# eichenberger/stereo-svo-slam

Measured on AMD Instinct MI355X. Metric: tracked_frames_per_sec, higher is better.
Workload: dtype f32

## Files before the change

### include/svo_hip.h

```cpp
#ifndef SVO_HIP_H
#define SVO_HIP_H

#include <stddef.h>

#include "svo_types.h"

#ifdef __cplusplus
extern "C" {
#endif

enum {
    SVO_OK = 0,
    SVO_ERR_INVALID = -1,
    SVO_ERR_HIP = -2,
    SVO_ERR_NO_DEVICE = -3,
    SVO_ERR_CAPACITY = -4
};

typedef struct svo_handle svo_handle;

const char *svo_last_error(void);
int svo_version(void);

int svo_handle_create(int device, int max_keypoints, svo_handle **out);
int svo_handle_destroy(svo_handle *h);
int svo_handle_set_stream(svo_handle *h, void *hip_stream);
int svo_handle_synchronize(svo_handle *h);
int svo_handle_set_fast_solver(svo_handle *h, int on);
int svo_handle_set_exact_pinv(svo_handle *h, int on);

int svo_device_malloc(size_t bytes, void **out);
int svo_device_free(void *p);
int svo_copy_to_device(svo_handle *h, void *dst, const void *src, size_t bytes);
int svo_copy_to_host(svo_handle *h, void *dst, const void *src, size_t bytes);
int svo_copy_image_to_device(svo_handle *h, void *dst, size_t dst_stride, const void *src,
                             size_t src_stride, size_t width, size_t height);

int svo_build_pyramid(svo_handle *h, int n_levels, svo_image *levels);
int svo_build_lk_pyramid(svo_handle *h, int max_levels, int win, svo_image *levels, int *n_out);

int svo_remap_linear(svo_handle *h, int n, const svo_image *src, svo_image *dst,
                     const float *map_x, const float *map_y);

int svo_remap_linear_multi(svo_handle *h, int n, const svo_image *src, svo_image *dst, int n_maps,
                           const float *const *map_x, const float *const *map_y, const int *map_of_image);

typedef struct svo_camera_calibration {
    double K[9], D[8], R[9], P[9];
} svo_camera_calibration;
int svo_rectify_inverse(const svo_camera_calibration *cal, double ir[9]);
int svo_build_rectify_maps(svo_handle *h, int n, const svo_camera_calibration *cal, int width, int height,
                           float *const *map_x, float *const *map_y);

enum { SVO_INPUT_GRAY_PAIR = 0,
       SVO_INPUT_BGR_PAIR  = 1,
       SVO_INPUT_RGB_PAIR  = 2,
       SVO_INPUT_SBS_GRAY  = 3,
       SVO_INPUT_SBS_BGR   = 4,
       SVO_INPUT_SBS_RGB   = 5,
       SVO_INPUT_CH3_ECON  = 6 };
enum { SVO_INGEST_COPY = 0,
       SVO_INGEST_GRAY = 1 };
typedef struct svo_input_side {
    int32_t buffer;
    int32_t start_column;
    int32_t op, channel;
    int32_t weight[3];
} svo_input_side;
typedef struct svo_input_layout {
    int32_t buffers;
    int32_t channels;
    int32_t min_row_pixels;
    svo_input_side left, right;
} svo_input_layout;
int svo_input_format_info(int format, int width, svo_input_layout *out);
int svo_convert_frames(svo_handle *h, int format, int n, const svo_image *src_a, const svo_image *src_b,
                       svo_image *left, svo_image *right);

int svo_sparse_align(svo_handle *h, const svo_image *prev_pyr, const svo_image *cur_pyr,
                     const svo_kp2d *kps2d, const svo_kp3d *kps3d, const uint32_t *flags, int n,
                     const svo_camera_settings *cam, const float *pose_guess, float *pose_out,
                     float *cost, svo_gn_trace *trace, float *dbg, int dbg_level);

int svo_project_keypoints(svo_handle *h, const float *pose, const svo_kp3d *kps3d, int n,
                          const svo_camera_settings *cam, svo_kp2d *out);

int svo_klt_track(svo_handle *h, const svo_image *prev_lk, const svo_image *cur_lk, int n_levels,
                  const svo_kp2d *prev_pts, svo_kp2d *cur_pts, int n, int win,
                  uint8_t *status, float *err);

int svo_reproj_gn(svo_handle *h, svo_kp2d *kps2d, const svo_kp3d *kps3d, uint32_t *flags, int n,
                  const svo_camera_settings *cam, const svo_kp2d *tracked, const float *err,
                  const float *pose_in, float *pose_out, float *cost, svo_gn_trace *trace);

int svo_ssd_disparity(svo_handle *h, const svo_image *left, const svo_image *right,
                      const svo_kp2d *kps2d, int n, int win, int search_x, int search_y,
                      int clamp_half, float *disparity);

int svo_depth_filter_update(svo_handle *h, const svo_kp2d *kps2d, svo_kp3d *kps3d,
                            const uint32_t *flags, int n, const svo_camera_settings *cam,
                            const float *frame_pose, const float *disparity,
                            const svo_kp3d *ref3d, const svo_kp2d *ref2d, const float *kf_pose,
                            int32_t *outlier_count, int32_t *inlier_count,
                            float *kf_inv_depth, float *kf_variance,
                            int do_outlier_check, int do_update);

typedef struct svo_det_cell {
    float   x, y;
    float   score;
    int32_t type;
} svo_det_cell;
int svo_detect_keypoints(svo_handle *h, int n_levels, const svo_image *levels, int grid_width,
                         int grid_height, int max_cells, svo_det_cell *cells, int32_t *counts);
int svo_detect_shape(int width, int height, int n_levels, int grid_width, int grid_height,
                     int *max_cells, int *cell_width, int *cell_height, int *list_capacity);

typedef struct svo_ctx svo_ctx;

enum { SVO_MEM_HOST = 0, SVO_MEM_DEVICE = 1, SVO_MEM_DEVICE_BORROW = 2 };

int svo_ctx_create(const svo_camera_settings *cam, int width, int height, int n_sequences,
                   int device, svo_ctx **out);
int svo_ctx_destroy(svo_ctx *ctx);

int svo_new_images(svo_ctx *ctx, const uint8_t *const *left, const uint8_t *const *right,
                   int stride, const float *time_stamps, int mem);
int svo_submit_images(svo_ctx *ctx, const uint8_t *const *left, const uint8_t *const *right,
                      int stride, const float *time_stamps, int mem);
int svo_wait(svo_ctx *ctx);
int svo_ctx_get_groups(svo_ctx *ctx, int *n_groups);
int svo_ctx_restart_sequences(svo_ctx *ctx, const int *seqs, int n);
typedef struct svo_run_info {
    int32_t seq, run;
    int32_t frames, keyframes;
    float   last_time_stamp;
    float   pose[6];
} svo_run_info;
int svo_get_finished_runs(svo_ctx *ctx, int seq, int *n);
int svo_get_finished_run(svo_ctx *ctx, int seq, int i, svo_run_info *info, svo_pose *trajectory,
                         int cap, int *n_poses);
int svo_drop_finished_runs(svo_ctx *ctx, int seq);
typedef struct svo_memory {
    int64_t device_bytes;
    int64_t klt_cache_bytes;
    int32_t image_sets, image_sets_free;
    int32_t keyframe_slabs, keyframe_slabs_free;
} svo_memory;
int svo_ctx_get_memory(svo_ctx *ctx, svo_memory *out);
int svo_submit_trim_keyframes(svo_ctx *ctx, const int *seqs, const int *below, int n);
int svo_trim_keyframes(svo_ctx *ctx, const int *seqs, const int *below, int n);
int svo_ctx_set_keyframe_window(svo_ctx *ctx, int keep);
typedef struct svo_keyframe_range {
    int32_t first;
    int32_t retired;
    int32_t count;
    int32_t table;
} svo_keyframe_range;
int svo_get_keyframe_range(svo_ctx *ctx, int seq, svo_keyframe_range *out);
int svo_ctx_set_rectification(svo_ctx *ctx, const float *left_map_x, const float *left_map_y,
                              const float *right_map_x, const float *right_map_y, int mem);
typedef struct svo_rig {
    float baseline, fx, fy, cx, cy, k1, k2, k3, p1, p2;
    const float *left_map_x, *left_map_y, *right_map_x, *right_map_y;
    int32_t mem;
    int32_t _reserved;
} svo_rig;
int svo_ctx_add_rigs(svo_ctx *ctx, const svo_rig *rigs, int n, int *ids);
int svo_ctx_remove_rigs(svo_ctx *ctx, const int *ids, int n);
int svo_ctx_assign_rigs(svo_ctx *ctx, const int *seqs, const int *rigs, int n);
int svo_ctx_get_slot_rig(svo_ctx *ctx, int seq, int *rig, svo_camera_settings *cam);
int svo_ctx_get_rigs(svo_ctx *ctx, int *n, int64_t *map_bytes);
int svo_ctx_add_rigs_calibrated(svo_ctx *ctx, const svo_rig *rigs, const svo_camera_calibration *left,
                                const svo_camera_calibration *right, int n, int *ids);
int svo_ctx_set_calibration(svo_ctx *ctx, const svo_camera_calibration *left, const svo_camera_calibration *right);
int svo_ctx_set_input_format(svo_ctx *ctx, int format);
int svo_new_image(svo_ctx *ctx, const uint8_t *left, int left_stride, const uint8_t *right,
                  int right_stride, int width, int height, float time_stamp);

int svo_get_pose(svo_ctx *ctx, int seq, float pose[6]);
int svo_get_frame_keypoints(svo_ctx *ctx, int seq, svo_kp2d *kps2d, svo_kp3d *kps3d,
                            svo_kp_info *info, int cap, int *n);
int svo_get_keyframe_count(svo_ctx *ctx, int seq, int *count);
int svo_get_keyframe(svo_ctx *ctx, int seq, int id, svo_kp2d *kps2d, svo_kp3d *kps3d,
                     svo_kp_info *info, float pose[6], int cap, int *n);
int svo_get_trajectory(svo_ctx *ctx, int seq, svo_pose *out, int cap, int *n);
int svo_update_pose(svo_ctx *ctx, int seq, const float pose[6], const float speed[6],
                    const float pose_var[6], const float speed_var[6], double dt,
                    float filtered[6]);

int svo_submit_pose_updates(svo_ctx *ctx, const int *seqs, const int *counts, int n,
                            const svo_pose_sample *samples, float *filtered);
int svo_update_poses(svo_ctx *ctx, const int *seqs, const int *counts, int n,
                     const svo_pose_sample *samples, float *filtered);
int svo_pose_filter_batch(svo_handle *h, int n_states, const float *state_in, const float *start_pose,
                          const int *first, int n_samples, const svo_pose_sample *samples, float *state_out,
                          float *filtered);

enum { SVO_EXPORT_FRAMES = 0,
       SVO_EXPORT_LAST_KEYFRAMES = 1 };

typedef struct svo_export_segment {
    int32_t seq, run;
    int32_t frame_id;
    int32_t keyframe_id;
    int32_t is_keyframe;
    int32_t n;
    int64_t first;
    float   pose[6];
    float   time_stamp;
    int32_t _pad;
} svo_export_segment;

typedef struct svo_export_dst {
    svo_export_segment *segments;
    svo_kp2d *kps2d; svo_kp3d *kps3d; svo_kp_info *info;
    int64_t capacity;
} svo_export_dst;

int svo_export_capacity(const svo_camera_settings *cam, int width, int height, int *records_per_sequence);
int svo_submit_export(svo_ctx *ctx, int what, const int *seqs, int n, const svo_export_dst *dst, int mem);
int svo_export(svo_ctx *ctx, int what, const int *seqs, int n, const svo_export_dst *dst, int mem);
int svo_pack_keypoints(svo_handle *h, int n_sets, const svo_keypoints *sets, const int64_t *first,
                       svo_kp2d *kps2d, svo_kp3d *kps3d, svo_kp_info *info);

typedef struct svo_map_point {
    float   x, y, z;
    uint8_t color[3];
    uint8_t flags;
} svo_map_point;

typedef struct svo_map_filter {
    uint32_t drop_flags;
    int32_t  own_only;
    int32_t  min_inliers;
    int32_t  _reserved;
} svo_map_filter;

typedef struct svo_map_keyframe {
    int32_t id, n_total, n, _pad;
    int64_t first;
    float   pose[6];
} svo_map_keyframe;

enum { SVO_MAP_COMPLETE = 0,
       SVO_MAP_TOO_SMALL = 1 };

typedef struct svo_map_segment {
    int32_t seq, run;
    int32_t frame_id;
    int32_t status;
    int32_t n_keyframes, keyframes_retired;
    int32_t from_keyframe, n_exported;
    int64_t n_points;
    int64_t points_bound;
    float   time_stamp;
    union {
        int32_t first_keyframe;
        int32_t _pad[3];
    };
} svo_map_segment;

typedef struct svo_map_region {
    int64_t first_point;
    int64_t point_capacity;
    int64_t first_keyframe_entry;
    int32_t keyframe_capacity;
    int32_t from_keyframe;
} svo_map_region;

typedef struct svo_map_dst {
    svo_map_segment  *segments;
    svo_map_keyframe *keyframes;
    svo_map_point    *points;
} svo_map_dst;

int svo_map_size(svo_ctx *ctx, int seq, int from_keyframe, int *keyframes, int64_t *points_bound);
int svo_submit_export_map(svo_ctx *ctx, const int *seqs, int n, const svo_map_region *regions,
                          const svo_map_filter *filter, const svo_map_dst *dst, int mem);
int svo_export_map(svo_ctx *ctx, const int *seqs, int n, const svo_map_region *regions,
                   const svo_map_filter *filter, const svo_map_dst *dst, int mem);
int svo_pack_map_points(svo_handle *h, int n_regions, const int32_t *set_begin, const svo_keypoints *sets,
                        const int32_t *own_id, const int64_t *first, const svo_map_filter *filter,
                        svo_map_point *points, int32_t *counts);

enum { SVO_PLANE_LEFT = 0, SVO_PLANE_RIGHT = 1 };
enum { SVO_PIXEL_GRAY8 = 0, SVO_PIXEL_RGB8 = 1, SVO_PIXEL_RGBA8 = 2 };
enum { SVO_VIEW_OK = 0,
       SVO_VIEW_NONE = 1 };

typedef struct svo_view_style {
    int32_t  plane;
    int32_t  level;
    int32_t  pixel;
    int32_t  markers;
    uint32_t drop_flags;
    int32_t  size, size_temporary;
    int32_t  _reserved;
} svo_view_style;

typedef struct svo_view_segment {
    int32_t seq, run;
    int32_t frame_id;
    int32_t keyframe_id;
    int32_t status;
    int32_t n;
    int64_t offset;
    float   pose[6];
    float   time_stamp;
    int32_t _pad;
} svo_view_segment;

typedef struct svo_view_dst {
    svo_view_segment *segments;
    uint8_t *pixels;
    int64_t capacity;
} svo_view_dst;

int svo_view_size(const svo_camera_settings *cam, int width, int height, const svo_view_style *style,
                  int *cols, int *rows, int64_t *pitch, int64_t *image_bytes);
int svo_submit_export_views(svo_ctx *ctx, int what, const int *seqs, int n, const svo_view_style *style,
                            const svo_view_dst *dst, int mem);
int svo_export_views(svo_ctx *ctx, int what, const int *seqs, int n, const svo_view_style *style,
                     const svo_view_dst *dst, int mem);
typedef struct svo_view_src {
    svo_image     image;
    svo_keypoints kps;
} svo_view_src;
int svo_render_views(svo_handle *h, int n, const svo_view_src *src, const int64_t *offset,
                     const svo_view_style *style, uint8_t *pixels);

enum { SVO_SCENE_POINTS = 1, SVO_SCENE_TRAJECTORY = 2, SVO_SCENE_KEYFRAMES = 4, SVO_SCENE_POSE = 8 };
enum { SVO_SCENE_CLASS_POSE = 0, SVO_SCENE_CLASS_KEYFRAME = 1, SVO_SCENE_CLASS_TRAJECTORY = 2, SVO_SCENE_CLASS_POINT = 3 };
enum { SVO_SCENE_OK = 0,
       SVO_SCENE_NONE = 1 };

typedef struct svo_scene_camera {
    float view[12];
    float f, cx, cy;
    float near;
} svo_scene_camera;

typedef struct svo_scene_style {
    int32_t  cols, rows;
    int32_t  pixel;
    int32_t  point_size;
    uint32_t background, trajectory_rgb, keyframe_rgb, pose_rgb;
    float    frustum_w, frustum_h, frustum_d;
    uint32_t show;
    int32_t  from_keyframe;
    int32_t  trajectory_tail;
    svo_map_filter filter;
    int32_t  _reserved;
} svo_scene_style;

typedef struct svo_scene_line {
    float    a[3], b[3];
    uint32_t cls_rgb;
    uint32_t _pad;
} svo_scene_line;

typedef struct svo_scene_segment {
    int32_t  seq, run;
    int32_t  frame_id;
    uint16_t status;
    uint16_t n_keyframes;
    int32_t  from_keyframe;
    int32_t  n_keypoints;
    int32_t  n_poses;
    float    time_stamp;
    int64_t  offset;
    float    pose[6];
} svo_scene_segment;

typedef struct svo_scene_dst {
    svo_scene_segment *segments;
    uint8_t *pixels;
    int64_t capacity;
} svo_scene_dst;

int svo_scene_size(const svo_scene_style *style, int64_t *pitch, int64_t *image_bytes);
int svo_scene_look_at(const float eye[3], const float centre[3], const float up[3], float fov_y_deg, int cols, int rows,
                      float near, svo_scene_camera *camera);
int svo_scene_frustum(const float pose[6], const float dims[3], float out[8][6]);
int svo_submit_export_scenes(svo_ctx *ctx, const int *seqs, int n, const svo_scene_style *style,
                             const svo_scene_camera *cameras, const svo_scene_dst *dst, int mem);
int svo_export_scenes(svo_ctx *ctx, const int *seqs, int n, const svo_scene_style *style,
                      const svo_scene_camera *cameras, const svo_scene_dst *dst, int mem);
typedef struct svo_scene_src {
    int32_t cols, rows;
    int32_t n_sets, n_lines;
    const svo_keypoints *sets;
    const int32_t *own_id;
    const svo_scene_line *lines;
} svo_scene_src;
int svo_render_scene(svo_handle *h, int n, const svo_scene_src *src, const svo_scene_camera *cameras,
                     const int64_t *offset, const svo_scene_style *style, uint8_t *pixels);

#define SVO_SNAPSHOT_MAGIC   0x534f5653u
#define SVO_SNAPSHOT_VERSION 1
#define SVO_SNAPSHOT_BYTE_ORDER 0x01020304u
enum { SVO_SNAPSHOT_COMPLETE = 0,
       SVO_SNAPSHOT_TOO_SMALL = 1 };

struct svo_snapshot_info {
    uint32_t magic, version, byte_order;
    uint32_t status;
    int64_t  host_bytes, data_bytes;
    svo_camera_settings cam;
    int32_t  width, height;
    int32_t  capacity;
    int32_t  pyramid_levels, lk_levels;
    int32_t  frame_id;
    int32_t  n_keypoints;
    int32_t  n_trajectory;
    int32_t  n_keyframes, keyframes_retired;
    int32_t  n_image_sets;
    int32_t  n_planes;
    int32_t  first_keyframe;
};
typedef struct svo_snapshot_keyframe {
    float   pose[6];
    int32_t n;
    int32_t image_set;
} svo_snapshot_keyframe;
typedef struct svo_snapshot_plane {
    int64_t offset;
    int32_t row_bytes, rows;
} svo_snapshot_plane;

typedef struct svo_snapshot {
    void   *host;  int64_t host_capacity;
    void   *data;  int64_t data_capacity;
// ... 118 lines not shown
```

### stereo-svo-slam_amd/csrc/svo_ctx.hip

```cpp
#include <hip/hip_runtime.h>

#include <algorithm>
#include <atomic>
#include <climits>
#include <cmath>
#include <condition_variable>
#include <cstdlib>
#include <cstring>
#include <deque>
#include <memory>
#include <mutex>
#include <new>
#include <string>
#include <thread>
#include <vector>

#include "svo_group.hpp"
#include "svo_group_state.hpp"
#include "svo_host.hpp"
#include "svo_kernels.hpp"

struct svo_ctx {
    struct Export {
        int what = 0, mem = 0;
        std::vector<int> seqs, seg;
        int64_t base = 0;
        svo_export_dst dst{};
    };
    struct MapExport {
        int mem = 0;
        std::vector<int> seqs, seg;
        std::vector<svo_map_region> regions;
        svo_map_filter filter{};
        svo_map_dst dst{};
    };
    struct ViewExport {
        int what = 0, mem = 0;
        std::vector<int> seqs, seg;
        svo_view_style style{};
        svo_view_dst dst{};
    };
    struct SceneExport {
        int mem = 0;
        std::vector<int> seqs, seg;
        std::vector<svo_scene_camera> cameras;
        svo_scene_style style{};
        svo_scene_dst dst{};
    };
    struct Snapshots {
        int mem = 0;
        std::vector<int> seqs;
        std::vector<svo_snapshot> snaps;
        std::vector<SnapshotLoad> loads;
    };
    struct PoseUpdates {
        std::vector<int> seqs, counts;
        std::vector<svo_pose_sample> samples;
        std::vector<float*> filtered;
    };
    struct Job {
        std::vector<const uint8_t*> left, right;
        std::vector<float> ts;
        int stride = 0, mem = 0;
        std::vector<int> restart;
        std::vector<int> trim, trim_below;
        std::vector<int> assign;
        std::vector<RigBinding> bindings;
        Export exp;
        Snapshots snap;
        PoseUpdates pose;
        MapExport map;
        ViewExport view;
        SceneExport scene;
    };
    struct Worker {
        Group g;
        int first = 0, count = 0;
        std::thread th;
        std::mutex m;
        std::condition_variable cv, cv_idle;
        std::deque<Job> jobs;
        bool busy = false, stop = false;
        int err = SVO_OK;
        std::string msg;
        std::atomic<bool>* ctx_failed = nullptr;
    };
    int B = 0, device = 0, width = 0, height = 0;
    std::atomic<bool> failed{false};
    std::vector<std::unique_ptr<Worker>> workers;
    svo::DevPtr<uint8_t> rect_mem;
    svo::RemapMap rect[2];
    int input_format = SVO_INPUT_GRAY_PAIR;
    struct Rig {
        bool used = false;
        svo_camera_settings cam{};
        svo::DevPtr<uint8_t> maps;
    };
    std::vector<Rig> rigs;
    std::vector<int> slot_rig;
    size_t rig_map_bytes() const {
        size_t b = 0;
        for (size_t i = 1; i < rigs.size(); i++)
            if (rigs[i].used && rigs[i].maps) b += 2 * svo::remap_map_bytes(width, height);
        return b;
    }
    bool one_buffer() const { return svo::ingest_format(input_format)->buffers == 1; }
};

namespace {

void worker_submit(svo_ctx::Worker& w, svo_ctx::Job&& job);

void worker_run_job(svo_ctx::Worker& w, const svo_ctx::Job& job) {
    if (w.err != SVO_OK || w.ctx_failed->load()) return;
    const svo_ctx::Export& e = job.exp;
    const svo_ctx::Snapshots& sn = job.snap;
    const svo_ctx::PoseUpdates& pu = job.pose;
    const svo_ctx::MapExport& mp = job.map;
    const svo_ctx::ViewExport& vw = job.view;
    const svo_ctx::SceneExport& sc = job.scene;
    const int rc = !sc.seqs.empty()
                       ? grp_export_scenes(w.g.get(), sc.mem, sc.seqs.data(), sc.seg.data(), (int)sc.seqs.size(), w.first, &sc.style, sc.cameras.data(), &sc.dst)
                   : !vw.seqs.empty()
                       ? grp_export_views(w.g.get(), vw.what, vw.mem, vw.seqs.data(), vw.seg.data(), (int)vw.seqs.size(), w.first, &vw.style, &vw.dst)
                   : !mp.seqs.empty()
                       ? grp_export_map(w.g.get(), mp.mem, mp.seqs.data(), mp.seg.data(), mp.regions.data(), (int)mp.seqs.size(), w.first, &mp.filter, &mp.dst)
                   : !pu.seqs.empty()
                       ? grp_pose_updates(w.g.get(), pu.seqs.data(), pu.counts.data(), (int)pu.seqs.size(), pu.samples.data(), pu.filtered.data())
                   : !sn.loads.empty()
                       ? grp_load(w.g.get(), sn.loads.data(), (int)sn.loads.size(), sn.mem)
                   : !sn.seqs.empty()
                       ? grp_save(w.g.get(), sn.seqs.data(), (int)sn.seqs.size(), sn.snaps.data(), sn.mem)
                   : !e.seqs.empty()
                       ? grp_export(w.g.get(), e.what, e.mem, e.seqs.data(), e.seg.data(), (int)e.seqs.size(), w.first, e.base, &e.dst)
                   : !job.assign.empty()
                       ? grp_assign_rigs(w.g.get(), job.assign.data(), job.bindings.data(), (int)job.assign.size())
                   : !job.trim.empty()
                       ? grp_trim_keyframes(w.g.get(), job.trim.data(), job.trim_below.data(), (int)job.trim.size())
                   : !job.restart.empty()
                       ? grp_restart_sequences(w.g.get(), job.restart.data(), (int)job.restart.size())
                       : grp_new_images(w.g.get(), job.left.data(), job.right.empty() ? nullptr : job.right.data(), job.stride,
                                        job.ts.data(), job.mem);
    if (rc != SVO_OK) {
        w.err = rc;
        w.msg = svo_last_error();
        w.ctx_failed->store(true);
    }
}

void worker_loop(svo_ctx::Worker* w) {
    for (;;) {
        svo_ctx::Job job;
        {
            std::unique_lock<std::mutex> lk(w->m);
            w->cv.wait(lk, [w] { return w->stop || !w->jobs.empty(); });
            if (w->jobs.empty()) return;
            job = std::move(w->jobs.front());
            w->jobs.pop_front();
            w->busy = true;
        }
        worker_run_job(*w, job);
        {
            std::lock_guard<std::mutex> lk(w->m);
            w->busy = false;
            if (w->jobs.empty()) w->cv_idle.notify_all();
        }
    }
}

void worker_submit(svo_ctx::Worker& w, svo_ctx::Job&& job) {
    if (w.th.joinable()) {
        {
            std::lock_guard<std::mutex> lk(w.m);
            w.jobs.push_back(std::move(job));
        }
        w.cv.notify_one();
    } else {
        worker_run_job(w, job);
    }
}

int ctx_drain(svo_ctx* c) {
    int rc = SVO_OK;
    for (auto& wp : c->workers) {
        svo_ctx::Worker& w = *wp;
        if (w.th.joinable()) {
            std::unique_lock<std::mutex> lk(w.m);
            w.cv_idle.wait(lk, [&w] { return w.jobs.empty() && !w.busy; });
        }
        if (w.err != SVO_OK && rc == SVO_OK) {
            rc = svo_set_error(w.err, "%s", w.msg.c_str());
            w.err = SVO_OK;
        }
    }
    return rc;
}

int ctx_seq(svo_ctx* c, int seq, svo_group** g, int* local) {
    if (!c || seq < 0 || seq >= c->B) return svo_set_error(SVO_ERR_INVALID, "bad ctx / sequence index");
    const int rc = ctx_drain(c);
    if (rc) return rc;
    for (auto& w : c->workers)
        if (seq < w->first + w->count) {
            *g = w->g.get();
            *local = seq - w->first;
            break;
        }
    HIP_TRY(hipSetDevice(c->device));
    return SVO_OK;
}

}

extern "C" int svo_ctx_create(const svo_camera_settings* cam, int width, int height, int n_sequences,
                              int device, svo_ctx** out) {
    if (!cam || !out || n_sequences < 1) return svo_set_error(SVO_ERR_INVALID, "svo_ctx_create: bad arguments");
    int hwq = 4;
    if (const char* e = std::getenv("GPU_MAX_HW_QUEUES")) hwq = std::max(2, std::atoi(e));
    const int kp_cap = (cam->grid_width > 0 && cam->grid_height > 0 ? (width / cam->grid_width) * (height / cam->grid_height) : 0) + 64;
    const int per_group = std::max(32, std::min(256, 131072 / std::max(kp_cap, 1)));
    int G = n_sequences >= 64 ? std::max(2, (n_sequences + per_group / 2) / per_group) : 1;
    G = std::min(G, hwq - 1);
    if (const char* e = std::getenv("SVO_GROUPS")) G = std::atoi(e);
    G = std::max(1, std::min(G, std::min(n_sequences, 16)));
    std::unique_ptr<svo_ctx> c(new (std::nothrow) svo_ctx());
    if (!c) return svo_set_error(SVO_ERR_INVALID, "out of host memory");
    c->B = n_sequences; c->device = device; c->width = width; c->height = height;
    c->rigs.resize(1);
    c->rigs[0].used = true; c->rigs[0].cam = *cam;
    c->slot_rig.assign(n_sequences, 0);
    int first = 0;
    for (int g = 0; g < G; g++) {
        const int count = n_sequences / G + (g < n_sequences % G ? 1 : 0);
        auto w = std::make_unique<svo_ctx::Worker>();
        w->first = first; w->count = count; w->ctx_failed = &c->failed;
        const int rc = grp_create(cam, width, height, count, device, &w->g);
        if (rc) return rc;
        first += count;
        c->workers.push_back(std::move(w));
    }
    if (G > 1)
        for (auto& w : c->workers) w->th = std::thread(worker_loop, w.get());
    *out = c.release();
    return SVO_OK;
}

extern "C" int svo_ctx_destroy(svo_ctx* c) {
    if (!c) return SVO_OK;
    (void)ctx_drain(c);
    for (auto& w : c->workers) {
        if (w->th.joinable()) {
            {
                std::lock_guard<std::mutex> lk(w->m);
                w->stop = true;
            }
            w->cv.notify_all();
            w->th.join();
        }
        w->g.reset();
    }
    c->rect_mem.reset();
    delete c;
    return SVO_OK;
}

extern "C" int svo_ctx_get_groups(svo_ctx* c, int* n_groups) {
    if (!c || !n_groups) return svo_set_error(SVO_ERR_INVALID, "svo_ctx_get_groups: bad arguments");
    *n_groups = (int)c->workers.size();
    return SVO_OK;
}

extern "C" int svo_submit_images(svo_ctx* c, const uint8_t* const* left, const uint8_t* const* right,
                                 int stride, const float* time_stamps, int mem) {
    if (!c || !left || !time_stamps || (!right && !c->one_buffer()))
        return svo_set_error(SVO_ERR_INVALID, "svo_submit_images: bad arguments");
    const svo::IngestFormat& f = *svo::ingest_format(c->input_format);
    if ((long long)stride < (long long)svo::ingest_row_pixels(f, c->width) * f.channels)
        return svo_set_error(SVO_ERR_INVALID, "svo_submit_images: stride %d is below the row's bytes", stride);
    if (c->failed.load()) {
        const int rc = ctx_drain(c);
        return rc ? rc : svo_set_error(SVO_ERR_INVALID, "svo_submit_images: an earlier frame of this ctx failed; create a new ctx");
    }
    for (auto& wp : c->workers) {
        svo_ctx::Worker& w = *wp;
        svo_ctx::Job job;
        job.left.assign(left + w.first, left + w.first + w.count);
        if (right && !c->one_buffer()) job.right.assign(right + w.first, right + w.first + w.count);
        job.ts.assign(time_stamps + w.first, time_stamps + w.first + w.count);
        job.stride = stride; job.mem = mem;
        worker_submit(w, std::move(job));
    }
    return SVO_OK;
}

extern "C" int svo_ctx_restart_sequences(svo_ctx* c, const int* seqs, int n) {
    if (!c || n < 0 || (n > 0 && !seqs)) return svo_set_error(SVO_ERR_INVALID, "svo_ctx_restart_sequences: bad arguments");
    for (int i = 0; i < n; i++)
        if (seqs[i] < 0 || seqs[i] >= c->B)
            return svo_set_error(SVO_ERR_INVALID, "svo_ctx_restart_sequences: sequence %d out of range", seqs[i]);
    if (c->failed.load()) {
        const int rc = ctx_drain(c);
        return rc ? rc : svo_set_error(SVO_ERR_INVALID, "svo_ctx_restart_sequences: an earlier frame of this ctx failed; create a new ctx");
    }
    for (auto& wp : c->workers) {
        svo_ctx::Worker& w = *wp;
        svo_ctx::Job job;
        for (int i = 0; i < n; i++)
            if (seqs[i] >= w.first && seqs[i] < w.first + w.count) job.restart.push_back(seqs[i] - w.first);
        if (!job.restart.empty()) worker_submit(w, std::move(job));
    }
    return SVO_OK;
}

extern "C" int svo_submit_trim_keyframes(svo_ctx* c, const int* seqs, const int* below, int n) {
    if (!c || (seqs && n < 0)) return svo_set_error(SVO_ERR_INVALID, "svo_submit_trim_keyframes: bad arguments");
    if (!seqs) n = c->B;
    std::vector<char> named(c->B, 0);
    for (int i = 0; i < n; i++) {
        const int s = seqs ? seqs[i] : i;
        if (s < 0 || s >= c->B || named[s])
            return svo_set_error(SVO_ERR_INVALID, "svo_submit_trim_keyframes: sequence %d is out of range or named twice", s);
        named[s] = 1;
    }
    if (c->failed.load()) {
        const int rc = ctx_drain(c);
        return rc ? rc : svo_set_error(SVO_ERR_INVALID, "svo_submit_trim_keyframes: an earlier frame of this ctx failed; create a new ctx");
    }
    for (auto& wp : c->workers) {
        svo_ctx::Worker& w = *wp;
        svo_ctx::Job job;
        for (int i = 0; i < n; i++) {
            const int s = seqs ? seqs[i] : i;
            if (s < w.first || s >= w.first + w.count) continue;
            job.trim.push_back(s - w.first);
            job.trim_below.push_back(below ? below[i] : INT_MAX);
        }
        if (!job.trim.empty()) worker_submit(w, std::move(job));
    }
    return SVO_OK;
}

extern "C" int svo_trim_keyframes(svo_ctx* c, const int* seqs, const int* below, int n) {
    const int rc = svo_submit_trim_keyframes(c, seqs, below, n);
    return rc ? rc : svo_wait(c);
}

extern "C" int svo_ctx_set_keyframe_window(svo_ctx* c, int keep) {
    if (!c || keep < -1) return svo_set_error(SVO_ERR_INVALID, "svo_ctx_set_keyframe_window: bad ctx, or keep %d below -1", keep);
    const int rc = ctx_drain(c);
    if (!rc)
        for (auto& w : c->workers) grp_set_keyframe_window(w->g.get(), keep);
    return rc;
}

extern "C" int svo_get_keyframe_range(svo_ctx* ctx, int seq, svo_keyframe_range* out) {
    svo_group* g; int s;
    if (const int rc = ctx_seq(ctx, seq, &g, &s)) return rc;
    if (out) *out = grp_keyframe_range(g, s);
    return SVO_OK;
}

extern "C" int svo_submit_export(svo_ctx* c, int what, const int* seqs, int n, const svo_export_dst* dst, int mem) {
    if (!c || !dst || !dst->segments || (what != SVO_EXPORT_FRAMES && what != SVO_EXPORT_LAST_KEYFRAMES) ||
        (mem != SVO_MEM_HOST && mem != SVO_MEM_DEVICE) || (seqs && n < 0))
        return svo_set_error(SVO_ERR_INVALID, "svo_submit_export: bad arguments (what %d, mem %d)", what, mem);
    if (!seqs) n = c->B;
    std::vector<char> named(c->B, 0);
    for (int i = 0; i < n; i++) {
        const int s = seqs ? seqs[i] : i;
        if (s < 0 || s >= c->B || named[s])
            return svo_set_error(SVO_ERR_INVALID, "svo_submit_export: sequence %d is out of range or named twice", s);
        named[s] = 1;
    }
    for (const void* p : {(const void*)dst->kps2d, (const void*)dst->kps3d, (const void*)dst->info})
        if ((uintptr_t)p & 3) return svo_set_error(SVO_ERR_INVALID, "svo_submit_export: an array is not 4-byte aligned");
    const int64_t per_seq = grp_capacity(c->workers[0]->g.get());
    if ((dst->kps2d || dst->kps3d || dst->info) && dst->capacity < n * per_seq)
        return svo_set_error(SVO_ERR_CAPACITY, "svo_submit_export: %d slots need arrays of %lld records, capacity %lld", n,
                             (long long)(n * per_seq), (long long)dst->capacity);
    if (c->failed.load()) {
        const int rc = ctx_drain(c);
        return rc ? rc : svo_set_error(SVO_ERR_INVALID, "svo_submit_export: an earlier frame of this ctx failed; create a new ctx");
    }
    int64_t before = 0;
    for (auto& wp : c->workers) {
        svo_ctx::Worker& w = *wp;
        svo_ctx::Job job;
        svo_ctx::Export& e = job.exp;
        for (int i = 0; i < n; i++) {
            const int s = seqs ? seqs[i] : i;
            if (s >= w.first && s < w.first + w.count) { e.seqs.push_back(s - w.first); e.seg.push_back(i); }
        }
        if (e.seqs.empty()) continue;
        e.what = what; e.mem = mem; e.dst = *dst; e.base = before * per_seq;
        before += (int64_t)e.seqs.size();
        worker_submit(w, std::move(job));
    }
    return SVO_OK;
}

extern "C" int svo_export(svo_ctx* c, int what, const int* seqs, int n, const svo_export_dst* dst, int mem) {
    const int rc = svo_submit_export(c, what, seqs, n, dst, mem);
    return rc ? rc : svo_wait(c);
}

namespace {

int check_snapshot_call(svo_ctx* c, const char* name, const int* seqs, int n, const svo_snapshot* snaps, int mem) {
    if (!c || n < 0 || (n > 0 && (!seqs || !snaps)) || (mem != SVO_MEM_HOST && mem != SVO_MEM_DEVICE))
        return svo_set_error(SVO_ERR_INVALID, "%s: bad arguments (mem %d)", name, mem);
    std::vector<char> named(c->B, 0);
    for (int i = 0; i < n; i++) {
        if (seqs[i] < 0 || seqs[i] >= c->B || named[seqs[i]])
            return svo_set_error(SVO_ERR_INVALID, "%s: sequence %d is out of range or named twice", name, seqs[i]);
        named[seqs[i]] = 1;
    }
    return SVO_OK;
}

int reject_failed(svo_ctx* c, const char* name) {
    const int rc = ctx_drain(c);
    return rc ? rc : svo_set_error(SVO_ERR_INVALID, "%s: an earlier frame of this ctx failed; create a new ctx", name);
}

}

extern "C" int svo_submit_export_map(svo_ctx* c, const int* seqs, int n, const svo_map_region* regions,
                                     const svo_map_filter* filter, const svo_map_dst* dst, int mem) {
    if (!c || !dst || !dst->segments || (mem != SVO_MEM_HOST && mem != SVO_MEM_DEVICE) || (seqs && n < 0))
        return svo_set_error(SVO_ERR_INVALID, "svo_submit_export_map: bad arguments (mem %d)", mem);
    if (!seqs) n = c->B;
    if (n > 0 && !regions) return svo_set_error(SVO_ERR_INVALID, "svo_submit_export_map: no regions");
    const svo_map_filter f = filter ? *filter : svo_map_filter{0, 0, 0, 0};
    if ((f.drop_flags & ~(uint32_t)(SVO_IGNORE_DURING_REFINEMENT | SVO_IGNORE_COMPLETELY | SVO_IGNORE_TEMPORARY)) || f._reserved != 0)
        return svo_set_error(SVO_ERR_INVALID, "svo_submit_export_map: drop_flags 0x%x has unknown bits, or _reserved is not 0", f.drop_flags);
    if ((uintptr_t)dst->points & 15) return svo_set_error(SVO_ERR_INVALID, "svo_submit_export_map: points is not 16-byte aligned");
    std::vector<char> named(c->B, 0);
    for (int i = 0; i < n; i++) {
        const int s = seqs ? seqs[i] : i;
        if (s < 0 || s >= c->B || named[s])
            return svo_set_error(SVO_ERR_INVALID, "svo_submit_export_map: sequence %d is out of range or named twice", s);
        named[s] = 1;
        const svo_map_region& r = regions[i];
        if (r.first_point < 0 || r.point_capacity < 0 || r.first_keyframe_entry < 0 || r.keyframe_capacity < 0 || r.from_keyframe < 0)
            return svo_set_error(SVO_ERR_INVALID, "svo_submit_export_map: region %d has a negative field", i);
        if ((r.point_capacity > 0 && !dst->points) || (r.keyframe_capacity > 0 && !dst->keyframes))
            return svo_set_error(SVO_ERR_INVALID, "svo_submit_export_map: region %d has a capacity, but its array is NULL", i);
    }
    if (c->failed.load()) return reject_failed(c, "svo_submit_export_map");
    for (auto& wp : c->workers) {
        svo_ctx::Worker& w = *wp;
        svo_ctx::Job job;
        svo_ctx::MapExport& e = job.map;
        for (int i = 0; i < n; i++) {
            const int s = seqs ? seqs[i] : i;
            if (s >= w.first && s < w.first + w.count) { e.seqs.push_back(s - w.first); e.seg.push_back(i); e.regions.push_back(regions[i]); }
        }
        if (e.seqs.empty()) continue;
        e.mem = mem; e.filter = f; e.dst = *dst;
        worker_submit(w, std::move(job));
    }
    return SVO_OK;
}

extern "C" int svo_export_map(svo_ctx* c, const int* seqs, int n, const svo_map_region* regions, const svo_map_filter* filter,
                              const svo_map_dst* dst, int mem) {
    const int rc = svo_submit_export_map(c, seqs, n, regions, filter, dst, mem);
    return rc ? rc : svo_wait(c);
}

extern "C" int svo_submit_export_views(svo_ctx* c, int what, const int* seqs, int n, const svo_view_style* style,
                                       const svo_view_dst* dst, int mem) {
    if (!c || !dst || !dst->segments || (what != SVO_EXPORT_FRAMES && what != SVO_EXPORT_LAST_KEYFRAMES) ||
        (mem != SVO_MEM_HOST && mem != SVO_MEM_DEVICE) || (seqs && n < 0))
        return svo_set_error(SVO_ERR_INVALID, "svo_submit_export_views: bad arguments (what %d, mem %d)", what, mem);
    const svo_group* g0 = c->workers[0]->g.get();
    if (const int rc = grp_check_view_style(g0, style)) return rc;
    if (!dst->pixels || ((uintptr_t)dst->pixels & 3))
        return svo_set_error(SVO_ERR_INVALID, "svo_submit_export_views: pixels is NULL or not 4-byte aligned");
    if (!seqs) n = c->B;
    std::vector<char> named(c->B, 0);
    for (int i = 0; i < n; i++) {
        const int s = seqs ? seqs[i] : i;
        if (s < 0 || s >= c->B || named[s])
            return svo_set_error(SVO_ERR_INVALID, "svo_submit_export_views: sequence %d is out of range or named twice", s);
        named[s] = 1;
    }
    const int64_t image_bytes = grp_view_bytes(g0, style);
    if (dst->capacity < n * image_bytes)
        return svo_set_error(SVO_ERR_CAPACITY, "svo_submit_export_views: %d slots need %lld bytes, capacity %lld", n,
                             (long long)(n * image_bytes), (long long)dst->capacity);
    if (c->failed.load()) return reject_failed(c, "svo_submit_export_views");
    for (auto& wp : c->workers) {
        svo_ctx::Worker& w = *wp;
        svo_ctx::Job job;
        svo_ctx::ViewExport& e = job.view;
        for (int i = 0; i < n; i++) {
            const int s = seqs ? seqs[i] : i;
            if (s >= w.first && s < w.first + w.count) { e.seqs.push_back(s - w.first); e.seg.push_back(i); }
        }
        if (e.seqs.empty()) continue;
        e.what = what; e.mem = mem; e.style = *style; e.dst = *dst;
        worker_submit(w, std::move(job));
    }
    return SVO_OK;
}

extern "C" int svo_export_views(svo_ctx* c, int what, const int* seqs, int n, const svo_view_style* style,
                                const svo_view_dst* dst, int mem) {
    const int rc = svo_submit_export_views(c, what, seqs, n, style, dst, mem);
    return rc ? rc : svo_wait(c);
}

extern "C" int svo_submit_export_scenes(svo_ctx* c, const int* seqs, int n, const svo_scene_style* style,
                                        const svo_scene_camera* cameras, const svo_scene_dst* dst, int mem) {
    if (!c || !dst || !dst->segments || !cameras || (mem != SVO_MEM_HOST && mem != SVO_MEM_DEVICE) || (seqs && n < 0))
        return svo_set_error(SVO_ERR_INVALID, "svo_submit_export_scenes: bad arguments (mem %d)", mem);
    if (const int rc = svo::scene_check_style(style, "svo_submit_export_scenes")) return rc;
    if (!dst->pixels || ((uintptr_t)dst->pixels & 3))
        return svo_set_error(SVO_ERR_INVALID, "svo_submit_export_scenes: pixels is NULL or not 4-byte aligned");
    if (!seqs) n = c->B;
    std::vector<char> named(c->B, 0);
    for (int i = 0; i < n; i++) {
        const int s = seqs ? seqs[i] : i;
        if (s < 0 || s >= c->B || named[s])
            return svo_set_error(SVO_ERR_INVALID, "svo_submit_export_scenes: sequence %d is out of range or named twice", s);
        named[s] = 1;
        if (const int rc = svo::scene_check_camera(&cameras[i], "svo_submit_export_scenes", i)) return rc;
    }
    const int64_t image_bytes = grp_scene_bytes(style);
    if (dst->capacity < n * image_bytes)
        return svo_set_error(SVO_ERR_CAPACITY, "svo_submit_export_scenes: %d slots need %lld bytes, capacity %lld", n,
                             (long long)(n * image_bytes), (long long)dst->capacity);
    if (c->failed.load()) return reject_failed(c, "svo_submit_export_scenes");
    for (auto& wp : c->workers) {
        svo_ctx::Worker& w = *wp;
        svo_ctx::Job job;
        svo_ctx::SceneExport& e = job.scene;
        for (int i = 0; i < n; i++) {
            const int s = seqs ? seqs[i] : i;
            if (s >= w.first && s < w.first + w.count) { e.seqs.push_back(s - w.first); e.seg.push_back(i); e.cameras.push_back(cameras[i]); }
        }
        if (e.seqs.empty()) continue;
        e.mem = mem; e.style = *style; e.dst = *dst;
        worker_submit(w, std::move(job));
    }
    return SVO_OK;
}

extern "C" int svo_export_scenes(svo_ctx* c, const int* seqs, int n, const svo_scene_style* style,
                                 const svo_scene_camera* cameras, const svo_scene_dst* dst, int mem) {
    const int rc = svo_submit_export_scenes(c, seqs, n, style, cameras, dst, mem);
    return rc ? rc : svo_wait(c);
}

extern "C" int svo_map_size(svo_ctx* ctx, int seq, int from_keyframe, int* keyframes, int64_t* points_bound) {
    if (from_keyframe < 0) return svo_set_error(SVO_ERR_INVALID, "svo_map_size: from_keyframe %d", from_keyframe);
    svo_group* g; int s;
    if (const int rc = ctx_seq(ctx, seq, &g, &s)) return rc;
    grp_map_size(g, s, from_keyframe, keyframes, points_bound);
    return SVO_OK;
}

extern "C" int svo_submit_save(svo_ctx* c, const int* seqs, int n, svo_snapshot* snaps, int mem) {
    if (const int rc = check_snapshot_call(c, "svo_submit_save", seqs, n, snaps, mem)) return rc;
    for (int i = 0; i < n; i++)
        if (!snaps[i].host || snaps[i].host_capacity < (int64_t)sizeof(struct svo_snapshot_info) || snaps[i].data_capacity < 0 ||
            (!snaps[i].data && snaps[i].data_capacity > 0))
            return svo_set_error(SVO_ERR_INVALID, "svo_submit_save: snapshot %d: the host part needs room for its header, the data part its memory", i);
    if (c->failed.load()) return reject_failed(c, "svo_submit_save");
    for (auto& wp : c->workers) {
        svo_ctx::Worker& w = *wp;
        svo_ctx::Job job;
        for (int i = 0; i < n; i++)
            if (seqs[i] >= w.first && seqs[i] < w.first + w.count) {
                job.snap.seqs.push_back(seqs[i] - w.first);
                job.snap.snaps.push_back(snaps[i]);
            }
        if (job.snap.seqs.empty()) continue;
        job.snap.mem = mem;
        worker_submit(w, std::move(job));
    }
    return SVO_OK;
}

extern "C" int svo_save_sequences(svo_ctx* c, const int* seqs, int n, svo_snapshot* snaps, int mem) {
    const int rc = svo_submit_save(c, seqs, n, snaps, mem);
    return rc ? rc : svo_wait(c);
}

extern "C" int svo_submit_load(svo_ctx* c, const int* seqs, int n, const svo_snapshot* snaps, int mem) {
    if (const int rc = check_snapshot_call(c, "svo_submit_load", seqs, n, snaps, mem)) return rc;
    std::vector<SnapshotLoad> loads((size_t)n);
    for (int i = 0; i < n; i++) {
        loads[i].seq = seqs[i];
        loads[i].data = snaps[i].data;
        if (const int rc = grp_check_snapshot(c->workers[0]->g.get(), &c->rigs[c->slot_rig[seqs[i]]].cam, &snaps[i], &loads[i].host))
            return rc;
    }
    if (c->failed.load()) return reject_failed(c, "svo_submit_load");
    for (auto& wp : c->workers) {
        svo_ctx::Worker& w = *wp;
        svo_ctx::Job job;
        for (int i = 0; i < n; i++)
            if (seqs[i] >= w.first && seqs[i] < w.first + w.count) {
                loads[i].seq -= w.first;
                job.snap.loads.push_back(std::move(loads[i]));
            }
        if (job.snap.loads.empty()) continue;
        job.snap.mem = mem;
        worker_submit(w, std::move(job));
    }
    return SVO_OK;
}

extern "C" int svo_load_sequences(svo_ctx* c, const int* seqs, int n, const svo_snapshot* snaps, int mem) {
    const int rc = svo_submit_load(c, seqs, n, snaps, mem);
    return rc ? rc : svo_wait(c);
}

extern "C" int svo_submit_pose_updates(svo_ctx* c, const int* seqs, const int* counts, int n, const svo_pose_sample* samples,
                                       float* filtered) {
    if (!c || !counts || (seqs && n < 0)) return svo_set_error(SVO_ERR_INVALID, "svo_submit_pose_updates: bad arguments");
    if (!seqs) n = c->B;
    std::vector<char> named(c->B, 0);
    std::vector<int64_t> first((size_t)n + 1, 0);
    for (int i = 0; i < n; i++) {
        const int s = seqs ? seqs[i] : i;
        if (s < 0 || s >= c->B || named[s])
            return svo_set_error(SVO_ERR_INVALID, "svo_submit_pose_updates: sequence %d is out of range or named twice", s);
        named[s] = 1;
        if (counts[i] < 0) return svo_set_error(SVO_ERR_INVALID, "svo_submit_pose_updates: sequence %d: negative count", s);
        first[i + 1] = first[i] + counts[i];
    }
    const int64_t total = first[n];
    if (total > (1 << 24)) return svo_set_error(SVO_ERR_INVALID, "svo_submit_pose_updates: %lld samples in one call", (long long)total);
    if (total > 0 && !samples) return svo_set_error(SVO_ERR_INVALID, "svo_submit_pose_updates: no samples");
    for (int64_t k = 0; k < total; k++)
        if (samples[k].flags & ~(uint32_t)SVO_POSE_SAMPLE_CHAIN)
            return svo_set_error(SVO_ERR_INVALID, "svo_submit_pose_updates: sample %lld: unknown flag bits 0x%x", (long long)k, samples[k].flags);
    if (c->failed.load()) return reject_failed(c, "svo_submit_pose_updates");
    for (auto& wp : c->workers) {
        svo_ctx::Worker& w = *wp;
        svo_ctx::Job job;
        svo_ctx::PoseUpdates& u = job.pose;
        for (int i = 0; i < n; i++) {
            const int s = seqs ? seqs[i] : i;
            if (counts[i] == 0 || s < w.first || s >= w.first + w.count) continue;
            u.seqs.push_back(s - w.first);
            u.counts.push_back(counts[i]);
            u.samples.insert(u.samples.end(), samples + first[i], samples + first[i + 1]);
            u.filtered.push_back(filtered ? filtered + first[i] * 6 : nullptr);
        }
        if (!u.seqs.empty()) worker_submit(w, std::move(job));
    }
    return SVO_OK;
}

extern "C" int svo_update_poses(svo_ctx* c, const int* seqs, const int* counts, int n, const svo_pose_sample* samples,
                                float* filtered) {
    const int rc = svo_submit_pose_updates(c, seqs, counts, n, samples, filtered);
    return rc ? rc : svo_wait(c);
}

extern "C" int svo_snapshot_size(svo_ctx* ctx, int seq, int64_t* host_bytes, int64_t* data_bytes) {
    svo_group* g; int s;
    if (const int rc = ctx_seq(ctx, seq, &g, &s)) return rc;
    return grp_snapshot_size(g, s, host_bytes, data_bytes);
}

extern "C" int svo_drop_finished_runs(svo_ctx* c, int seq) {
    if (!c || seq >= c->B) return svo_set_error(SVO_ERR_INVALID, "bad ctx / sequence index");
    const int rc = ctx_drain(c);
    if (rc) return rc;
    for (auto& w : c->workers) {
        if (seq < 0) grp_drop_finished_runs(w->g.get(), -1);
        else if (seq >= w->first && seq < w->first + w->count) grp_drop_finished_runs(w->g.get(), seq - w->first);
    }
    return SVO_OK;
}

extern "C" int svo_ctx_get_memory(svo_ctx* c, svo_memory* out) {
    if (!c || !out) return svo_set_error(SVO_ERR_INVALID, "svo_ctx_get_memory: bad arguments");
    const int rc = ctx_drain(c);
    if (rc) return rc;
    std::memset(out, 0, sizeof(*out));
    for (auto& w : c->workers) {
        const svo_memory m = grp_memory(w->g.get());
        out->device_bytes += m.device_bytes; out->klt_cache_bytes += m.klt_cache_bytes;
        out->image_sets += m.image_sets; out->image_sets_free += m.image_sets_free;
        out->keyframe_slabs += m.keyframe_slabs; out->keyframe_slabs_free += m.keyframe_slabs_free;
    }
    out->device_bytes += (int64_t)c->rig_map_bytes();
    return SVO_OK;
}

extern "C" int svo_wait(svo_ctx* c) {
    if (!c) return svo_set_error(SVO_ERR_INVALID, "svo_wait: bad ctx");
    return ctx_drain(c);
}

extern "C" int svo_new_images(svo_ctx* c, const uint8_t* const* left, const uint8_t* const* right,
                              int stride, const float* time_stamps, int mem) {
    const int rc = svo_submit_images(c, left, right, stride, time_stamps, mem);
    return rc ? rc : svo_wait(c);
}

extern "C" int svo_new_image(svo_ctx* c, const uint8_t* left, int left_stride, const uint8_t* right,
                             int right_stride, int width, int height, float time_stamp) {
    if (!c || c->B != 1) return svo_set_error(SVO_ERR_INVALID, "svo_new_image needs a 1-sequence ctx");
    if (width != c->width || height != c->height || (!c->one_buffer() && left_stride != right_stride))
        return svo_set_error(SVO_ERR_INVALID, "svo_new_image: image size / stride mismatch");
    return grp_new_images(c->workers[0]->g.get(), &left, &right, left_stride, &time_stamp, SVO_MEM_HOST);
}

extern "C" int svo_ctx_set_input_format(svo_ctx* c, int format) {
    if (!c || !svo::ingest_format(format))
        return svo_set_error(SVO_ERR_INVALID, "svo_ctx_set_input_format: unknown format %d", format);
    const int rc = ctx_drain(c);
    if (rc) return rc;
    for (size_t i = 0; i < c->workers.size(); i++) {
        const int e = grp_set_input_format(c->workers[i]->g.get(), format);
        if (e == SVO_OK) continue;
        for (size_t k = 0; k < i; k++) (void)grp_set_input_format(c->workers[k]->g.get(), c->input_format);
        return e;
    }
    c->input_format = format;
    return SVO_OK;
}

namespace {

int rig_cameras(const char* who, const svo_ctx* c, const svo_camera_calibration* left, const svo_camera_calibration* right,
                int n, std::vector<svo::RigCam>& cams) {
    const long long tiles = (long long)((c->width + svo::REMAP_TILE - 1) / svo::REMAP_TILE) * ((c->height + svo::REMAP_TILE - 1) / svo::REMAP_TILE);
    if (tiles * 2 * n >= svo::RIG_MAX_WORKGROUPS) return svo_set_error(SVO_ERR_INVALID, "%s: %d rigs are too many for one call", who, n);
    cams.resize(2 * (size_t)n);
    for (int i = 0; i < n; i++)
        for (int side = 0; side < 2; side++)
            if (!svo::rig_camera(side ? right[i] : left[i], cams[2 * (size_t)i + side]))
                return svo_set_error(SVO_ERR_INVALID, "%s: rig %d, %s camera: a value is not finite, or P R has no inverse", who, i,
                                     side ? "right" : "left");
    return SVO_OK;
}

int build_calibrated_maps(svo_ctx* c, std::vector<svo::RigCam>& cams, std::vector<svo::DevPtr<uint8_t>>& out) {
    const size_t n = cams.size() / 2, map_bytes = svo::remap_map_bytes(c->width, c->height);
    std::vector<svo::DevPtr<uint8_t>> made(n);
    for (size_t i = 0; i < n; i++) {
        HIP_TRY(svo::dev_malloc(made[i], 2 * map_bytes));
        cams[2 * i].fixed = made[i].get();
        cams[2 * i + 1].fixed = made[i].get() + map_bytes;
    }
    if (n == 0) return SVO_OK;
    svo::DevPtr<svo::RigCam> table;
    HIP_TRY(svo::dev_malloc(table, sizeof(svo::RigCam) * cams.size()));
    svo::Stream st;
    HIP_TRY(svo::make_stream(st));
    HIP_TRY(hipMemcpyAsync(table.get(), cams.data(), sizeof(svo::RigCam) * cams.size(), hipMemcpyHostToDevice, st.get()));
    svo::launch_rig_maps(table.get(), (int)cams.size(), c->width, c->height, true, st.get());
    HIP_TRY(hipGetLastError());
    HIP_TRY(hipStreamSynchronize(st.get()));
    out = std::move(made);
    return SVO_OK;
}

}

extern "C" int svo_ctx_set_calibration(svo_ctx* c, const svo_camera_calibration* left, const svo_camera_calibration* right) {
    if (!c || (left != nullptr) != (right != nullptr))
        return svo_set_error(SVO_ERR_INVALID, "svo_ctx_set_calibration: give both calibrations or none");
    if (!left) return svo_ctx_set_rectification(c, nullptr, nullptr, nullptr, nullptr, SVO_MEM_HOST);
    std::vector<svo::RigCam> cams;
    if (const int e = rig_cameras("svo_ctx_set_calibration", c, left, right, 1, cams)) return e;
    const int rc = ctx_drain(c);
    if (rc) return rc;
    HIP_TRY(hipSetDevice(c->device));
    std::vector<svo::DevPtr<uint8_t>> made;
    if (const int e = build_calibrated_maps(c, cams, made)) return e;
    const size_t map_bytes = svo::remap_map_bytes(c->width, c->height);
    for (int side = 0; side < 2; side++) c->rect[side] = svo::remap_map_view(made[0].get() + side * map_bytes, c->width, c->height);
    c->rect_mem = std::move(made[0]);
    for (auto& w : c->workers) grp_set_rectification(w->g.get(), c->rect);
    return SVO_OK;
}

extern "C" int svo_ctx_set_rectification(svo_ctx* c, const float* left_map_x, const float* left_map_y,
                                         const float* right_map_x, const float* right_map_y, int mem) {
    const float* maps[4] = {left_map_x, left_map_y, right_map_x, right_map_y};
    const int given = (int)std::count_if(maps, maps + 4, [](const float* p) { return p != nullptr; });
    if (!c || (given != 0 && given != 4) || (mem != SVO_MEM_HOST && mem != SVO_MEM_DEVICE))
        return svo_set_error(SVO_ERR_INVALID, "svo_ctx_set_rectification: give all four maps or none, mem host or device");
    const int rc = ctx_drain(c);
    if (rc) return rc;
    HIP_TRY(hipSetDevice(c->device));
    if (given == 0) {
        for (auto& w : c->workers) grp_set_rectification(w->g.get(), nullptr);
        c->rect_mem.reset();
        return SVO_OK;
    }
    const size_t map_bytes = svo::remap_map_bytes(c->width, c->height);
    const size_t plane = sizeof(float) * (size_t)c->width * c->height;
    svo::DevPtr<uint8_t> mem_new;
    HIP_TRY(svo::dev_malloc(mem_new, 2 * map_bytes + (mem == SVO_MEM_HOST ? 4 * plane : 0)));
    svo::Stream st;
    HIP_TRY(svo::make_stream(st));
    const float* dev_maps[4];
    for (int i = 0; i < 4; i++) {
        if (mem == SVO_MEM_HOST) {
            float* d = reinterpret_cast<float*>(mem_new.get() + 2 * map_bytes + i * plane);
            HIP_TRY(hipMemcpyAsync(d, maps[i], plane, hipMemcpyHostToDevice, st.get()));
            dev_maps[i] = d;
        } else {
            dev_maps[i] = maps[i];
        }
    }
    svo::RemapMap rect[2];
    for (int side = 0; side < 2; side++) {
        rect[side] = svo::remap_map_view(mem_new.get() + side * map_bytes, c->width, c->height);
        svo::launch_remap_prep(dev_maps[2 * side], dev_maps[2 * side + 1], rect[side], st.get());
        HIP_TRY(hipGetLastError());
    }
    HIP_TRY(hipStreamSynchronize(st.get()));
    c->rect[0] = rect[0];
    c->rect[1] = rect[1];
    c->rect_mem = std::move(mem_new);
    for (auto& w : c->workers) grp_set_rectification(w->g.get(), c->rect);
    return SVO_OK;
}


namespace {

int build_rig_maps(svo_ctx* c, const float* const maps[4], int mem, svo::DevPtr<uint8_t>& out) {
    const size_t map_bytes = svo::remap_map_bytes(c->width, c->height);
    const size_t plane = sizeof(float) * (size_t)c->width * c->height;
    svo::DevPtr<uint8_t> mem_new, stage;
    HIP_TRY(svo::dev_malloc(mem_new, 2 * map_bytes));
    if (mem == SVO_MEM_HOST) HIP_TRY(svo::dev_malloc(stage, 4 * plane));
    svo::Stream st;
    HIP_TRY(svo::make_stream(st));
    const float* dev_maps[4];
    for (int i = 0; i < 4; i++) {
        dev_maps[i] = maps[i];
        if (mem != SVO_MEM_HOST) continue;
        float* d = reinterpret_cast<float*>(stage.get() + i * plane);
        HIP_TRY(hipMemcpyAsync(d, maps[i], plane, hipMemcpyHostToDevice, st.get()));
        dev_maps[i] = d;
    }
    for (int side = 0; side < 2; side++) {
        svo::launch_remap_prep(dev_maps[2 * side], dev_maps[2 * side + 1],
                               svo::remap_map_view(mem_new.get() + side * map_bytes, c->width, c->height), st.get());
        HIP_TRY(hipGetLastError());
    }
    HIP_TRY(hipStreamSynchronize(st.get()));
    out = std::move(mem_new);
    return SVO_OK;
}

bool rig_exists(const svo_ctx* c, int id) { return id >= 0 && id < (int)c->rigs.size() && c->rigs[id].used; }

}

namespace {

int check_rigs(const char* who, const svo_rig* rigs, int n) {
    for (int i = 0; i < n; i++) {
        const svo_rig& r = rigs[i];
        const float v[10] = {r.baseline, r.fx, r.fy, r.cx, r.cy, r.k1, r.k2, r.k3, r.p1, r.p2};
        for (float x : v)
            if (!std::isfinite(x)) return svo_set_error(SVO_ERR_INVALID, "%s: rig %d has a value that is not finite", who, i);
        if (!(r.fx > 0) || !(r.fy > 0)) return svo_set_error(SVO_ERR_INVALID, "%s: rig %d: fx and fy must be positive", who, i);
        const int given = (r.left_map_x != nullptr) + (r.left_map_y != nullptr) + (r.right_map_x != nullptr) + (r.right_map_y != nullptr);
        if ((given != 0 && given != 4) || (given == 4 && r.mem != SVO_MEM_HOST && r.mem != SVO_MEM_DEVICE) || r._reserved != 0)
            return svo_set_error(SVO_ERR_INVALID, "%s: rig %d: give all four maps or none, mem host or device, _reserved 0", who, i);
    }
    return SVO_OK;
}

svo_ctx::Rig new_rig(const svo_ctx* c, const svo_rig& r) {
    svo_ctx::Rig out;
    svo_camera_settings& s = out.cam;
    s = c->rigs[0].cam;
    s.baseline = r.baseline; s.fx = r.fx; s.fy = r.fy; s.cx = r.cx; s.cy = r.cy;
    s.k1 = r.k1; s.k2 = r.k2; s.k3 = r.k3; s.p1 = r.p1; s.p2 = r.p2;
    out.used = true;
    return out;
}

}

extern "C" int svo_ctx_add_rigs(svo_ctx* c, const svo_rig* rigs, int n, int* ids) {
    if (!c || n < 0 || (n > 0 && (!rigs || !ids))) return svo_set_error(SVO_ERR_INVALID, "svo_ctx_add_rigs: bad arguments");
    if (const int e = check_rigs("svo_ctx_add_rigs", rigs, n)) return e;
    const int rc = ctx_drain(c);
    if (rc) return rc;
    HIP_TRY(hipSetDevice(c->device));
    std::vector<svo_ctx::Rig> made((size_t)n);
    for (int i = 0; i < n; i++) {
        const svo_rig& r = rigs[i];
        made[i] = new_rig(c, r);
        if (!r.left_map_x) continue;
        const float* const maps[4] = {r.left_map_x, r.left_map_y, r.right_map_x, r.right_map_y};
        if (const int e = build_rig_maps(c, maps, r.mem, made[i].maps)) return e;
    }
    for (int i = 0; i < n; i++) {
        ids[i] = (int)c->rigs.size();
        c->rigs.push_back(std::move(made[i]));
    }
    return SVO_OK;
}

extern "C" int svo_ctx_add_rigs_calibrated(svo_ctx* c, const svo_rig* rigs, const svo_camera_calibration* left,
                                           const svo_camera_calibration* right, int n, int* ids) {
    const char* who = "svo_ctx_add_rigs_calibrated";
    if (!c || n < 0 || (n > 0 && (!rigs || !left || !right || !ids))) return svo_set_error(SVO_ERR_INVALID, "%s: bad arguments", who);
    if (const int e = check_rigs(who, rigs, n)) return e;
    for (int i = 0; i < n; i++)
        if (rigs[i].left_map_x) return svo_set_error(SVO_ERR_INVALID, "%s: rig %d: the maps come from the calibrations, the map pointers are NULL", who, i);
    std::vector<svo::RigCam> cams;
    if (const int e = rig_cameras(who, c, left, right, n, cams)) return e;
    const int rc = ctx_drain(c);
    if (rc) return rc;
    HIP_TRY(hipSetDevice(c->device));
    std::vector<svo::DevPtr<uint8_t>> maps;
    if (const int e = build_calibrated_maps(c, cams, maps)) return e;
    for (int i = 0; i < n; i++) {
        svo_ctx::Rig r = new_rig(c, rigs[i]);
        r.maps = std::move(maps[i]);
        ids[i] = (int)c->rigs.size();
        c->rigs.push_back(std::move(r));
    }
    return SVO_OK;
}

extern "C" int svo_ctx_remove_rigs(svo_ctx* c, const int* ids, int n) {
    if (!c || n < 0 || (n > 0 && !ids)) return svo_set_error(SVO_ERR_INVALID, "svo_ctx_remove_rigs: bad arguments");
    const int rc = ctx_drain(c);
    if (rc) return rc;
    for (int i = 0; i < n; i++) {
        if (ids[i] == 0 || !rig_exists(c, ids[i]))
            return svo_set_error(SVO_ERR_INVALID, "svo_ctx_remove_rigs: rig %d is rig 0 or does not exist", ids[i]);
        if (std::find(c->slot_rig.begin(), c->slot_rig.end(), ids[i]) != c->slot_rig.end())
            return svo_set_error(SVO_ERR_INVALID, "svo_ctx_remove_rigs: a slot is bound to rig %d", ids[i]);
    }
    HIP_TRY(hipSetDevice(c->device));
    for (int i = 0; i < n; i++) {
        c->rigs[ids[i]].used = false;
        c->rigs[ids[i]].maps.reset();
    }
    return SVO_OK;
}

extern "C" int svo_ctx_assign_rigs(svo_ctx* c, const int* seqs, const int* rigs, int n) {
    if (!c || n < 0 || (n > 0 && (!seqs || !rigs))) return svo_set_error(SVO_ERR_INVALID, "svo_ctx_assign_rigs: bad arguments");
    for (int i = 0; i < n; i++) {
        if (seqs[i] < 0 || seqs[i] >= c->B)
            return svo_set_error(SVO_ERR_INVALID, "svo_ctx_assign_rigs: sequence %d out of range", seqs[i]);
        if (!rig_exists(c, rigs[i])) return svo_set_error(SVO_ERR_INVALID, "svo_ctx_assign_rigs: rig %d does not exist", rigs[i]);
    }
    if (c->failed.load()) return reject_failed(c, "svo_ctx_assign_rigs");
    const size_t map_bytes = svo::remap_map_bytes(c->width, c->height);
    for (auto& wp : c->workers) {
        svo_ctx::Worker& w = *wp;
        svo_ctx::Job job;
        for (int i = 0; i < n; i++) {
            if (seqs[i] < w.first || seqs[i] >= w.first + w.count) continue;
            const svo_ctx::Rig& r = c->rigs[rigs[i]];
            const uint8_t* base = r.maps.get();
            job.assign.push_back(seqs[i] - w.first);
            job.bindings.push_back(RigBinding{rigs[i], r.cam, {base, base ? base + map_bytes : nullptr}});
        }
        if (!job.assign.empty()) worker_submit(w, std::move(job));
    }
    for (int i = 0; i < n; i++) c->slot_rig[seqs[i]] = rigs[i];
    return SVO_OK;
}

extern "C" int svo_ctx_get_slot_rig(svo_ctx* c, int seq, int* rig, svo_camera_settings* cam) {
    if (!c || seq < 0 || seq >= c->B) return svo_set_error(SVO_ERR_INVALID, "bad ctx / sequence index");
    const int rc = ctx_drain(c);
    if (rc) return rc;
    if (rig) *rig = c->slot_rig[seq];
    if (cam) *cam = c->rigs[c->slot_rig[seq]].cam;
    return SVO_OK;
}

extern "C" int svo_ctx_get_rigs(svo_ctx* c, int* n, int64_t* map_bytes) {
    if (!c) return svo_set_error(SVO_ERR_INVALID, "svo_ctx_get_rigs: bad ctx");
    const int rc = ctx_drain(c);
    if (rc) return rc;
    if (n) *n = (int)std::count_if(c->rigs.begin(), c->rigs.end(), [](const svo_ctx::Rig& r) { return r.used; });
    if (map_bytes) *map_bytes = (int64_t)c->rig_map_bytes();
    return SVO_OK;
}

extern "C" int svo_ctx_set_exact_pinv(svo_ctx* c, int on);
extern "C" int svo_ctx_set_fast_solver(svo_ctx* c, int on) { return svo_ctx_set_exact_pinv(c, on == 0); }

// ... 173 lines not shown
```

### stereo-svo-slam_amd/csrc/svo_group.hip

```cpp
#include <hip/hip_runtime.h>

#include <algorithm>
#include <cstdio>
#include <cstdlib>
#include <cstring>
#include <memory>
#include <new>
#include <vector>

#include "svo_group_state.hpp"

using namespace svo;

void GroupDelete::operator()(svo_group* c) const {
    (void)hipSetDevice(c->device);
    if (c->stream) (void)hipStreamSynchronize(c->stream.get());
    if (std::getenv("SVO_HOST_TIMING") && c->host_steps > 0) {
        static const char* names[7] = {"args", "launch", "pose_filter", "wait_frame", "kf_enqueue", "wait_kf", "bookkeeping"};
        std::fprintf(stderr, "[svo host ms/step over %ld steps]", c->host_steps);
        for (int i = 0; i < 7; i++) std::fprintf(stderr, " %s=%.3f", names[i], c->host_ms[i] / c->host_steps);
        std::fprintf(stderr, "\n");
    }
    delete c;
}

namespace svo {

size_t align_up(size_t v, size_t a) { return (v + a - 1) / a * a; }

void dev_release(svo_group* c, void* p, size_t bytes) {
    for (auto it = c->dev_mem.begin(); it != c->dev_mem.end(); ++it)
        if (it->get() == p) {
            c->dev_mem.erase(it);
            c->device_bytes -= bytes;
            return;
        }
}


static int grow_set_slabs(svo_group* c, int count) {
    uint8_t* base = nullptr;
    const int rc = dev_alloc(c, &base, c->set_layout.bytes * (size_t)count, false);
    if (rc) return rc;
    for (int i = count - 1; i >= 0; i--) c->set_slabs.push_back(base + c->set_layout.bytes * (size_t)i);
    return SVO_OK;
}

static SetLayout image_set_layout(const svo_group* c) {
    SetLayout t{};
    size_t off = 0;
    auto place = [&off](ImgView& v, size_t& at, int w, int h) {
        v = ImgView{nullptr, w, h, (int)align_up((size_t)std::max(w, 1), 64)};
        at = off;
        off += align_up((size_t)v.stride * std::max(h, 1), 256);
    };
    int w = c->width, h = c->height;
    for (int l = 0; l < c->cam.max_pyramid_levels; l++, w /= 2, h /= 2) place(t.views.left[l], t.left[l], w, h);
    place(t.views.right, t.right, c->width, c->height);
    w = c->width; h = c->height;
    for (int l = 1; l < c->n_lk; l++) {
        w = (w + 1) / 2; h = (h + 1) / 2;
        place(t.views.lk[l], t.lk[l], w, h);
    }
    t.bytes = off;
    return t;
}

static int new_image_set(svo_group* c, Seq& q) {
    if (c->set_slabs.empty()) {
        const int rc = grow_set_slabs(c, std::max(c->B, 16));
        if (rc) return rc;
    }
    const SetLayout& t = c->set_layout;
    auto s = std::make_unique<ImageSet>(t.views);
    s->base = c->set_slabs.back();
    c->set_slabs.pop_back();
    for (int l = 0; l < c->cam.max_pyramid_levels; l++) s->left[l].data = s->base + t.left[l];
    s->right.data = s->base + t.right;
    s->lk[0] = s->left[0];
    s->own_left0 = s->left[0];
    s->own_right = s->right;
    for (int l = 1; l < c->n_lk; l++) s->lk[l].data = s->base + t.lk[l];
    q.free_sets.push_back(s.get());
    q.sets.push_back(std::move(s));
    c->image_sets++;
    return SVO_OK;
}

int acquire_set(svo_group* c, Seq& q, ImageSet** out) {
    if (q.free_sets.empty()) {
        const int rc = new_image_set(c, q);
        if (rc) return rc;
    }
    *out = q.free_sets.back();
    q.free_sets.pop_back();
    (*out)->refs = 1;
    return SVO_OK;
}

void release_set(Seq& q, ImageSet*& s) {
    if (s && --s->refs <= 0) q.free_sets.push_back(s);
    s = nullptr;
}

static int alloc_kps(svo_group* c, KpsDev& k, int* n_ptr) {
    int rc = SVO_OK;
    auto alloc = [&](auto** p) { if (!rc) rc = dev_alloc(c, p, (size_t)c->cap); };
    alloc(&k.kps2d); alloc(&k.kps3d); alloc(&k.flags); alloc(&k.kf_id); alloc(&k.kp_index); alloc(&k.outl);
    alloc(&k.inl); alloc(&k.kfx); alloc(&k.kfP); alloc(&k.score); alloc(&k.level_type); alloc(&k.color);
    k.n = n_ptr;
    return rc;
}

static size_t kf_slab_bytes(const svo_group* c) { return align_up((size_t)c->cap * 15 * 4, 256); }

static int grow_kf_slabs(svo_group* c, int count) {
    const size_t sb = kf_slab_bytes(c);
    uint8_t* base = nullptr;
    const int rc = dev_alloc(c, &base, sb * count, false);
    if (rc) return rc;
    for (int i = count - 1; i >= 0; i--) c->kf_slabs.push_back(base + sb * i);
    c->kf_slab_count += count;
    return SVO_OK;
}

static KpsDev carve_kps(uint8_t* base, size_t cap) {
    KpsDev k;
    std::memset(&k, 0, sizeof(k));
    k.kps3d = reinterpret_cast<svo_kp3d*>(base);
    k.kps2d = reinterpret_cast<svo_kp2d*>(base + cap * sizeof(svo_kp3d));
    k.flags = reinterpret_cast<uint32_t*>(base + cap * (sizeof(svo_kp3d) + sizeof(svo_kp2d)));
    k.outl = reinterpret_cast<int*>(k.flags + cap);
    k.inl = k.outl + cap;
    k.kf_id = k.inl + cap;
    k.kp_index = k.kf_id + cap;
    k.score = reinterpret_cast<float*>(k.kp_index + cap);
    k.level_type = reinterpret_cast<int*>(k.score + cap);
    k.color = reinterpret_cast<uint32_t*>(k.level_type + cap);
    k.kfx = reinterpret_cast<float*>(k.color + cap);
    k.kfP = k.kfx + cap;
    return k;
}

void fill_kf_record(const svo_group* c, const Seq& q, int id, const KfHost& k, KfDev& d) {
    clear(d);
    if (k.set)
        for (int l = 0; l < c->n_lk; l++) d.lk[l] = k.set->lk[l];
    d.n_lk = c->n_lk;
    d.kps2d = k.kps.kps2d; d.kps3d = k.kps.kps3d; d.flags = k.kps.flags;
    d.outlier_count = k.kps.outl; d.inlier_count = k.kps.inl;
    d.kf_id = k.kps.kf_id; d.kp_index = k.kps.kp_index; d.score = k.kps.score; d.level_type = k.kps.level_type;
    d.color = k.kps.color; d.kfx = k.kps.kfx; d.kfP = k.kps.kfP;
    if (c->tmpl_kf > 0) {
        const int r = id % c->tmpl_kf;
        d.tmpl = q.tmpl_base + (size_t)r * c->tmpl_block_bytes;
        d.tmpl_valid = q.tmpl_valid + (size_t)r * c->tmpl_valid_bytes;
        d.tmpl_cap = c->tmpl_cap;
        d.tmpl_win = c->cam.window_size_opt_flow;
    }
}

int take_kf_slab(svo_group* c, KpsDev* out) {
    if (c->kf_slabs.empty()) {
        const int rc = grow_kf_slabs(c, std::max(c->B, 32));
        if (rc) return rc;
    }
    *out = carve_kps(c->kf_slabs.back(), c->cap);
    c->kf_slabs.pop_back();
    return SVO_OK;
}


int check_settings(const svo_camera_settings* cam, int width, int height, int n_sequences) {
    if (!cam || width < 16 || height < 16 || n_sequences < 1)
        return svo_set_error(SVO_ERR_INVALID, "svo_ctx_create: bad arguments");
    if (cam->max_pyramid_levels < 1 || cam->max_pyramid_levels > 7 ||
        cam->min_pyramid_level_pose_estimation < 0 ||
        cam->min_pyramid_level_pose_estimation >= cam->max_pyramid_levels)
        return svo_set_error(SVO_ERR_INVALID, "max_pyramid_levels must be 1..7 and > min level");
    if (cam->window_size_opt_flow < 3 || cam->window_size_opt_flow > 35 ||
        cam->window_size_depth_calculator < 1 || cam->window_size_depth_calculator > 35 ||
        cam->search_x < 0 || cam->search_x > 64 || cam->search_y < 0 || cam->search_y > 8)
        return svo_set_error(SVO_ERR_INVALID, "windows <= 35, search_x <= 64, search_y <= 8 supported");
    if (cam->window_size_pose_estimator != 4)
        return svo_set_error(SVO_ERR_INVALID, "window_size_pose_estimator must be 4");
    if (cam->grid_width < 4 || cam->grid_height < 4 || cam->grid_width > 96 || cam->grid_height > 64)
        return svo_set_error(SVO_ERR_INVALID, "grid cell must be within 4..96 x 4..64");
    return SVO_OK;
}

int keypoint_capacity(const svo_camera_settings& cam, int width, int height) {
    const int cells = (width / cam.grid_width) * (height / cam.grid_height);
    return (int)align_up((size_t)(2 * cells + 128), 64);
}

int usable_lk_levels(const svo_camera_settings& cam, int width, int height) {
    for (int l = 0, w = width, h = height; l < SVO_LK_LEVELS; l++) {
        w = (w + 1) / 2; h = (h + 1) / 2;
        if (w <= cam.window_size_opt_flow || h <= cam.window_size_opt_flow) return l + 1;
    }
    return SVO_LK_LEVELS;
}


static void size_group(svo_group* c) {
    const svo_camera_settings& cam = c->cam;
    const int width = c->width, height = c->height;
    c->cap = keypoint_capacity(cam, width, height);
    c->rec_cap = (int)align_up((size_t)c->cap, 512);
    c->max_kf = MAX_KEYFRAMES;
    if (const char* e = std::getenv("SVO_KEYFRAME_TABLE")) {
        const int t = std::atoi(e);
        if (t >= 4 && t <= MAX_KEYFRAMES && (t & (t - 1)) == 0) c->max_kf = t;
    }
    if (const char* e = std::getenv("SVO_KEEP_KEYFRAME_IMAGES")) c->retire_kf_images = std::atoi(e) == 0;
    c->n_lk = usable_lk_levels(cam, width, height);
    c->det_levels = cam.max_pyramid_levels / 2;
    c->max_cells = 1;
    for (int l = 0; l < c->det_levels; l++) {
        const int gw = cam.grid_width >> l, gh = cam.grid_height >> l;
        if (gw <= 0 || gh <= 0) { c->det_levels = l; break; }
        const int nc = ((width >> l) / gw) * std::max((height >> l) / gh, 1);
        c->max_cells = std::max(c->max_cells, nc);
    }
    c->merge_cells = ((width + cam.grid_height - 1) / cam.grid_height) *
                     ((height + cam.grid_width - 1) / cam.grid_width);
    c->set_layout = image_set_layout(c);
}

static int alloc_blocks(svo_group* c) {
    ArgBlocks& a = c->args;
    const size_t B = c->B;
    size_t off = 0;
    auto size = [&](auto& arr) { off += align_up(sizeof(typename std::decay_t<decltype(arr)>::type) * B, 256); };
    a.frame_arrays(size);
    a.frame_bytes = off;
    a.rig_arrays(size);
    a.frame_rig_bytes = off;
    a.keyframe_arrays(size);
    a.bytes = off;
    HIP_TRY(pinned_malloc(a.host, a.bytes));
    std::memset(a.host.get(), 0, a.bytes);
    int rc;
    if ((rc = dev_alloc(c, &a.dev, a.bytes))) return rc;
    off = 0;
    auto place = [&](auto& arr) {
        using T = typename std::decay_t<decltype(arr)>::type;
        arr.h = reinterpret_cast<T*>(a.host.get() + off);
        arr.d = reinterpret_cast<T*>(a.dev + off);
        off += align_up(sizeof(T) * B, 256);
    };
    a.frame_arrays(place);
    a.rig_arrays(place);
    a.keyframe_arrays(place);

    const size_t res_bytes = sizeof(FrameResult) * B, n_bytes = sizeof(int) * 2 * B, in_bytes = sizeof(int) * B;
    c->readback_bytes = res_bytes + n_bytes;
    uint8_t* db = nullptr;
    HIP_TRY(pinned_malloc(c->readback_host, res_bytes + n_bytes + in_bytes));
    uint8_t* hb = c->readback_host.get();
    std::memset(hb, 0, res_bytes + n_bytes + in_bytes);
    if ((rc = dev_alloc(c, &db, res_bytes + n_bytes + in_bytes))) return rc;
    c->h_res = reinterpret_cast<FrameResult*>(hb); c->d_res = reinterpret_cast<FrameResult*>(db);
    c->h_n = reinterpret_cast<int*>(hb + res_bytes); c->d_n_all = reinterpret_cast<int*>(db + res_bytes);
    c->h_inside = reinterpret_cast<int*>(hb + res_bytes + n_bytes);
    c->d_inside = reinterpret_cast<int*>(db + res_bytes + n_bytes);
    return SVO_OK;
}

static int alloc_sequence(svo_group* c, Seq& q, int s) {
    q.d_n = c->d_n_all + 2 * s;
    int rc = alloc_kps(c, q.kps[0], q.d_n);
    if (!rc) rc = alloc_kps(c, q.kps[1], q.d_n + 1);
    auto alloc = [&](auto** p, size_t count) { if (!rc) rc = dev_alloc(c, p, count); };
    const size_t cap = c->cap, cells = c->max_cells;
    alloc(&q.tracked, cap); alloc(&q.klt_err, cap); alloc(&q.klt_status, cap); alloc(&q.disparity, cap);
    alloc(&q.sia_rec, sia_rec_ws_floats(c->cam, c->rec_cap)); alloc(&q.sia_kpws, (size_t)9 * c->rec_cap);
    alloc(&q.sia_mats, 1); alloc(&q.d_kfs, c->max_kf);
    alloc(&q.det, SVO_MAX_PYRAMID_LEVELS * cells); alloc(&q.n_det, SVO_MAX_PYRAMID_LEVELS);
    alloc(&q.sel, cells); alloc(&q.sel_level, cells); alloc(&q.sel_cell, cells); alloc(&q.occupied, c->merge_cells);
    alloc(&q.color_lcg, 1);
    if (rc) return rc;
    q.kf.init();
    std::memset(&q.stats, 0, sizeof(q.stats));
    for (int i = 0; i < 4; i++)
        if ((rc = new_image_set(c, q))) return rc;
    return SVO_OK;
}

static int alloc_template_cache(svo_group* c) {
    const int B = c->B;
    const int cells = (c->width / c->cam.grid_width) * (c->height / c->cam.grid_height);
    c->tmpl_cap = std::min(c->cap, cells + 64);
    c->tmpl_block_bytes = align_up((size_t)c->tmpl_cap * SVO_LK_LEVELS * klt_template_bytes(c->cam.window_size_opt_flow), 256);
    int K = c->tmpl_block_bytes <= ((size_t)8 << 20) ? 8 : 4;
    if (const char* e = std::getenv("SVO_KLT_CACHE_KF")) K = std::max(0, std::min(std::atoi(e), 64));
    c->tmpl_valid_bytes = align_up((size_t)c->tmpl_cap * SVO_LK_LEVELS, 256);
    size_t free_b = 0, total_b = 0;
    HIP_TRY(hipMemGetInfo(&free_b, &total_b));
    while (K > 0 && (size_t)B * K * c->tmpl_block_bytes > free_b / 3) K--;
    c->tmpl_kf = K;
    if (K == 0) return SVO_OK;
    uint8_t* base = nullptr; uint8_t* vbase = nullptr;
    int rc;
    if ((rc = dev_alloc(c, &base, (size_t)B * K * c->tmpl_block_bytes, false))) return rc;
    if ((rc = dev_alloc(c, &vbase, (size_t)B * K * c->tmpl_valid_bytes))) return rc;
    for (int s = 0; s < B; s++) {
        c->seqs[s].tmpl_base = base + (size_t)s * K * c->tmpl_block_bytes;
        c->seqs[s].tmpl_valid = vbase + (size_t)s * K * c->tmpl_valid_bytes;
    }
    return SVO_OK;
}

template <typename T>
static int alloc_mirrored_table(svo_group* c, ArgArray<T>& table, PinnedPtr<T>& host, size_t n) {
    PinnedPtr<T> pinned;
    HIP_TRY(pinned_malloc(pinned, sizeof(T) * n));
    T* dev = nullptr;
    if (const int rc = dev_alloc(c, &dev, n)) return rc;
    host = std::move(pinned);
    table.h = host.get();
    table.d = dev;
    return SVO_OK;
}

}

int grp_create(const svo_camera_settings* cam, int width, int height, int n_sequences, int device, Group* out) {
    int rc = check_settings(cam, width, height, n_sequences);
    if (rc) return rc;
    int count = 0;
    if (hipGetDeviceCount(&count) != hipSuccess || count <= 0)
        return svo_set_error(SVO_ERR_NO_DEVICE, "no HIP device visible: libsvo_hip has no CPU fallback");
    if (device < 0 || device >= count) return svo_set_error(SVO_ERR_INVALID, "device %d out of range", device);
    HIP_TRY(hipSetDevice(device));
    Group g(new (std::nothrow) svo_group());
    svo_group* c = g.get();
    if (!c) return svo_set_error(SVO_ERR_INVALID, "out of host memory");
    c->fmt = ingest_format(SVO_INPUT_GRAY_PAIR);
    c->device = device; c->B = n_sequences; c->width = width; c->height = height; c->cam = *cam;
    std::memset(&c->totals, 0, sizeof(c->totals));
    HIP_TRY(make_stream(c->stream));
    size_group(c);
    if ((rc = alloc_blocks(c))) return rc;
    for (Event& e : c->ev) HIP_TRY(make_event(e));
    c->seqs.resize(n_sequences);
    for (Seq& q : c->seqs) q.cam = c->cam;
    if ((rc = grow_set_slabs(c, 4 * n_sequences))) return rc;
    for (int s = 0; s < n_sequences; s++)
        if ((rc = alloc_sequence(c, c->seqs[s], s))) return rc;
    if ((rc = grow_kf_slabs(c, std::max(2 * n_sequences, 32)))) return rc;
    if ((rc = alloc_template_cache(c))) return rc;
    if ((rc = alloc_mirrored_table(c, c->remap_img, c->remap_img_host, 2 * (size_t)n_sequences))) return rc;
    HIP_TRY(hipDeviceSynchronize());
    *out = std::move(g);
    return SVO_OK;
}

void grp_set_exact_pinv(svo_group* c, int on) { c->exact_pinv = on != 0; }
void grp_set_rectification(svo_group* c, const RemapMap* maps) { c->rect = maps; }
void grp_enable_timing(svo_group* c, int on) { c->timing = on != 0; }

int grp_set_input_format(svo_group* c, int format) {
    if (converts(format) && !c->ingest_img.d) {
        HIP_TRY(hipSetDevice(c->device));
        if (const int rc = alloc_mirrored_table(c, c->ingest_img, c->ingest_img_host, 2 * (size_t)c->B)) return rc;
    }
    c->input_format = format;
    c->fmt = ingest_format(format);
    return SVO_OK;
}

svo_totals grp_totals(const svo_group* c) {
    svo_totals t = c->totals;
    t.image_sets = c->image_sets;
    return t;
}

const std::vector<svo_launch_shape>& grp_launch_shapes(const svo_group* c) { return c->launch_shapes; }

namespace svo {

void flush_one(Seq& q) {
    if (!q.pending) return;
    q.pending = false;
    float prev_pose[6];
    std::memcpy(prev_pose, q.pose, sizeof(prev_pose));
    std::memcpy(q.pose, q.pending_pose, sizeof(q.pose));
    const double dt = q.pending_ts - q.ts;
    const double inv = 1. / dt;
    float motion[6];
    for (int i = 0; i < 6; i++) motion[i] = (float)((q.pose[i] - prev_pose[i]) * inv);
    const float pv[6] = {0.1f, 0.1f, 0.1f, 0.1f, 0.1f, 0.1f};
    const float mv[6] = {1, 1, 1, 1, 1, 1};
    float filtered[6];
    q.kf.update(q.pose, motion, pv, mv, 0.0, filtered);
    std::memcpy(q.pose, filtered, sizeof(q.pose));
    q.ts = q.pending_ts;
    svo_pose p;
    std::memcpy(&p, q.pose, sizeof(p));
    q.trajectory.push_back(p);
}

void flush_pending(svo_group* c) {
    for (Seq& q : c->seqs) flush_one(q);
}


void end_sequence(svo_group* c, int s) {
    Seq& q = c->seqs[s];
    if (q.frame_id < 0) return;
    flush_one(q);
    FinishedRun f;
    clear(f.info);
    f.info.seq = s; f.info.run = q.run; f.info.frames = q.frame_id + 1; f.info.keyframes = (int)q.kfs.size();
    f.info.last_time_stamp = (float)q.ts;
    std::memcpy(f.info.pose, q.pose, sizeof(f.info.pose));
    f.trajectory = std::move(q.trajectory);
    c->finished.push_back(std::move(f));
    for (KfHost& k : q.kfs) {
        release_set(q, k.set);
        c->kf_slabs.push_back(reinterpret_cast<uint8_t*>(k.kps.kps3d));
    }
    release_set(q, q.cur_set);
    release_set(q, q.prev_set);
    q.kfs.clear();
    q.kfs_retired = 0;
    q.trajectory.clear();
    q.cur = 0; q.n_host = 0; q.frame_id = -1; q.ts = 0; q.run++;
    std::memset(q.pose, 0, sizeof(q.pose));
    q.kf.init();
    clear(q.stats);
}

void trim_keyframes(svo_group* c, Seq& q, int below) {
    const int to = std::min(below, q.kfs_retired);
    if (to <= q.kfs.first()) return;
    for (int id = q.kfs.first(); id < to; id++) {
        KfHost& k = q.kfs[(size_t)id];
        release_set(q, k.set);
        c->kf_slabs.push_back(reinterpret_cast<uint8_t*>(k.kps.kps3d));
    }
    q.kfs.drop_below(to);
}

}

int grp_trim_keyframes(svo_group* c, const int* seqs, const int* below, int n) {
    if (c->failed)
        return svo_set_error(SVO_ERR_INVALID, "svo_submit_trim_keyframes: an earlier frame of this ctx failed; create a new ctx");
    for (int i = 0; i < n; i++) trim_keyframes(c, c->seqs[seqs[i]], below[i]);
    return SVO_OK;
}

void grp_set_keyframe_window(svo_group* c, int keep) { c->kf_window = keep; }

svo_keyframe_range grp_keyframe_range(const svo_group* c, int seq) {
    const Seq& q = c->seqs[seq];
    return svo_keyframe_range{q.kfs.first(), q.kfs_retired, (int)q.kfs.size(), c->max_kf};
}

int grp_restart_sequences(svo_group* c, const int* seqs, int n) {
    if (c->failed)
        return svo_set_error(SVO_ERR_INVALID, "svo_ctx_restart_sequences: an earlier frame of this ctx failed; create a new ctx");
    for (int i = 0; i < n; i++) end_sequence(c, seqs[i]);
    return SVO_OK;
}

int grp_assign_rigs(svo_group* c, const int* seqs, const RigBinding* b, int n) {
    if (c->failed)
        return svo_set_error(SVO_ERR_INVALID, "svo_ctx_assign_rigs: an earlier frame of this ctx failed; create a new ctx");
    for (int i = 0; i < n; i++) {
        end_sequence(c, seqs[i]);
        Seq& q = c->seqs[seqs[i]];
        q.rig = b[i].rig; q.cam = b[i].cam;
        q.rig_maps[0] = b[i].rig ? b[i].maps[0] : nullptr;
        q.rig_maps[1] = b[i].rig ? b[i].maps[1] : nullptr;
    }
    return SVO_OK;
}

void grp_drop_finished_runs(svo_group* c, int seq) {
    if (seq < 0) { c->finished.clear(); return; }
    c->finished.erase(std::remove_if(c->finished.begin(), c->finished.end(),
                                     [seq](const FinishedRun& f) { return f.info.seq == seq; }),
                      c->finished.end());
}

svo_memory grp_memory(const svo_group* c) {
    svo_memory m;
    clear(m);
    m.device_bytes = (int64_t)c->device_bytes;
    m.klt_cache_bytes = (int64_t)((size_t)c->B * c->tmpl_kf * (c->tmpl_block_bytes + c->tmpl_valid_bytes));
    m.image_sets = c->image_sets;
    for (const Seq& q : c->seqs) m.image_sets_free += (int)q.free_sets.size();
    m.keyframe_slabs = c->kf_slab_count;
    m.keyframe_slabs_free = (int)c->kf_slabs.size();
    return m;
}
```

### stereo-svo-slam_amd/csrc/svo_group.hpp

```cpp
#pragma once

#include <cstdint>
#include <memory>
#include <vector>

#include "../../include/svo_hip.h"

namespace svo { struct RemapMap; }
struct svo_group;
struct GroupDelete { void operator()(svo_group* g) const; };
using Group = std::unique_ptr<svo_group, GroupDelete>;

int grp_create(const svo_camera_settings* cam, int width, int height, int n_sequences, int device, Group* out);
int grp_new_images(svo_group* g, const uint8_t* const* left, const uint8_t* const* right, int stride,
                   const float* time_stamps, int mem);
int grp_restart_sequences(svo_group* g, const int* seqs, int n);
int grp_trim_keyframes(svo_group* g, const int* seqs, const int* below, int n);
void grp_set_keyframe_window(svo_group* g, int keep);
svo_keyframe_range grp_keyframe_range(const svo_group* g, int seq);
struct RigBinding {
    int rig;
    svo_camera_settings cam;
    const uint8_t* maps[2];
};
int grp_assign_rigs(svo_group* g, const int* seqs, const RigBinding* b, int n);
int grp_export(svo_group* g, int what, int mem, const int* seqs, const int* seg, int n, int seq0, int64_t base,
               const svo_export_dst* dst);
int grp_export_map(svo_group* g, int mem, const int* seqs, const int* seg, const svo_map_region* regions, int n, int seq0,
                   const svo_map_filter* filter, const svo_map_dst* dst);
int grp_export_views(svo_group* g, int what, int mem, const int* seqs, const int* seg, int n, int seq0,
                     const svo_view_style* style, const svo_view_dst* dst);
int grp_check_view_style(const svo_group* g, const svo_view_style* style);
int64_t grp_view_bytes(const svo_group* g, const svo_view_style* style);
int grp_export_scenes(svo_group* g, int mem, const int* seqs, const int* seg, int n, int seq0, const svo_scene_style* style,
                      const svo_scene_camera* cameras, const svo_scene_dst* dst);
int64_t grp_scene_bytes(const svo_scene_style* style);
void grp_map_size(const svo_group* g, int seq, int from_keyframe, int* keyframes, int64_t* points_bound, int* from = nullptr);
struct SnapshotLoad {
    int seq;
    std::vector<uint8_t> host;
    const void* data;
};
int grp_check_snapshot(const svo_group* g, const svo_camera_settings* slot_cam, const svo_snapshot* snap,
                       std::vector<uint8_t>* host_copy);
int grp_save(svo_group* g, const int* seqs, int n, const svo_snapshot* snaps, int mem);
int grp_load(svo_group* g, const SnapshotLoad* loads, int n, int mem);
int grp_snapshot_size(svo_group* g, int seq, int64_t* host_bytes, int64_t* data_bytes);
int grp_pose_updates(svo_group* g, const int* seqs, const int* counts, int n, const svo_pose_sample* samples,
                     float* const* filtered);
int grp_capacity(const svo_group* g);
void grp_drop_finished_runs(svo_group* g, int seq);
svo_memory grp_memory(const svo_group* g);
void grp_set_exact_pinv(svo_group* g, int on);
void grp_set_rectification(svo_group* g, const svo::RemapMap* maps);
int grp_set_input_format(svo_group* g, int format);
void grp_enable_timing(svo_group* g, int on);
svo_totals grp_totals(const svo_group* g);
const std::vector<svo_launch_shape>& grp_launch_shapes(const svo_group* g);
```

### stereo-svo-slam_amd/csrc/svo_group_state.hpp

```cpp
#pragma once

#include <hip/hip_runtime.h>

#include <algorithm>
#include <cmath>
#include <cstddef>
#include <cstdint>
#include <cstring>
#include <memory>
#include <vector>

#include "svo_group.hpp"
#include "svo_host.hpp"
#include "svo_tracker.hpp"
namespace svo {

struct PoseFilter {
    static constexpr int N = 12;
    float statePre[N], statePost[N];
    float A[N * N], Hm[N * N], Q[N * N], R[N * N];
    float errorCovPre[N * N], errorCovPost[N * N], gain[N * N];

    static void identity(float* m, float v) {
        std::memset(m, 0, sizeof(float) * N * N);
        for (int i = 0; i < N; i++) m[i * N + i] = v;
    }
    void init() {
        std::memset(this, 0, sizeof(*this));
        identity(A, 1.f); identity(Hm, 1.f); identity(Q, 100.f); identity(R, 1.f);
        identity(errorCovPost, 1.f);
    }
    static void gemm(const float* a, const float* b, bool bt, double alpha, const float* c,
                     double beta, float* d, int m, int k, int n) {
        float tmp[N * N];
        for (int i = 0; i < m; i++)
            for (int j = 0; j < n; j++) {
                double s = 0;
                for (int p = 0; p < k; p++)
                    s += (double)a[i * k + p] * (double)(bt ? b[j * k + p] : b[p * n + j]);
                s *= alpha;
                if (c) s += (double)c[i * n + j] * beta;
                tmp[i * n + j] = (float)s;
            }
        std::memcpy(d, tmp, sizeof(float) * m * n);
    }
    static void solve_svd(const float* Am, const float* B, float* X) {
        float At[N][N], Vt[N][N], W[N];
        for (int i = 0; i < N; i++)
            for (int j = 0; j < N; j++) At[i][j] = Am[j * N + i];
        jacobi_svd<N, N>(At, W, Vt);
        for (int i = 0; i < N * N; i++) X[i] = 0;
        double threshold = 0;
        for (int i = 0; i < N; i++) threshold += W[i];
        threshold *= (float)(DBL_EPSILON * 2);
        for (int i = 0; i < N; i++) {
            double wi = W[i];
            if (std::fabs(wi) <= threshold) continue;
            wi = 1 / wi;
            double buffer[N];
            for (int j = 0; j < N; j++) buffer[j] = 0;
            for (int r = 0; r < N; r++) {
                const float s = At[i][r];
                for (int j = 0; j < N; j++) buffer[j] = buffer[j] + (double)(s * B[r * N + j]);
            }
            for (int j = 0; j < N; j++) buffer[j] *= wi;
            for (int r = 0; r < N; r++) {
                const float s = Vt[i][r];
                for (int j = 0; j < N; j++) X[r * N + j] = (float)(X[r * N + j] + s * buffer[j]);
            }
        }
    }
    void predict() {
        float temp1[N * N];
        gemm(A, statePost, false, 1, nullptr, 0, statePre, N, N, 1);
        gemm(A, errorCovPost, false, 1, nullptr, 0, temp1, N, N, N);
        gemm(temp1, A, true, 1, Q, 1, errorCovPre, N, N, N);
        std::memcpy(statePost, statePre, sizeof(statePre));
        std::memcpy(errorCovPost, errorCovPre, sizeof(errorCovPre));
    }
    void correct(const float* z) {
        float temp2[N * N], temp3[N * N], temp4[N * N], temp5[N], hx[N];
        gemm(Hm, errorCovPre, false, 1, nullptr, 0, temp2, N, N, N);
        gemm(temp2, Hm, true, 1, R, 1, temp3, N, N, N);
        solve_svd(temp3, temp2, temp4);
        for (int i = 0; i < N; i++)
            for (int j = 0; j < N; j++) gain[i * N + j] = temp4[j * N + i];
        gemm(Hm, statePre, false, 1, nullptr, 0, hx, N, N, 1);
        for (int i = 0; i < N; i++) temp5[i] = z[i] - hx[i];
        gemm(gain, temp5, false, 1, statePre, 1, statePost, N, N, 1);
        gemm(gain, temp2, false, -1, errorCovPre, 1, errorCovPost, N, N, N);
    }
    void update(const float pose[6], const float speed[6], const float pv[6], const float sv[6],
                double dt, float filtered[6]) {
        for (int i = 0; i < 6; i++) A[i * N + 6 + i] = (float)dt;
        predict();
        for (int i = 0; i < 6; i++) { R[i * N + i] = pv[i]; R[(6 + i) * N + 6 + i] = sv[i]; }
        float z[N];
        for (int i = 0; i < 6; i++) { z[i] = pose[i]; z[6 + i] = speed[i]; }
        correct(z);
        for (int i = 0; i < 6; i++) filtered[i] = statePost[i];
    }
};

struct ImageSet {
    uint8_t* base = nullptr;
    ImgView left[SVO_MAX_PYRAMID_LEVELS];
    ImgView right;
    ImgView lk[SVO_LK_LEVELS];
    ImgView own_left0, own_right;
    int refs = 0;
};

struct SetLayout {
    ImageSet views;
    size_t left[SVO_MAX_PYRAMID_LEVELS], right, lk[SVO_LK_LEVELS];
    size_t bytes;
};

struct FrameResult {
    float pose_sia[6];
    float pose_refined[6];
    float sia_cost, reproj_cost;
    int inside, overflow, kf_n, old_count;
    int min_kf;
    unsigned live_kf[2];
    svo_gn_trace sia_trace[SVO_MAX_PYRAMID_LEVELS];
    svo_gn_trace reproj_trace;
};

struct KfHost {
    ImageSet* set;
    float pose[6];
    int n;
    KpsDev kps;
};

class KfList {
  public:
    int first() const { return first_; }
    size_t size() const { return (size_t)first_ + v_.size(); }
    int resident() const { return (int)v_.size(); }
    bool empty() const { return v_.empty(); }
    KfHost& operator[](size_t id) { return v_[id - (size_t)first_]; }
    const KfHost& operator[](size_t id) const { return v_[id - (size_t)first_]; }
    KfHost& back() { return v_.back(); }
    const KfHost& back() const { return v_.back(); }
    void push_back(const KfHost& k) { v_.push_back(k); }
    std::vector<KfHost>::iterator begin() { return v_.begin(); }
    std::vector<KfHost>::iterator end() { return v_.end(); }
    std::vector<KfHost>::const_iterator begin() const { return v_.begin(); }
    std::vector<KfHost>::const_iterator end() const { return v_.end(); }
    void drop_below(int id) {
        v_.erase(v_.begin(), v_.begin() + (id - first_));
        first_ = id;
    }
    void clear(int first = 0) { v_.clear(); first_ = first; }
  private:
    std::vector<KfHost> v_;
    int first_ = 0;
};

struct Seq {
    KpsDev kps[2];
    int cur = 0;
    int* d_n = nullptr;
    svo_kp2d* tracked = nullptr;
    float* klt_err = nullptr;
    uint8_t* klt_status = nullptr;
    float* disparity = nullptr;
    float* sia_rec = nullptr;
    float* sia_kpws = nullptr;
    PoseMats* sia_mats = nullptr;
    uint8_t* tmpl_base = nullptr;
    uint8_t* tmpl_valid = nullptr;
    KfDev* d_kfs = nullptr;
    KfList kfs;
    int kfs_retired = 0;
    DetCell* det = nullptr; int* n_det = nullptr;
    DetCell* sel = nullptr; int* sel_level = nullptr; int* sel_cell = nullptr; int* occupied = nullptr;
    uint32_t* color_lcg = nullptr;
    std::vector<std::unique_ptr<ImageSet>> sets;
    std::vector<ImageSet*> free_sets;
    ImageSet* cur_set = nullptr;
    ImageSet* prev_set = nullptr;
    int rig = 0;
    svo_camera_settings cam{};
    const uint8_t* rig_maps[2] = {nullptr, nullptr};
    PoseFilter kf;
    int frame_id = -1;
    int run = 0;
    double ts = 0;
    float pose[6] = {0, 0, 0, 0, 0, 0};
    std::vector<svo_pose> trajectory;
    svo_frame_stats stats;
    int n_host = 0;
    bool pending = false;
    float pending_pose[6] = {0, 0, 0, 0, 0, 0};
    double pending_ts = 0;
};

struct FinishedRun {
    svo_run_info info;
    std::vector<svo_pose> trajectory;
};

template <typename T>
struct ArgArray {
    using type = T;
    T* h = nullptr;
    T* d = nullptr;
};

struct ArgBlocks {
    ArgArray<PyrArgs> pyr;
    ArgArray<CompactArgs> compact;
    ArgArray<SiaArgs> sia;
    ArgArray<KltArgs> klt;
    ArgArray<ReprojArgs> reproj;
    ArgArray<SsdArgs> ssd;
    ArgArray<FilterArgs> filter;
    ArgArray<float[8]> guess;
    ArgArray<RemapChunk> remap_chunk;
    ArgArray<DetectArgs> detect;
    ArgArray<MergeArgs> merge;
    ArgArray<KfInitArgs> kf_init;
    ArgArray<int> enable;
    ArgArray<KfDev> kf_record;
    template <typename F> void frame_arrays(F f) { f(pyr); f(compact); f(sia); f(klt); f(reproj); f(ssd); f(filter); f(guess); }
    template <typename F> void rig_arrays(F f) { f(remap_chunk); }
    template <typename F> void keyframe_arrays(F f) { f(detect); f(merge); f(kf_init); f(enable); f(kf_record); }
    PinnedPtr<uint8_t> host;
    uint8_t* dev = nullptr;
    size_t frame_bytes = 0, frame_rig_bytes = 0, bytes = 0;
};

}

struct svo_group {
    svo::Stream stream;
    int device, B, width, height, cap, rec_cap, max_kf, n_lk, det_levels, max_cells, merge_cells;
    svo_camera_settings cam;
    std::vector<svo::DevPtr<void>> dev_mem;
    std::vector<svo::Seq> seqs;
    svo::ArgBlocks args;
    svo::PinnedPtr<uint8_t> readback_host;
    svo::FrameResult* d_res = nullptr; svo::FrameResult* h_res = nullptr;
    int* h_n = nullptr;
    int* d_n_all = nullptr;
    int* d_inside = nullptr; int* h_inside = nullptr;
    size_t readback_bytes = 0;
    uint8_t* d_stage_in = nullptr; size_t stage_frame_bytes = 0;
    const svo::RemapMap* rect = nullptr;
    svo::ArgArray<svo::RemapImg> remap_img;
    svo::PinnedPtr<svo::RemapImg> remap_img_host;
    int input_format = SVO_INPUT_GRAY_PAIR;
    const svo::IngestFormat* fmt = nullptr;
    svo::ArgArray<svo::IngestImg> ingest_img;
    svo::PinnedPtr<svo::IngestImg> ingest_img_host;
    uint8_t* d_raw_gray = nullptr; size_t raw_plane_bytes = 0;
    uint8_t* d_export = nullptr;
    uint8_t* d_snap = nullptr; size_t snap_bytes = 0;
    int* d_map_counts = nullptr; size_t map_counts = 0;
    svo::PinnedPtr<int> map_counts_host;
    svo_map_point* d_map_points = nullptr; size_t map_points = 0;
    uint8_t* d_view = nullptr; size_t view_bytes = 0;
    uint8_t* d_scene_in = nullptr; size_t scene_in_bytes = 0;
    svo::PinnedPtr<uint8_t> scene_in_host;
    uint8_t* d_scene = nullptr; size_t scene_bytes = 0;
    uint8_t* d_pose = nullptr; size_t pose_up_bytes = 0, pose_down_bytes = 0;
    svo::PinnedPtr<uint8_t> pose_host;
    bool timing = false;
    bool failed = false;
    int exact_pinv = 1;
    svo::Event ev[10];
    svo::SetLayout set_layout;
    std::vector<uint8_t*> kf_slabs;
    int kf_slab_count = 0;
    size_t device_bytes = 0;
    std::vector<svo::FinishedRun> finished;
    std::vector<uint8_t*> set_slabs;
    int tmpl_kf = 0, tmpl_cap = 0;
    size_t tmpl_block_bytes = 0, tmpl_valid_bytes = 0;
    svo_totals totals;
    std::vector<svo_launch_shape> launch_shapes;
    bool retire_kf_images = true;
    int kf_window = -1;
    int image_sets = 0;
    double host_ms[8] = {0, 0, 0, 0, 0, 0, 0, 0};
    long host_steps = 0;
};

namespace svo {

template <typename T>
T& clear(T& x) {
    std::memset(&x, 0, sizeof(x));
    return x;
}

template <typename T>
int dev_alloc(svo_group* c, T** p, size_t count, bool zero = true) {
    const size_t bytes = sizeof(T) * std::max<size_t>(count, 1);
    DevPtr<void> q;
    HIP_TRY(dev_malloc(q, bytes));
    if (zero) {
        HIP_TRY(hipMemsetAsync(q.get(), 0, bytes, nullptr));
        HIP_TRY(hipStreamSynchronize(nullptr));
    }
    *p = static_cast<T*>(q.get());
    c->dev_mem.push_back(std::move(q));
    c->device_bytes += bytes;
    return SVO_OK;
}

inline bool converts(int format) { return format != SVO_INPUT_GRAY_PAIR && format != SVO_INPUT_SBS_GRAY; }

constexpr int MAX_KEYFRAMES = 4096;

template <typename Tile, typename Launch>
TileTable<Tile, Launch> group_tile_table(svo_group* c, const char* env, Launch run) {
    return {reinterpret_cast<Tile*>(c->args.host.get()), reinterpret_cast<Tile*>(c->args.dev),
            table_tiles(env, c->args.bytes / sizeof(Tile)), c->stream.get(), run};
}

size_t align_up(size_t v, size_t a);
void dev_release(svo_group* c, void* p, size_t bytes);
int acquire_set(svo_group* c, Seq& q, ImageSet** out);
void release_set(Seq& q, ImageSet*& s);
int take_kf_slab(svo_group* c, KpsDev* out);
void fill_kf_record(const svo_group* c, const Seq& q, int id, const KfHost& k, KfDev& d);
void flush_one(Seq& q);
void flush_pending(svo_group* c);
void end_sequence(svo_group* c, int s);
void trim_keyframes(svo_group* c, Seq& q, int below);
int check_settings(const svo_camera_settings* cam, int width, int height, int n_sequences);
int keypoint_capacity(const svo_camera_settings& cam, int width, int height);
int usable_lk_levels(const svo_camera_settings& cam, int width, int height);
}
```

### stereo-svo-slam_amd/csrc/svo_group_step.hip

```cpp
#include <hip/hip_runtime.h>

#include <algorithm>
#include <chrono>
#include <cstring>
#include <vector>

#include "svo_group_state.hpp"

using namespace svo;

namespace {

struct Step {
    const uint8_t* const* left;
    const uint8_t* const* right;
    int stride, mem;
    const float* time_stamps;
    std::vector<int> act;
    std::vector<int> trk;
    std::vector<int> start;
    std::vector<int> need;
    int pyr_stream = -1;
    struct Remap { const uint8_t* map[2]; RemapImg left, right; };
    std::vector<Remap> remap;
    bool remap_shared = true, remap_single = false;
    int remap_chunks = 0;
    bool copy_right = false;
    float stage_ms[8] = {0, 0, 0, 0, 0, 0, 0, 0};
    std::chrono::steady_clock::time_point t0, lap_start;
};

hipError_t mark(svo_group* c, int i) {
    return c->timing ? hipEventRecord(c->ev[i].get(), c->stream.get()) : hipSuccess;
}

void lap(svo_group* c, Step& s, int phase) {
    const auto now = std::chrono::steady_clock::now();
    c->host_ms[phase] += std::chrono::duration<double, std::milli>(now - s.lap_start).count();
    s.lap_start = now;
}

int select_sequences(svo_group* c, Step& s) {
    s.act.reserve(c->B);
    s.trk.reserve(c->B);
    s.start.assign(c->B, 0);
    s.need.assign(c->B, 0);
    const bool one_buffer = c->fmt->buffers == 1;
    for (int q = 0; q < c->B; q++)
        if (s.left[q] && (one_buffer || s.right[q])) {
            s.act.push_back(q);
            if (c->seqs[q].frame_id < 0) s.start[q] = 1;
            else s.trk.push_back(q);
        } else if (!one_buffer && (s.left[q] != nullptr) != (s.right[q] != nullptr)) {
            return svo_set_error(SVO_ERR_INVALID, "svo_new_images: sequence %d has only one image", q);
        }
    return SVO_OK;
}

int stage_host_frames(svo_group* c, const Step& s) {
    const int B = c->B;
    const size_t row_bytes = (size_t)ingest_row_pixels(*c->fmt, c->width) * c->fmt->channels;
    const size_t used = (size_t)(c->height - 1) * s.stride + row_bytes;
    const size_t fb = align_up((size_t)c->height * s.stride, 256);
    if (fb > c->stage_frame_bytes) {
        HIP_TRY(hipStreamSynchronize(c->stream.get()));
        const int rc = dev_alloc(c, &c->d_stage_in, fb * 2 * B);
        if (rc) return rc;
        c->stage_frame_bytes = fb;
    }
    const size_t spacing = (size_t)c->height * s.stride;
    for (int side = 0; side < c->fmt->buffers; side++) {
        const uint8_t* const* src = side ? s.right : s.left;
        int s0 = 0;
        while (s0 < B) {
            if (!src[s0]) { s0++; continue; }
            int s1 = s0 + 1;
            while (s1 < B && src[s1] && src[s1] == src[s1 - 1] + spacing) s1++;
            uint8_t* dst = c->d_stage_in + (size_t)(side * B + s0) * c->stage_frame_bytes;
            if (s1 - s0 > 1) {
                HIP_TRY(hipMemcpy2DAsync(dst, c->stage_frame_bytes, src[s0], spacing, spacing, s1 - s0,
                                         hipMemcpyHostToDevice, c->stream.get()));
            } else {
                HIP_TRY(hipMemcpyAsync(dst, src[s0], used, hipMemcpyHostToDevice, c->stream.get()));
            }
            s0 = s1;
        }
    }
    return SVO_OK;
}

void slot_maps(const svo_group* c, const Seq& q, const uint8_t* maps[2]) {
    for (int side = 0; side < 2; side++)
        maps[side] = q.rig ? q.rig_maps[side] : c->rect ? reinterpret_cast<const uint8_t*>(c->rect[side].xy) : nullptr;
}

void pack_remap(svo_group* c, Step& s) {
    const int R = (int)s.remap.size();
    for (const Step::Remap& r : s.remap)
        s.remap_shared = s.remap_shared && r.map[0] == s.remap[0].map[0] && r.map[1] == s.remap[0].map[1];
    std::vector<int> order((size_t)R);
    for (int k = 0; k < R; k++) order[k] = k;
    if (!s.remap_shared) {
        std::vector<const uint8_t*> rigs;
        for (const Step::Remap& r : s.remap) rigs.push_back(r.map[0]);
        std::sort(rigs.begin(), rigs.end());
        rigs.erase(std::unique(rigs.begin(), rigs.end()), rigs.end());
        std::vector<int> map_of((size_t)R);
        for (int k = 0; k < R; k++) map_of[k] = (int)(std::lower_bound(rigs.begin(), rigs.end(), s.remap[k].map[0]) - rigs.begin());
        std::vector<RemapChunkSpan> spans;
        s.remap_single = remap_chunks(map_of.data(), R, order, spans) == 1;
        s.remap_chunks = (int)spans.size();
        for (int k = 0; k < s.remap_chunks; k++) {
            const Step::Remap& r = s.remap[order[spans[k].first]];
            c->args.remap_chunk.h[k] = RemapChunk{{r.map[0], r.map[1]}, spans[k].first, spans[k].count};
        }
    }
    for (int k = 0; k < R; k++) {
        c->remap_img.h[k] = s.remap[order[k]].left;
        c->remap_img.h[R + k] = s.remap[order[k]].right;
    }
}

int pack_pyramids(svo_group* c, Step& s) {
    bool any_rect = false;
    for (int seq : s.act) {
        const uint8_t* maps[2];
        slot_maps(c, c->seqs[seq], maps);
        any_rect = any_rect || maps[0] != nullptr;
    }
    if (converts(c->input_format) && any_rect && !c->d_raw_gray) {
        c->raw_plane_bytes = align_up(align_up((size_t)c->width, 64) * c->height, 256);
        const int rc = dev_alloc(c, &c->d_raw_gray, c->raw_plane_bytes * 2 * c->B, false);
        if (rc) return rc;
    }
    for (int j = 0; j < (int)s.act.size(); j++) {
        const int seq = s.act[j];
        Seq& q = c->seqs[seq];
        release_set(q, q.prev_set);
        q.prev_set = q.cur_set;
        const int rc = acquire_set(c, q, &q.cur_set);
        if (rc) return rc;
        ImageSet* is = q.cur_set;
        PyrArgs& hs = clear(c->args.pyr.h[j]);
        hs.n_levels = c->cam.max_pyramid_levels;
        const bool host = s.mem == SVO_MEM_HOST;
        const uint8_t* buf[2];
        buf[0] = host ? c->d_stage_in + (size_t)seq * c->stage_frame_bytes : s.left[seq];
        buf[1] = c->fmt->buffers == 1 ? buf[0] : host ? c->d_stage_in + (size_t)(c->B + seq) * c->stage_frame_bytes : s.right[seq];
        const uint8_t* src_l = buf[c->fmt->left.buffer] + (size_t)c->fmt->left.start * c->width;
        const uint8_t* src_r = buf[c->fmt->right.buffer] + (size_t)c->fmt->right.start * c->width;
        const int M = (int)s.act.size();
        const uint8_t* maps[2];
        slot_maps(c, q, maps);
        const bool rect = maps[0] != nullptr;
        if (converts(c->input_format)) {
            is->left[0] = is->own_left0;
            is->right = is->own_right;
            ImgView gray_l = is->own_left0, gray_r = is->own_right;
            if (rect) {
                const int pitch = (int)align_up((size_t)c->width, 64);
                gray_l = ImgView{c->d_raw_gray + (size_t)seq * c->raw_plane_bytes, c->width, c->height, pitch};
                gray_r = ImgView{c->d_raw_gray + (size_t)(c->B + seq) * c->raw_plane_bytes, c->width, c->height, pitch};
                s.remap.push_back({{maps[0], maps[1]}, RemapImg{gray_l, is->own_left0}, RemapImg{gray_r, is->own_right}});
            }
            c->ingest_img.h[j] = ingest_image(*c->fmt, 0, buf[c->fmt->left.buffer], s.stride, gray_l);
            c->ingest_img.h[M + j] = ingest_image(*c->fmt, 1, buf[c->fmt->right.buffer], s.stride, gray_r);
            hs.src_left = is->left[0];
        } else if (rect) {
            is->left[0] = is->own_left0;
            is->right = is->own_right;
            s.remap.push_back({{maps[0], maps[1]}, RemapImg{ImgView{src_l, c->width, c->height, s.stride}, is->own_left0},
                               RemapImg{ImgView{src_r, c->width, c->height, s.stride}, is->own_right}});
            hs.src_left = is->left[0];
        } else if (s.mem == SVO_MEM_DEVICE_BORROW) {
            is->left[0] = ImgView{src_l, c->width, c->height, s.stride};
            is->right = ImgView{src_r, c->width, c->height, s.stride};
            hs.src_left = is->left[0];
        } else {
            is->left[0] = is->own_left0;
            is->right = is->own_right;
            hs.src_left = ImgView{src_l, c->width, c->height, s.stride};
            hs.src_right = ImgView{src_r, c->width, c->height, s.stride};
            hs.dst_right = is->right;
            s.copy_right = true;
        }
        is->lk[0] = is->left[0];
        for (int l = 0; l < hs.n_levels; l++) hs.level[l] = is->left[l];
        hs.n_lk = c->n_lk;
        for (int l = 0; l < c->n_lk; l++) hs.lk[l] = is->lk[l];
        const int rows = pyr_stream_rows(hs);
        s.pyr_stream = (s.pyr_stream == 0 || rows == 0) ? 0 : std::max(s.pyr_stream, rows);
    }
    if (!s.remap.empty()) pack_remap(c, s);
    return SVO_OK;
}

CompactArgs& pack_compact(svo_group* c, Seq& q, int slot, int mode) {
    CompactArgs& ca = clear(c->args.compact.h[slot]);
    ca.src = q.kps[q.cur]; ca.dst = q.kps[q.cur ^ 1]; ca.mode = mode;
    q.cur ^= 1;
    return ca;
}

void pack_ssd(svo_group* c, const Seq& q, int slot, int clamp_half, const int* first_ptr) {
    SsdArgs& sa = clear(c->args.ssd.h[slot]);
    const KpsDev& k = q.kps[q.cur];
    sa.left = q.cur_set->left[0]; sa.right = q.cur_set->right;
    sa.n_ptr = k.n; sa.kps2d = k.kps2d; sa.disparity = q.disparity;
    sa.win = c->cam.window_size_depth_calculator; sa.search_x = c->cam.search_x;
    sa.search_y = c->cam.search_y; sa.clamp_half = clamp_half;
    sa.first = 0; sa.first_ptr = first_ptr;
}

void pack_tracking_args(svo_group* c, const Step& st) {
    ArgBlocks& a = c->args;
    for (int slot = 0; slot < (int)st.trk.size(); slot++) {
        const int s = st.trk[slot];
        Seq& q = c->seqs[s];
        FrameResult* dr = c->d_res + s;
        for (int i = 0; i < 6; i++) a.guess.h[s][i] = q.pending ? q.kf.statePost[i] : q.kf.statePre[i];
        pack_compact(c, q, slot, 0).min_kf = &dr->min_kf;
        const KpsDev& k = q.kps[q.cur];
        SiaArgs& sa = clear(a.sia.h[slot]);
        for (int l = 0; l < c->cam.max_pyramid_levels; l++) {
            sa.prev[l] = q.prev_set->left[l];
            sa.cur[l] = q.cur_set->left[l];
        }
        sa.cam = q.cam; sa.n_ptr = k.n; sa.kps2d = k.kps2d; sa.kps3d = k.kps3d; sa.flags = k.flags;
        sa.pose_guess = a.guess.d[s]; sa.pose_out = dr->pose_sia; sa.cost_out = &dr->sia_cost;
        sa.trace = dr->sia_trace; sa.kp_ws = q.sia_kpws;
        sa.rec_ws = q.sia_rec; sa.rec_cap = c->rec_cap;
        sa.mats_out = q.sia_mats;
        sa.dbg_H = nullptr; sa.dbg_level = -1; sa.cap = c->cap; sa.exact_pinv = c->exact_pinv;
        KltArgs& ka = clear(a.klt.h[slot]);
        ka.kfs = q.d_kfs; ka.kf_mask = c->max_kf - 1; ka.kf_id = k.kf_id; ka.n_cur = c->n_lk;
        for (int l = 0; l < c->n_lk; l++) ka.cur[l] = q.cur_set->lk[l];
        ka.n_ptr = k.n; ka.prev_pts = nullptr; ka.cur_pts = q.tracked; ka.status = q.klt_status;
        ka.err = q.klt_err; ka.win = c->cam.window_size_opt_flow;
        ka.proj_pose = dr->pose_sia; ka.proj_mats = q.sia_mats; ka.kps3d = k.kps3d; ka.proj_out = k.kps2d;
        ka.kp_index = k.kp_index; ka.ref_out = nullptr; ka.cam = q.cam;
        ReprojArgs& ra = clear(a.reproj.h[slot]);
        ra.cam = q.cam; ra.n_ptr = k.n; ra.kps2d = k.kps2d; ra.kps3d = k.kps3d; ra.flags = k.flags;
        ra.tracked = q.tracked; ra.err = q.klt_err; ra.pose_in = dr->pose_sia;
        ra.pose_out = dr->pose_refined; ra.cost_out = &dr->reproj_cost; ra.trace = &dr->reproj_trace;
        ra.exact_pinv = c->exact_pinv;
        ra.zero_out = c->d_inside + s;
        pack_ssd(c, q, slot, 1, nullptr);
        FilterArgs& fa = clear(a.filter.h[slot]);
        fa.cam = q.cam; fa.n_ptr = k.n; fa.frame_pose = dr->pose_refined;
        fa.kps2d = k.kps2d; fa.kps3d = k.kps3d; fa.flags = k.flags;
        fa.outlier_count = k.outl; fa.inlier_count = k.inl; fa.kf_inv_depth = k.kfx;
        fa.kf_variance = k.kfP; fa.disparity = q.disparity;
        fa.kfs = q.d_kfs; fa.kf_mask = c->max_kf - 1; fa.kf_id = k.kf_id; fa.kp_index = k.kp_index;
        fa.do_outlier_check = 1; fa.do_update = 1; fa.do_flags = 1; fa.do_reproject = 1;
        fa.width = c->width; fa.height = c->height; fa.inside_count = c->d_inside + s;
    }
}

void count_launch(svo_group* c, int kernel, const LaunchShape& sh) {
    for (svo_launch_shape& e : c->launch_shapes)
        if (e.kernel == kernel && e.waves == sh.waves && e.mode == sh.mode && e.cap == sh.cap) {
            e.launches++;
            return;
        }
    c->launch_shapes.push_back({kernel, sh.waves, sh.mode, sh.cap, 1});
}

int launch_tracking(svo_group* c, const Step& s) {
    const ArgBlocks& a = c->args;
    hipStream_t st = c->stream.get();
    const int M = (int)s.act.size(), T = (int)s.trk.size();
    HIP_TRY(hipMemcpyAsync(a.dev, a.host.get(), s.remap_chunks ? a.frame_rig_bytes : a.frame_bytes, hipMemcpyHostToDevice, st));
    const bool ingest = converts(c->input_format);
    if (ingest) {
        HIP_TRY(hipMemcpyAsync(c->ingest_img.d, c->ingest_img.h, sizeof(IngestImg) * 2 * M, hipMemcpyHostToDevice, st));
        for (int i0 = 0; i0 < 2 * M; i0 += 32768) {
            launch_ingest(c->ingest_img.d + i0, std::min(32768, 2 * M - i0), c->width, c->height, st);
            HIP_TRY(hipGetLastError());
        }
    }
    if (const int R = (int)s.remap.size()) {
        HIP_TRY(hipMemcpyAsync(c->remap_img.d, c->remap_img.h, sizeof(RemapImg) * 2 * R, hipMemcpyHostToDevice, st));
        if (s.remap_shared) {
            RemapLaunch ra;
            for (int side = 0; side < 2; side++)
                ra.map[side] = remap_map_view(const_cast<uint8_t*>(s.remap[0].map[side]), c->width, c->height);
            ra.img = c->remap_img.d; ra.n = R;
            launch_remap(ra, 2, st);
        } else {
            RemapMultiLaunch ra;
            clear(ra);
            ra.chunks = a.remap_chunk.d; ra.img = c->remap_img.d; ra.n = R;
            launch_remap_multi(ra, c->width, c->height, s.remap_chunks, s.remap_single, 2, st);
        }
        HIP_TRY(hipGetLastError());
    }
    launch_pyr_fused(a.pyr.d, M, c->width, c->height, s.copy_right, std::max(s.pyr_stream, 0), st);
    HIP_TRY(hipGetLastError());
    HIP_TRY(mark(c, 1));
    if (T == 0) {
        for (int i = 2; i <= 7; i++) HIP_TRY(mark(c, i));
        return SVO_OK;
    }
    launch_compact(a.compact.d, T, c->cap, st);
    HIP_TRY(hipGetLastError());
    HIP_TRY(mark(c, 2));
    int grid_n = 1;
    for (int seq : s.trk) grid_n = std::max(grid_n, c->seqs[seq].n_host);
    grid_n = std::min(grid_n, c->cap);
    const LaunchStatus sia_launch =
        launch_sia(a.sia.d, T, c->cam, c->width, c->height, grid_n, c->rec_cap, c->exact_pinv, st);
    HIP_TRY(sia_launch.err);
    if (!sia_launch.shape.fits)
        return svo_set_error(SVO_ERR_CAPACITY, "sparse alignment: %d keypoints exceed the workspaces", grid_n);
    count_launch(c, SVO_KERNEL_SIA_GN, sia_launch.shape);
    HIP_TRY(hipGetLastError());
    HIP_TRY(mark(c, 3));
    launch_klt(a.klt.d, T, grid_n, c->cam.window_size_opt_flow, st);
    HIP_TRY(hipGetLastError());
    HIP_TRY(mark(c, 4));
    const LaunchStatus reproj_launch = launch_reproj(a.reproj.d, T, grid_n, st);
    HIP_TRY(reproj_launch.err);
    if (!reproj_launch.shape.fits)
        return svo_set_error(SVO_ERR_CAPACITY, "reprojection GN: %d keypoints do not fit LDS", grid_n);
    count_launch(c, SVO_KERNEL_REPROJ_GN, reproj_launch.shape);
    HIP_TRY(hipGetLastError());
    HIP_TRY(mark(c, 5));
    launch_ssd(a.ssd.d, T, grid_n, c->cam.window_size_depth_calculator, c->cam.search_y, st);
    HIP_TRY(hipGetLastError());
    HIP_TRY(mark(c, 6));
    launch_filter(a.filter.d, T, grid_n, st);
    HIP_TRY(hipGetLastError());
    HIP_TRY(mark(c, 7));
    HIP_TRY(hipMemcpyAsync(c->h_inside, c->d_inside, sizeof(int) * c->B, hipMemcpyDeviceToHost, st));
    return SVO_OK;
}

int new_keyframe_storage(svo_group* c, Seq& q, int s, int id) {
    if (id - q.kfs.first() >= c->max_kf)
        return svo_set_error(SVO_ERR_CAPACITY, "more than %d resident keyframes (svo_trim_keyframes makes room)", c->max_kf);
    KfHost k{};
    if (const int rc = take_kf_slab(c, &k.kps)) return rc;
    k.set = q.cur_set;
    q.cur_set->refs++;
    q.kfs.push_back(k);
    fill_kf_record(c, q, id, k, c->args.kf_record.h[s]);
    return SVO_OK;
}

int pack_keyframe_args(svo_group* c, int slot, int s, bool first_frame) {
    ArgBlocks& a = c->args;
    Seq& q = c->seqs[s];
    FrameResult* dr = c->d_res + s;
    const int id = (int)q.kfs.size();
    const int rc = new_keyframe_storage(c, q, s, id);
    if (rc) return rc;
    CompactArgs& ca = pack_compact(c, q, slot, 1);
    ca.width = c->width; ca.height = c->height;
    ca.zero = q.n_det; ca.zero_count = SVO_MAX_PYRAMID_LEVELS;
    if (first_frame) {
        ca.start = 1;
        ca.zero_res = reinterpret_cast<int*>(dr); ca.zero_res_count = (int)(sizeof(FrameResult) / sizeof(int));
    }
    DetectArgs& da = clear(a.detect.h[slot]);
    for (int l = 0; l < c->cam.max_pyramid_levels; l++) da.level[l] = q.cur_set->left[l];
    da.n_levels = c->det_levels; da.grid_w = c->cam.grid_width; da.grid_h = c->cam.grid_height;
    da.out = q.det; da.n_out = q.n_det; da.max_cells = c->max_cells;
    MergeArgs& ma = clear(a.merge.h[slot]);
    ma.cam = q.cam; ma.width = c->width; ma.height = c->height;
    ma.det = q.det; ma.n_det = q.n_det; ma.n_levels = c->det_levels; ma.max_cells = c->max_cells;
    ma.kps = q.kps[q.cur]; ma.cap = c->cap;
    ma.sel = q.sel; ma.sel_level = q.sel_level; ma.sel_cell = q.sel_cell; ma.occupied = q.occupied;
    ma.old_count = &dr->old_count; ma.overflow = &dr->overflow;
    pack_ssd(c, q, slot, 0, &dr->old_count);
    KfInitArgs& ia = clear(a.kf_init.h[slot]);
    ia.cam = q.cam; ia.kps = q.kps[q.cur]; ia.old_count = &dr->old_count;
    ia.disparity = q.disparity; ia.frame_pose = dr->pose_refined;
    ia.first_frame = first_frame ? 1 : 0; ia.new_kf_id = id; ia.kfs = q.d_kfs; ia.kf_mask = c->max_kf - 1;
    ia.color_lcg = q.color_lcg; ia.n_out = &dr->kf_n;
    ia.record = a.kf_record.h[s];
    ia.tmpl_valid_bytes = (int)c->tmpl_valid_bytes;
    ia.evict_id = (c->tmpl_kf > 0 && id - c->tmpl_kf >= q.kfs.first()) ? id - c->tmpl_kf : -1;
    return SVO_OK;
}

int enqueue_keyframes(svo_group* c, const Step& s) {
    const ArgBlocks& a = c->args;
    hipStream_t st = c->stream.get();
    int m = 0;
    for (int seq = 0; seq < c->B; seq++) {
        if (!s.need[seq]) continue;
        const int rc = pack_keyframe_args(c, m++, seq, s.start[seq] != 0);
        if (rc) return rc;
    }
    if (m == 0) return SVO_OK;
    HIP_TRY(hipMemcpyAsync(a.dev, a.host.get(), a.bytes, hipMemcpyHostToDevice, st));
    launch_compact(a.compact.d, m, c->cap, st);
    HIP_TRY(hipGetLastError());
    if (c->det_levels > 0) {
        launch_detect(a.detect.d, m, c->max_cells, c->det_levels, c->cam.grid_width, c->cam.grid_height, st);
        HIP_TRY(hipGetLastError());
    }
    launch_select_merge(a.merge.d, m, c->max_cells, st);
    HIP_TRY(hipGetLastError());
    launch_ssd(a.ssd.d, m, c->cap, c->cam.window_size_depth_calculator, c->cam.search_y, st);
    HIP_TRY(hipGetLastError());
    launch_kf_init(a.kf_init.d, m, st);
    HIP_TRY(hipGetLastError());
    return SVO_OK;
}

int decide_keyframes(svo_group* c, Step& s) {
    const int max_keypoints = (c->width / c->cam.grid_width) * (c->height / c->cam.grid_height);
    bool any = false;
    for (int seq : s.act) {
        s.need[seq] = s.start[seq] || (double)c->h_inside[seq] < 0.66 * max_keypoints ? 1 : 0;
        any = any || s.need[seq];
    }
    return any ? enqueue_keyframes(c, s) : SVO_OK;
}

int read_stage_times(svo_group* c, Step& s) {
    HIP_TRY(mark(c, 8));
    if (!c->timing) return SVO_OK;
    HIP_TRY(hipEventSynchronize(c->ev[8].get()));
    for (int i = 0; i < 8; i++) (void)hipEventElapsedTime(&s.stage_ms[i], c->ev[i].get(), c->ev[i + 1].get());
    return SVO_OK;
}

void retire_keyframe_images(svo_group* c, const Step& s) {
    for (int seq : s.trk) {
        Seq& q = c->seqs[seq];
        const FrameResult& r = c->h_res[seq];
        const int newest = (int)q.kfs.size() - 1;
        for (; q.kfs_retired < std::min(r.min_kf, newest); q.kfs_retired++) release_set(q, q.kfs[q.kfs_retired].set);
        for (int i = 0; i < 64 && r.min_kf < newest && r.min_kf + i < newest; i++) {
            KfHost& old = q.kfs[r.min_kf + i];
            if (old.set && !((r.live_kf[i >> 5] >> (i & 31)) & 1u)) release_set(q, old.set);
        }
    }
}

int book_frame(svo_group* c, Step& s) {
    int overflow_seq = -1;
    for (int seq : s.act) {
        Seq& q = c->seqs[seq];
        const FrameResult& r = c->h_res[seq];
        const double ts = (double)s.time_stamps[seq];
        const bool first = s.start[seq] != 0;
        q.frame_id++;
        if (first) {
            std::memset(q.pose, 0, sizeof(q.pose));
            q.ts = ts;
            q.trajectory.push_back(svo_pose{});
        } else {
            q.pending = true;
            std::memcpy(q.pending_pose, r.pose_refined, sizeof(q.pending_pose));
            q.pending_ts = ts;
        }
        if (s.need[seq]) {
            KfHost& k = q.kfs.back();
            k.n = r.kf_n;
            if (first) std::memset(k.pose, 0, sizeof(k.pose));
            else std::memcpy(k.pose, r.pose_refined, sizeof(k.pose));
        }
        q.n_host = c->h_n[2 * seq + q.cur];
        svo_frame_stats& st = clear(q.stats);
        st.frame_id = q.frame_id; st.is_keyframe = s.need[seq]; st.n_keypoints = q.n_host;
        st.n_keyframes = (int)q.kfs.size(); st.inside_count = first ? 0 : c->h_inside[seq]; st.overflow = r.overflow;
        std::memcpy(st.pose_sia, r.pose_sia, sizeof(st.pose_sia));
        std::memcpy(st.pose_refined, r.pose_refined, sizeof(st.pose_refined));
        st.sia_cost = r.sia_cost; st.reproj_cost = r.reproj_cost; st.sia_ms = s.stage_ms[2];
        std::memcpy(st.stage_ms, s.stage_ms, sizeof(s.stage_ms));
        std::memcpy(st.sia_trace, r.sia_trace, sizeof(st.sia_trace));
        st.reproj_trace = r.reproj_trace;
        c->totals.frames++;
        c->totals.keyframes += s.need[seq];
        c->totals.keypoints += q.n_host;
        if (!first)
            for (int l = 0; l < SVO_MAX_PYRAMID_LEVELS; l++) {
                c->totals.gn_gradient_calls += r.sia_trace[l].n_gradient;
                c->totals.gn_cost_calls += r.sia_trace[l].n_cost;
            }
        if (r.overflow && overflow_seq < 0) overflow_seq = seq;
    }
    lap(c, s, 6);
    c->host_steps++;
    c->totals.launches++;
    for (int i = 0; i < 8; i++) c->totals.stage_ms[i] += s.stage_ms[i];
    c->totals.wall_ms += std::chrono::duration<double, std::milli>(std::chrono::steady_clock::now() - s.t0).count();
    if (overflow_seq >= 0)
        return svo_set_error(SVO_ERR_CAPACITY, "sequence %d: more than %d keypoints", overflow_seq, c->cap);
    return SVO_OK;
}

int step(svo_group* c, Step& s) {
    HIP_TRY(hipSetDevice(c->device));
    s.t0 = s.lap_start = std::chrono::steady_clock::now();
    int rc = select_sequences(c, s);
    if (rc || s.act.empty()) return rc;
    HIP_TRY(mark(c, 0));
    if (s.mem == SVO_MEM_HOST && (rc = stage_host_frames(c, s))) return rc;
    if ((rc = pack_pyramids(c, s))) return rc;
    pack_tracking_args(c, s);
    lap(c, s, 0);
    if ((rc = launch_tracking(c, s))) return rc;
    lap(c, s, 1);
    flush_pending(c);
    lap(c, s, 2);
    if (!s.trk.empty()) HIP_TRY(hipStreamSynchronize(c->stream.get()));
    lap(c, s, 3);
    if ((rc = decide_keyframes(c, s))) return rc;
    lap(c, s, 4);
    HIP_TRY(hipMemcpyAsync(c->h_res, c->d_res, c->readback_bytes, hipMemcpyDeviceToHost, c->stream.get()));
    HIP_TRY(hipStreamSynchronize(c->stream.get()));
    lap(c, s, 5);
    if ((rc = read_stage_times(c, s))) return rc;
    if (c->retire_kf_images) retire_keyframe_images(c, s);
    if (c->kf_window >= 0)
        for (int seq : s.trk) {
            Seq& q = c->seqs[seq];
            if (q.kfs_retired - q.kfs.first() > c->kf_window) trim_keyframes(c, q, q.kfs_retired - c->kf_window);
        }
    return book_frame(c, s);
}

}

int grp_new_images(svo_group* c, const uint8_t* const* left, const uint8_t* const* right, int stride,
                   const float* time_stamps, int mem) {
    if (!c || !left || (!right && c->fmt->buffers == 2) || !time_stamps ||
        (long long)stride < (long long)ingest_row_pixels(*c->fmt, c->width) * c->fmt->channels)
        return svo_set_error(SVO_ERR_INVALID, "svo_new_images: bad arguments");
    if (c->failed)
        return svo_set_error(SVO_ERR_INVALID, "svo_new_images: an earlier frame of this ctx failed; create a new ctx");
    Step s;
    s.left = left; s.right = right; s.stride = stride; s.mem = mem; s.time_stamps = time_stamps;
    const int rc = step(c, s);
    if (rc != SVO_OK) c->failed = true;
    return rc;
}
```

### stereo-svo-slam_amd/stereo_svo_slam_amd/hip_lib.py

```python
import ctypes as C
import os

import numpy as np
import torch

_HERE = os.path.dirname(os.path.abspath(__file__))
CSRC = os.path.normpath(os.path.join(_HERE, "..", "csrc"))
LIB_PATH = os.environ.get("SVO_HIP_LIB", os.path.join(CSRC, "libsvo_hip.so"))
_LIB = None

SYMBOLS = (
    "svo_last_error", "svo_version", "svo_handle_create", "svo_handle_destroy",
    "svo_handle_set_stream", "svo_handle_synchronize", "svo_build_pyramid",
    "svo_build_lk_pyramid", "svo_sparse_align", "svo_klt_track", "svo_reproj_gn",
    "svo_ssd_disparity", "svo_depth_filter_update",
    "svo_ctx_create", "svo_ctx_destroy", "svo_new_images", "svo_submit_images", "svo_wait",
    "svo_ctx_get_groups", "svo_new_image", "svo_get_pose",
    "svo_get_frame_keypoints", "svo_get_keyframe_count", "svo_get_keyframe",
    "svo_get_trajectory", "svo_update_pose", "svo_get_frame_stats", "svo_ctx_enable_timing",
    "svo_get_totals", "svo_handle_set_exact_pinv", "svo_ctx_set_exact_pinv",
    "svo_handle_set_fast_solver", "svo_ctx_set_fast_solver",
    "svo_device_malloc", "svo_device_free", "svo_copy_to_device", "svo_copy_to_host",
    "svo_copy_image_to_device", "svo_project_keypoints",
    "svo_ctx_get_launch_shapes", "svo_pick_launch_shapes", "svo_pick_sia_lds_bytes", "svo_pinv6_check",
    "svo_solve6_check", "svo_remap_linear", "svo_ctx_set_rectification",
    "svo_detect_keypoints", "svo_detect_shape",
    "svo_ctx_restart_sequences", "svo_get_finished_runs", "svo_get_finished_run",
    "svo_drop_finished_runs", "svo_ctx_get_memory",
    "svo_input_format_info", "svo_convert_frames", "svo_ctx_set_input_format",
    "svo_export_capacity", "svo_submit_export", "svo_export", "svo_pack_keypoints",
    "svo_snapshot_size", "svo_submit_save", "svo_save_sequences", "svo_submit_load", "svo_load_sequences",
    "svo_snapshot_info", "svo_copy_segments",
    "svo_reproj_gn_batch", "svo_filter_update_batch", "svo_sparse_align_batch",
    "svo_submit_pose_updates", "svo_update_poses", "svo_pose_filter_batch",
    "svo_map_size", "svo_submit_export_map", "svo_export_map", "svo_pack_map_points",
    "svo_view_size", "svo_submit_export_views", "svo_export_views", "svo_render_views",
    "svo_scene_size", "svo_scene_look_at", "svo_scene_frustum", "svo_submit_export_scenes", "svo_export_scenes",
    "svo_render_scene",
    "svo_remap_linear_multi", "svo_ctx_add_rigs", "svo_ctx_remove_rigs", "svo_ctx_assign_rigs", "svo_ctx_get_slot_rig",
    "svo_ctx_get_rigs",
    "svo_klt_track_batch", "svo_klt_cache_layout",
    "svo_rectify_inverse", "svo_build_rectify_maps", "svo_ctx_add_rigs_calibrated", "svo_ctx_set_calibration",
    "svo_submit_trim_keyframes", "svo_trim_keyframes", "svo_ctx_set_keyframe_window", "svo_get_keyframe_range",
)

INPUT_GRAY_PAIR, INPUT_BGR_PAIR, INPUT_RGB_PAIR, INPUT_SBS_GRAY, INPUT_SBS_BGR, INPUT_SBS_RGB, INPUT_CH3_ECON = range(7)
INPUT_FORMATS = ("gray_pair", "bgr_pair", "rgb_pair", "sbs_gray", "sbs_bgr", "sbs_rgb", "ch3_econ")
INGEST_COPY, INGEST_GRAY = 0, 1
EXPORT_FRAMES, EXPORT_LAST_KEYFRAMES = 0, 1
EXPORT_WHAT = ("frames", "last_keyframes")
MEM_HOST, MEM_DEVICE = 0, 1


class SvoError(RuntimeError):
    pass


class CameraSettings(C.Structure):
    _fields_ = [(n, C.c_float) for n in
                ("baseline", "fx", "fy", "cx", "cy", "k1", "k2", "k3", "p1", "p2")] + \
               [(n, C.c_int32) for n in
                ("grid_height", "grid_width", "search_x", "search_y",
                 "window_size_pose_estimator", "window_size_opt_flow",
                 "window_size_depth_calculator", "max_pyramid_levels",
                 "min_pyramid_level_pose_estimation")]

    @classmethod
    def from_dict(cls, d):
        cam = cls()
        for name, _ in cls._fields_:
            setattr(cam, name, d[name])
        return cam


RIG_FLOATS = ("baseline", "fx", "fy", "cx", "cy", "k1", "k2", "k3", "p1", "p2")


class Rig(C.Structure):
    _fields_ = [(n, C.c_float) for n in RIG_FLOATS] + \
               [(n, C.c_void_p) for n in ("left_map_x", "left_map_y", "right_map_x", "right_map_y")] + \
               [("mem", C.c_int32), ("_reserved", C.c_int32)]

    @classmethod
    def from_dict(cls, d):
        get = d.__getitem__ if isinstance(d, dict) else lambda n: getattr(d, n)
        return cls(**{n: get(n) for n in RIG_FLOATS})


assert C.sizeof(Rig) == 80


class CameraCalibration(C.Structure):
    _fields_ = [("K", C.c_double * 9), ("D", C.c_double * 8), ("R", C.c_double * 9), ("P", C.c_double * 9)]

    @classmethod
    def from_mats(cls, K, D, R, P):
        K, P = np.asarray(K, np.float64), np.asarray(P, np.float64)
        D = np.asarray(D, np.float64).ravel()
        R = np.eye(3) if R is None else np.asarray(R, np.float64)
        if K.shape != (3, 3) or R.shape != (3, 3) or P.shape not in ((3, 3), (3, 4)):
            raise ValueError(f"K, R are 3x3 and P is 3x3 or 3x4, not {K.shape}, {R.shape}, {P.shape}")
        if D.size not in (4, 5, 8):
            raise ValueError(f"D has 4, 5 or 8 coefficients, not {D.size}")
        cal = cls()
        cal.K[:] = K.ravel().tolist()
        cal.D[:] = D.tolist() + [0.0] * (8 - D.size)
        cal.R[:] = R.ravel().tolist()
        cal.P[:] = P[:, :3].ravel().tolist()
        return cal


assert C.sizeof(CameraCalibration) == 280


class Image(C.Structure):
    _fields_ = [("data", C.c_void_p), ("width", C.c_int32), ("height", C.c_int32),
                ("stride", C.c_int32)]


class KltKeyframe(C.Structure):
    _fields_ = [("lk", Image * 3), ("n_lk", C.c_int32), ("n_kps", C.c_int32), ("kps2d", C.c_void_p),
                ("tmpl", C.c_void_p), ("tmpl_valid", C.c_void_p), ("tmpl_bytes", C.c_int64),
                ("tmpl_valid_bytes", C.c_int64), ("tmpl_cap", C.c_int32), ("tmpl_win", C.c_int32)]


class KltSequence(C.Structure):
    _fields_ = [("kfs", C.POINTER(KltKeyframe)), ("n_kfs", C.c_int32), ("n_cur", C.c_int32), ("cur", Image * 3),
                ("n", C.c_void_p), ("kf_id", C.c_void_p), ("kp_index", C.c_void_p), ("kps3d", C.c_void_p),
                ("pose", C.c_void_p), ("cam", CameraSettings)] + \
               [(n, C.c_void_p) for n in ("tracked", "status", "err", "proj_out", "ref_out")]


assert (C.sizeof(KltKeyframe), C.sizeof(KltSequence)) == (128, 248)


class InputSide(C.Structure):
    _fields_ = [("buffer", C.c_int32), ("start_column", C.c_int32), ("op", C.c_int32), ("channel", C.c_int32),
                ("weight", C.c_int32 * 3)]


class InputLayout(C.Structure):
    _fields_ = [("buffers", C.c_int32), ("channels", C.c_int32), ("min_row_pixels", C.c_int32),
                ("left", InputSide), ("right", InputSide)]


GN_TRACE_DTYPE = np.dtype([("level", "<i4"), ("n_gradient", "<i4"), ("n_cost", "<i4"),
                           ("n_accepted", "<i4"), ("exit_small", "<i4"),
                           ("initial_cost", "<f4"), ("final_cost", "<f4"), ("pose", "<f4", (6,))])
assert GN_TRACE_DTYPE.itemsize == 52


DET_CELL_DTYPE = np.dtype([("x", "<f4"), ("y", "<f4"), ("score", "<f4"), ("type", "<i4")])
assert DET_CELL_DTYPE.itemsize == 16


EXPORT_SEGMENT_DTYPE = np.dtype([("seq", "<i4"), ("run", "<i4"), ("frame_id", "<i4"), ("keyframe_id", "<i4"),
                                 ("is_keyframe", "<i4"), ("n", "<i4"), ("first", "<i8"), ("pose", "<f4", (6,)),
                                 ("time_stamp", "<f4"), ("_pad", "<i4")])
assert EXPORT_SEGMENT_DTYPE.itemsize == 64


class ExportDst(C.Structure):
    _fields_ = [("segments", C.c_void_p), ("kps2d", C.c_void_p), ("kps3d", C.c_void_p), ("info", C.c_void_p),
                ("capacity", C.c_int64)]


MAP_POINT_DTYPE = np.dtype([("x", "<f4"), ("y", "<f4"), ("z", "<f4"), ("color", "u1", (3,)), ("flags", "u1")])
MAP_KEYFRAME_DTYPE = np.dtype([("id", "<i4"), ("n_total", "<i4"), ("n", "<i4"), ("_pad", "<i4"), ("first", "<i8"),
                               ("pose", "<f4", (6,))])
MAP_SEGMENT_DTYPE = np.dtype([("seq", "<i4"), ("run", "<i4"), ("frame_id", "<i4"), ("status", "<i4"),
                              ("n_keyframes", "<i4"), ("keyframes_retired", "<i4"), ("from_keyframe", "<i4"),
                              ("n_exported", "<i4"), ("n_points", "<i8"), ("points_bound", "<i8"),
                              ("time_stamp", "<f4"), ("_pad", "<i4", (3,))])
MAP_REGION_DTYPE = np.dtype([("first_point", "<i8"), ("point_capacity", "<i8"), ("first_keyframe_entry", "<i8"),
                             ("keyframe_capacity", "<i4"), ("from_keyframe", "<i4")])
assert (MAP_POINT_DTYPE.itemsize, MAP_KEYFRAME_DTYPE.itemsize, MAP_SEGMENT_DTYPE.itemsize,
        MAP_REGION_DTYPE.itemsize) == (16, 48, 64, 32)
MAP_COMPLETE, MAP_TOO_SMALL = 0, 1


def map_first_keyframe(segment):
    return int(segment["_pad"][0])
IGNORE_DURING_REFINEMENT, IGNORE_COMPLETELY, IGNORE_TEMPORARY = 1, 2, 4


class MapFilter(C.Structure):
    _fields_ = [("drop_flags", C.c_uint32), ("own_only", C.c_int32), ("min_inliers", C.c_int32),
                ("_reserved", C.c_int32)]


class MapDst(C.Structure):
    _fields_ = [("segments", C.c_void_p), ("keyframes", C.c_void_p), ("points", C.c_void_p)]


def map_filter(f):
    if f is None:
        return MapFilter()
    return f if isinstance(f, MapFilter) else MapFilter(**f)


PLANE_LEFT, PLANE_RIGHT = 0, 1
PLANES = ("left", "right")
PIXEL_GRAY8, PIXEL_RGB8, PIXEL_RGBA8 = 0, 1, 2
PIXELS = ("gray8", "rgb8", "rgba8")
PIXEL_BYTES = (1, 3, 4)
VIEW_OK, VIEW_NONE = 0, 1
VIEW_SEGMENT_DTYPE = np.dtype([("seq", "<i4"), ("run", "<i4"), ("frame_id", "<i4"), ("keyframe_id", "<i4"),
                               ("status", "<i4"), ("n", "<i4"), ("offset", "<i8"), ("pose", "<f4", (6,)),
                               ("time_stamp", "<f4"), ("_pad", "<i4")])
assert VIEW_SEGMENT_DTYPE.itemsize == 64


class ViewStyle(C.Structure):
    _fields_ = [("plane", C.c_int32), ("level", C.c_int32), ("pixel", C.c_int32), ("markers", C.c_int32),
                ("drop_flags", C.c_uint32), ("size", C.c_int32), ("size_temporary", C.c_int32),
                ("_reserved", C.c_int32)]


class ViewDst(C.Structure):
    _fields_ = [("segments", C.c_void_p), ("pixels", C.c_void_p), ("capacity", C.c_int64)]


def view_style(what=EXPORT_FRAMES, plane=PLANE_LEFT, level=0, pixel=PIXEL_GRAY8, markers=False, drop_flags=None,
               size=None, size_temporary=None):
    if isinstance(plane, str):
        plane = PLANES.index(plane)
    if isinstance(pixel, str):
        pixel = PIXELS.index(pixel)
    frames = int(what) == EXPORT_FRAMES
    return ViewStyle(int(plane), int(level), int(pixel), int(bool(markers)),
                     (IGNORE_COMPLETELY if frames else 0) if drop_flags is None else int(drop_flags),
                     (20 if frames else 10) if size is None else int(size),
                     10 if size_temporary is None else int(size_temporary), 0)


def view_size(cam, width, height, style):
    cols, rows, pitch, nbytes = C.c_int(0), C.c_int(0), C.c_int64(0), C.c_int64(0)
    _check(lib().svo_view_size(C.byref(cam), int(width), int(height), C.byref(style), C.byref(cols), C.byref(rows),
                               C.byref(pitch), C.byref(nbytes)))
    return cols.value, rows.value, pitch.value, nbytes.value


class Keypoints(C.Structure):
    _fields_ = [("n", C.c_int32)] + [(name, C.c_void_p) for name in (
        "kps2d", "kps3d", "flags", "keyframe_id", "keypoint_index", "outlier_count", "inlier_count",
        "kf_inv_depth", "kf_variance", "score", "level_type", "color")]


class ViewSrc(C.Structure):
    _fields_ = [("image", Image), ("kps", Keypoints)]


SCENE_POINTS, SCENE_TRAJECTORY, SCENE_KEYFRAMES, SCENE_POSE = 1, 2, 4, 8
SCENE_ALL = 15
SCENE_CLASS_POSE, SCENE_CLASS_KEYFRAME, SCENE_CLASS_TRAJECTORY, SCENE_CLASS_POINT = range(4)
SCENE_OK, SCENE_NONE = 0, 1
SCENE_LINE_DTYPE = np.dtype([("a", "<f4", (3,)), ("b", "<f4", (3,)), ("cls_rgb", "<u4"), ("_pad", "<u4")])
SCENE_SEGMENT_DTYPE = np.dtype([("seq", "<i4"), ("run", "<i4"), ("frame_id", "<i4"), ("status", "<u2"),
                                ("n_keyframes", "<u2"), ("from_keyframe", "<i4"), ("n_keypoints", "<i4"),
                                ("n_poses", "<i4"), ("time_stamp", "<f4"), ("offset", "<i8"), ("pose", "<f4", (6,))])
assert (SCENE_LINE_DTYPE.itemsize, SCENE_SEGMENT_DTYPE.itemsize) == (32, 64)
SCENE_FRONT = ((0.0, 0.0, -1.0), (0.0, 0.0, 0.0), (0.0, -1.0, 0.0))
SCENE_TOP = ((0.0, -5.0, 0.0), (0.0, 0.0, 0.0), (0.0, 0.0, 1.0))
SCENE_SIDE = ((-5.0, 0.0, 0.0), (0.0, 0.0, 0.0), (0.0, -1.0, 0.0))
SCENE_PRESETS = dict(front=SCENE_FRONT, top=SCENE_TOP, side=SCENE_SIDE)
SCENE_FOV_Y, SCENE_NEAR = 45.0, 0.1


class SceneCamera(C.Structure):
    _fields_ = [("view", C.c_float * 12), ("f", C.c_float), ("cx", C.c_float), ("cy", C.c_float), ("near", C.c_float)]


class SceneStyle(C.Structure):
    _fields_ = [("cols", C.c_int32), ("rows", C.c_int32), ("pixel", C.c_int32), ("point_size", C.c_int32),
                ("background", C.c_uint32), ("trajectory_rgb", C.c_uint32), ("keyframe_rgb", C.c_uint32),
                ("pose_rgb", C.c_uint32), ("frustum_w", C.c_float), ("frustum_h", C.c_float), ("frustum_d", C.c_float),
                ("show", C.c_uint32), ("from_keyframe", C.c_int32), ("trajectory_tail", C.c_int32),
                ("filter", MapFilter), ("_reserved", C.c_int32)]


class SceneDst(C.Structure):
    _fields_ = [("segments", C.c_void_p), ("pixels", C.c_void_p), ("capacity", C.c_int64)]


class SceneSrc(C.Structure):
    _fields_ = [("cols", C.c_int32), ("rows", C.c_int32), ("n_sets", C.c_int32), ("n_lines", C.c_int32),
                ("sets", C.c_void_p), ("own_id", C.c_void_p), ("lines", C.c_void_p)]


assert (C.sizeof(SceneCamera), C.sizeof(SceneStyle)) == (64, 76)


def scene_style(cols=256, rows=256, pixel=PIXEL_RGB8, point_size=3, background=0xffffff, trajectory_rgb=0xff0000,
                keyframe_rgb=0x0000ff, pose_rgb=0x00ff00, frustum=(0.1, 0.08, 0.07), show=SCENE_ALL, from_keyframe=0,
                trajectory_tail=0, filter=None):
    if isinstance(pixel, str):
        pixel = PIXELS.index(pixel)
    return SceneStyle(int(cols), int(rows), int(pixel), int(point_size), int(background), int(trajectory_rgb),
                      int(keyframe_rgb), int(pose_rgb), float(frustum[0]), float(frustum[1]), float(frustum[2]),
                      int(show), int(from_keyframe), int(trajectory_tail), map_filter(filter), 0)


def scene_size(style):
    pitch, nbytes = C.c_int64(0), C.c_int64(0)
    _check(lib().svo_scene_size(C.byref(style), C.byref(pitch), C.byref(nbytes)))
    return pitch.value, nbytes.value


def scene_look_at(eye, centre, up, fov_y_deg=SCENE_FOV_Y, cols=256, rows=256, near=SCENE_NEAR):
    v3 = lambda v: (C.c_float * 3)(*[float(x) for x in v])
    out = SceneCamera()
    _check(lib().svo_scene_look_at(v3(eye), v3(centre), v3(up), float(fov_y_deg), int(cols), int(rows), float(near),
                                   C.byref(out)))
    return out


def scene_preset(name, cols=256, rows=256):
    return scene_look_at(*SCENE_PRESETS[name], SCENE_FOV_Y, cols, rows, SCENE_NEAR)

# ... 487 lines not shown
```

Baseline: 281,900.

## Prefetch next frame's pyramids and defer stats booking across steps

Adds a lookahead path: the worker peeks at its job queue and, when the next job is a frame set, builds that frame's image pyramids into a second double-buffered arg block while the current step is still waiting on tracking results. Stats booking can also be deferred to overlap with the next step, and the stream syncs become event syncs. The cost targeted is the GPU idling during host-side keyframe decision and readback. Both prefetch and late booking default to off (compile macros set to 0, env overrides), so the main visible default change is the restructured arg blocks, packed keyframe upload and event-based sync. The extra state management and settle calls add complexity and a risk of stale image sets.

```diff
diff --git a/include/svo_hip.h b/include/svo_hip.h
--- a/include/svo_hip.h
+++ b/include/svo_hip.h
@@ -128,6 +128,8 @@
 int svo_submit_images(svo_ctx *ctx, const uint8_t *const *left, const uint8_t *const *right,
                       int stride, const float *time_stamps, int mem);
 int svo_wait(svo_ctx *ctx);
+enum { SVO_NEXT_NONE = 0, SVO_NEXT_FRAMES = 1, SVO_NEXT_RESTART = 2, SVO_NEXT_LOAD = 3, SVO_NEXT_RIGS = 4, SVO_NEXT_JOB = 5 };
+int svo_step_prefetch_allowed(int next_entry, int ctx_failed, int has_left, int has_right, int one_buffer);
 int svo_ctx_get_groups(svo_ctx *ctx, int *n_groups);
 int svo_ctx_restart_sequences(svo_ctx *ctx, const int *seqs, int n);
 typedef struct svo_run_info {
diff --git a/stereo-svo-slam_amd/csrc/svo_ctx.hip b/stereo-svo-slam_amd/csrc/svo_ctx.hip
--- a/stereo-svo-slam_amd/csrc/svo_ctx.hip
+++ b/stereo-svo-slam_amd/csrc/svo_ctx.hip
@@ -111,8 +111,30 @@
 
 void worker_submit(svo_ctx::Worker& w, svo_ctx::Job&& job);
 
+bool is_frame_set(const svo_ctx::Job& j) {
+    return j.scene.seqs.empty() && j.view.seqs.empty() && j.map.seqs.empty() && j.pose.seqs.empty() && j.snap.loads.empty() &&
+           j.snap.seqs.empty() && j.exp.seqs.empty() && j.assign.empty() && j.trim.empty() && j.restart.empty();
+}
+
+GroupNext worker_peek(void* queue) {
+    svo_ctx::Worker& w = *static_cast<svo_ctx::Worker*>(queue);
+    GroupNext n{GRP_NEXT_NONE, nullptr, nullptr, 0, 0};
+    if (w.ctx_failed->load()) return n;
+    std::lock_guard<std::mutex> lk(w.m);
+    if (w.jobs.empty()) return n;
+    const svo_ctx::Job& j = w.jobs.front();
+    if (is_frame_set(j)) n = GroupNext{GRP_NEXT_FRAMES, j.left.data(), j.right.empty() ? nullptr : j.right.data(), j.stride, j.mem};
+    else n.kind = !j.restart.empty() ? GRP_NEXT_RESTART : !j.snap.loads.empty() ? GRP_NEXT_LOAD : !j.assign.empty() ? GRP_NEXT_RIGS : GRP_NEXT_JOB;
+    return n;
+}
+
 void worker_run_job(svo_ctx::Worker& w, const svo_ctx::Job& job) {
-    if (w.err != SVO_OK || w.ctx_failed->load()) return;
+    if (w.err != SVO_OK || w.ctx_failed->load()) {
+        grp_settle(w.g.get());
+        return;
+    }
+    const bool frames = is_frame_set(job);
+    if (!frames) grp_settle(w.g.get());
     const svo_ctx::Export& e = job.exp;
     const svo_ctx::Snapshots& sn = job.snap;
     const svo_ctx::PoseUpdates& pu = job.pose;
@@ -140,7 +162,7 @@
                    : !job.restart.empty()
                        ? grp_restart_sequences(w.g.get(), job.restart.data(), (int)job.restart.size())
                        : grp_new_images(w.g.get(), job.left.data(), job.right.empty() ? nullptr : job.right.data(), job.stride,
-                                        job.ts.data(), job.mem);
+                                        job.ts.data(), job.mem, w.th.joinable() ? worker_peek : nullptr, &w);
     if (rc != SVO_OK) {
         w.err = rc;
         w.msg = svo_last_error();
@@ -695,6 +717,10 @@
     return SVO_OK;
 }
 
+extern "C" int svo_step_prefetch_allowed(int next_entry, int ctx_failed, int has_left, int has_right, int one_buffer) {
+    return grp_prefetch_allowed(next_entry, ctx_failed != 0, has_left != 0, has_right != 0, one_buffer != 0) ? 1 : 0;
+}
+
 extern "C" int svo_wait(svo_ctx* c) {
     if (!c) return svo_set_error(SVO_ERR_INVALID, "svo_wait: bad ctx");
     return ctx_drain(c);
diff --git a/stereo-svo-slam_amd/csrc/svo_group.hip b/stereo-svo-slam_amd/csrc/svo_group.hip
--- a/stereo-svo-slam_amd/csrc/svo_group.hip
+++ b/stereo-svo-slam_amd/csrc/svo_group.hip
@@ -19,7 +19,7 @@
         static const char* names[7] = {"args", "launch", "pose_filter", "wait_frame", "kf_enqueue", "wait_kf", "bookkeeping"};
         std::fprintf(stderr, "[svo host ms/step over %ld steps]", c->host_steps);
         for (int i = 0; i < 7; i++) std::fprintf(stderr, " %s=%.3f", names[i], c->host_ms[i] / c->host_steps);
-        std::fprintf(stderr, "\n");
+        std::fprintf(stderr, " pyramids_ahead=%ld\n", c->ahead_steps);
     }
     delete c;
 }
@@ -214,6 +214,8 @@
         if (t >= 4 && t <= MAX_KEYFRAMES && (t & (t - 1)) == 0) c->max_kf = t;
     }
     if (const char* e = std::getenv("SVO_KEEP_KEYFRAME_IMAGES")) c->retire_kf_images = std::atoi(e) == 0;
+    if (const char* e = std::getenv("SVO_STEP_PREFETCH")) c->prefetch = std::atoi(e) != 0;
+    if (const char* e = std::getenv("SVO_LATE_BOOKING")) c->late_booking = std::atoi(e) != 0;
     c->n_lk = usable_lk_levels(cam, width, height);
     c->det_levels = cam.max_pyramid_levels / 2;
     c->max_cells = 1;
@@ -235,9 +237,10 @@
     auto size = [&](auto& arr) { off += align_up(sizeof(typename std::decay_t<decltype(arr)>::type) * B, 256); };
     a.frame_arrays(size);
     a.frame_bytes = off;
-    a.rig_arrays(size);
-    a.frame_rig_bytes = off;
+    a.kf_off = off;
     a.keyframe_arrays(size);
+    const size_t record_off = off;
+    size(a.kf_record);
     a.bytes = off;
     HIP_TRY(pinned_malloc(a.host, a.bytes));
     std::memset(a.host.get(), 0, a.bytes);
@@ -251,8 +254,25 @@
         off += align_up(sizeof(T) * B, 256);
     };
     a.frame_arrays(place);
-    a.rig_arrays(place);
     a.keyframe_arrays(place);
+    off = record_off;
+    place(a.kf_record);
+
+    for (PyrBlocks& pb : c->pyr_args) {
+        pb.pyr_bytes = align_up(sizeof(PyrArgs) * B, 256);
+        pb.chunk_bytes = pb.pyr_bytes + align_up(sizeof(RemapChunk) * B, 256);
+        const size_t bytes = pb.chunk_bytes + align_up(sizeof(RemapImg) * 2 * B, 256);
+        HIP_TRY(pinned_malloc(pb.host, bytes));
+        std::memset(pb.host.get(), 0, bytes);
+        uint8_t* dev = nullptr;
+        if ((rc = dev_alloc(c, &dev, bytes))) return rc;
+        pb.pyr = {reinterpret_cast<PyrArgs*>(pb.host.get()), reinterpret_cast<PyrArgs*>(dev)};
+        pb.remap_chunk = {reinterpret_cast<RemapChunk*>(pb.host.get() + pb.pyr_bytes), reinterpret_cast<RemapChunk*>(dev + pb.pyr_bytes)};
+        pb.remap_img = {reinterpret_cast<RemapImg*>(pb.host.get() + pb.chunk_bytes), reinterpret_cast<RemapImg*>(dev + pb.chunk_bytes)};
+        for (Event& e : pb.ev) HIP_TRY(make_event(e));
+    }
+    HIP_TRY(make_event(c->ev_inside));
+    HIP_TRY(make_event(c->ev_res));
 
     const size_t res_bytes = sizeof(FrameResult) * B, n_bytes = sizeof(int) * 2 * B, in_bytes = sizeof(int) * B;
     c->readback_bytes = res_bytes + n_bytes;
@@ -312,15 +332,17 @@
     return SVO_OK;
 }
 
-template <typename T>
-static int alloc_mirrored_table(svo_group* c, ArgArray<T>& table, PinnedPtr<T>& host, size_t n) {
-    PinnedPtr<T> pinned;
-    HIP_TRY(pinned_malloc(pinned, sizeof(T) * n));
-    T* dev = nullptr;
-    if (const int rc = dev_alloc(c, &dev, n)) return rc;
-    host = std::move(pinned);
-    table.h = host.get();
-    table.d = dev;
+static int alloc_ingest_tables(svo_group* c) {
+    const size_t bytes = sizeof(IngestImg) * 2 * (size_t)c->B;
+    PinnedPtr<uint8_t> pinned[2];
+    for (PinnedPtr<uint8_t>& p : pinned) HIP_TRY(pinned_malloc(p, bytes));
+    uint8_t* dev = nullptr;
+    if (const int rc = dev_alloc(c, &dev, 2 * bytes)) return rc;
+    for (int i = 0; i < 2; i++) {
+        PyrBlocks& pb = c->pyr_args[i];
+        pb.ingest_host = std::move(pinned[i]);
+        pb.ingest_img = {reinterpret_cast<IngestImg*>(pb.ingest_host.get()), reinterpret_cast<IngestImg*>(dev + i * bytes)};
+    }
     return SVO_OK;
 }
 
@@ -351,20 +373,23 @@
         if ((rc = alloc_sequence(c, c->seqs[s], s))) return rc;
     if ((rc = grow_kf_slabs(c, std::max(2 * n_sequences, 32)))) return rc;
     if ((rc = alloc_template_cache(c))) return rc;
-    if ((rc = alloc_mirrored_table(c, c->remap_img, c->remap_img_host, 2 * (size_t)n_sequences))) return rc;
     HIP_TRY(hipDeviceSynchronize());
     *out = std::move(g);
     return SVO_OK;
 }
 
 void grp_set_exact_pinv(svo_group* c, int on) { c->exact_pinv = on != 0; }
-void grp_set_rectification(svo_group* c, const RemapMap* maps) { c->rect = maps; }
+void grp_set_rectification(svo_group* c, const RemapMap* maps) {
+    grp_settle(c);
+    c->rect = maps;
+}
 void grp_enable_timing(svo_group* c, int on) { c->timing = on != 0; }
 
 int grp_set_input_format(svo_group* c, int format) {
-    if (converts(format) && !c->ingest_img.d) {
+    grp_settle(c);
+    if (converts(format) && !c->pyr_args[0].ingest_img.d) {
         HIP_TRY(hipSetDevice(c->device));
-        if (const int rc = alloc_mirrored_table(c, c->ingest_img, c->ingest_img_host, 2 * (size_t)c->B)) return rc;
+        if (const int rc = alloc_ingest_tables(c)) return rc;
     }
     c->input_format = format;
     c->fmt = ingest_format(format);
diff --git a/stereo-svo-slam_amd/csrc/svo_group.hpp b/stereo-svo-slam_amd/csrc/svo_group.hpp
--- a/stereo-svo-slam_amd/csrc/svo_group.hpp
+++ b/stereo-svo-slam_amd/csrc/svo_group.hpp
@@ -12,8 +12,18 @@
 using Group = std::unique_ptr<svo_group, GroupDelete>;
 
 int grp_create(const svo_camera_settings* cam, int width, int height, int n_sequences, int device, Group* out);
+enum { GRP_NEXT_NONE = 0, GRP_NEXT_FRAMES = 1, GRP_NEXT_RESTART = 2, GRP_NEXT_LOAD = 3, GRP_NEXT_RIGS = 4, GRP_NEXT_JOB = 5 };
+struct GroupNext {
+    int kind;
+    const uint8_t* const* left;
+    const uint8_t* const* right;
+    int stride, mem;
+};
+using GroupPeek = GroupNext (*)(void* queue);
 int grp_new_images(svo_group* g, const uint8_t* const* left, const uint8_t* const* right, int stride,
-                   const float* time_stamps, int mem);
+                   const float* time_stamps, int mem, GroupPeek peek = nullptr, void* queue = nullptr);
+bool grp_prefetch_allowed(int next_kind, bool failed, bool has_left, bool has_right, bool one_buffer);
+void grp_settle(svo_group* g);
 int grp_restart_sequences(svo_group* g, const int* seqs, int n);
 int grp_trim_keyframes(svo_group* g, const int* seqs, const int* below, int n);
 void grp_set_keyframe_window(svo_group* g, int keep);
diff --git a/stereo-svo-slam_amd/csrc/svo_group_state.hpp b/stereo-svo-slam_amd/csrc/svo_group_state.hpp
--- a/stereo-svo-slam_amd/csrc/svo_group_state.hpp
+++ b/stereo-svo-slam_amd/csrc/svo_group_state.hpp
@@ -13,6 +13,17 @@
 #include "svo_group.hpp"
 #include "svo_host.hpp"
 #include "svo_tracker.hpp"
+
+#ifndef SVO_STEP_PREFETCH
+#define SVO_STEP_PREFETCH 0
+#endif
+#ifndef SVO_KF_PACKED_UPLOAD
+#define SVO_KF_PACKED_UPLOAD 1
+#endif
+#ifndef SVO_LATE_BOOKING
+#define SVO_LATE_BOOKING 0
+#endif
+
 namespace svo {
 
 struct PoseFilter {
@@ -183,6 +194,7 @@
     std::vector<ImageSet*> free_sets;
     ImageSet* cur_set = nullptr;
     ImageSet* prev_set = nullptr;
+    ImageSet* next_set = nullptr;
     int rig = 0;
     svo_camera_settings cam{};
     const uint8_t* rig_maps[2] = {nullptr, nullptr};
@@ -212,7 +224,6 @@
 };
 
 struct ArgBlocks {
-    ArgArray<PyrArgs> pyr;
     ArgArray<CompactArgs> compact;
     ArgArray<SiaArgs> sia;
     ArgArray<KltArgs> klt;
@@ -220,18 +231,43 @@
     ArgArray<SsdArgs> ssd;
     ArgArray<FilterArgs> filter;
     ArgArray<float[8]> guess;
-    ArgArray<RemapChunk> remap_chunk;
+    ArgArray<CompactArgs> kf_compact;
     ArgArray<DetectArgs> detect;
     ArgArray<MergeArgs> merge;
+    ArgArray<SsdArgs> kf_ssd;
     ArgArray<KfInitArgs> kf_init;
-    ArgArray<int> enable;
     ArgArray<KfDev> kf_record;
-    template <typename F> void frame_arrays(F f) { f(pyr); f(compact); f(sia); f(klt); f(reproj); f(ssd); f(filter); f(guess); }
-    template <typename F> void rig_arrays(F f) { f(remap_chunk); }
-    template <typename F> void keyframe_arrays(F f) { f(detect); f(merge); f(kf_init); f(enable); f(kf_record); }
+    template <typename F> void frame_arrays(F f) { f(compact); f(sia); f(klt); f(reproj); f(ssd); f(filter); f(guess); }
+    template <typename F> void keyframe_arrays(F f) { f(kf_compact); f(detect); f(merge); f(kf_ssd); f(kf_init); }
     PinnedPtr<uint8_t> host;
     uint8_t* dev = nullptr;
-    size_t frame_bytes = 0, frame_rig_bytes = 0, bytes = 0;
+    size_t frame_bytes = 0, kf_off = 0, bytes = 0;
+};
+
+struct PyrBlocks {
+    ArgArray<PyrArgs> pyr;
+    ArgArray<RemapChunk> remap_chunk;
+    ArgArray<RemapImg> remap_img;
+    ArgArray<IngestImg> ingest_img;
+    PinnedPtr<uint8_t> host, ingest_host;
+    size_t pyr_bytes = 0, chunk_bytes = 0;
+    Event ev[2];
+};
+
+struct PyrAhead {
+    bool valid = false;
+    const uint8_t* const* left = nullptr;
+    const uint8_t* const* right = nullptr;
+    int stride = 0, mem = 0, turn = 0;
+    std::vector<int> act;
+};
+
+struct LateBooking {
+    bool pending = false;
+    std::vector<int> act, start, need;
+    std::vector<int> inside;
+    float stage_ms[8] = {0, 0, 0, 0, 0, 0, 0, 0};
+    double wall_ms = 0;
 };
 
 }
@@ -243,6 +279,12 @@
     std::vector<svo::DevPtr<void>> dev_mem;
     std::vector<svo::Seq> seqs;
     svo::ArgBlocks args;
+    svo::PyrBlocks pyr_args[2];
+    int pyr_turn = 0;
+    svo::PyrAhead ahead;
+    svo::LateBooking late;
+    bool prefetch = SVO_STEP_PREFETCH != 0, late_booking = SVO_LATE_BOOKING != 0;
+    svo::Event ev_inside, ev_res;
     svo::PinnedPtr<uint8_t> readback_host;
     svo::FrameResult* d_res = nullptr; svo::FrameResult* h_res = nullptr;
     int* h_n = nullptr;
@@ -251,12 +293,8 @@
     size_t readback_bytes = 0;
     uint8_t* d_stage_in = nullptr; size_t stage_frame_bytes = 0;
     const svo::RemapMap* rect = nullptr;
-    svo::ArgArray<svo::RemapImg> remap_img;
-    svo::PinnedPtr<svo::RemapImg> remap_img_host;
     int input_format = SVO_INPUT_GRAY_PAIR;
     const svo::IngestFormat* fmt = nullptr;
-    svo::ArgArray<svo::IngestImg> ingest_img;
-    svo::PinnedPtr<svo::IngestImg> ingest_img_host;
     uint8_t* d_raw_gray = nullptr; size_t raw_plane_bytes = 0;
     uint8_t* d_export = nullptr;
     uint8_t* d_snap = nullptr; size_t snap_bytes = 0;
@@ -288,6 +326,7 @@
     int image_sets = 0;
     double host_ms[8] = {0, 0, 0, 0, 0, 0, 0, 0};
     long host_steps = 0;
+    long ahead_steps = 0;
 };
 
 namespace svo {
@@ -331,6 +370,8 @@
 void fill_kf_record(const svo_group* c, const Seq& q, int id, const KfHost& k, KfDev& d);
 void flush_one(Seq& q);
 void flush_pending(svo_group* c);
+void book_late(svo_group* c);
+void drop_ahead(svo_group* c);
 void end_sequence(svo_group* c, int s);
 void trim_keyframes(svo_group* c, Seq& q, int below);
 int check_settings(const svo_camera_settings* cam, int width, int height, int n_sequences);
diff --git a/stereo-svo-slam_amd/csrc/svo_group_step.hip b/stereo-svo-slam_amd/csrc/svo_group_step.hip
--- a/stereo-svo-slam_amd/csrc/svo_group_step.hip
+++ b/stereo-svo-slam_amd/csrc/svo_group_step.hip
@@ -3,6 +3,7 @@
 #include <algorithm>
 #include <chrono>
 #include <cstring>
+#include <type_traits>
 #include <vector>
 
 #include "svo_group_state.hpp"
@@ -28,6 +29,10 @@
     bool copy_right = false;
     float stage_ms[8] = {0, 0, 0, 0, 0, 0, 0, 0};
     std::chrono::steady_clock::time_point t0, lap_start;
+    GroupPeek peek = nullptr;
+    void* queue = nullptr;
+    PyrBlocks* pyr = nullptr;
+    PyrBlocks* ahead = nullptr;
 };
 
 hipError_t mark(svo_group* c, int i) {
@@ -94,7 +99,7 @@
         maps[side] = q.rig ? q.rig_maps[side] : c->rect ? reinterpret_cast<const uint8_t*>(c->rect[side].xy) : nullptr;
 }
 
-void pack_remap(svo_group* c, Step& s) {
+void pack_remap(PyrBlocks& pb, Step& s) {
     const int R = (int)s.remap.size();
     for (const Step::Remap& r : s.remap)
         s.remap_shared = s.remap_shared && r.map[0] == s.remap[0].map[0] && r.map[1] == s.remap[0].map[1];
@@ -112,16 +117,16 @@
         s.remap_chunks = (int)spans.size();
         for (int k = 0; k < s.remap_chunks; k++) {
             const Step::Remap& r = s.remap[order[spans[k].first]];
-            c->args.remap_chunk.h[k] = RemapChunk{{r.map[0], r.map[1]}, spans[k].first, spans[k].count};
+            pb.remap_chunk.h[k] = RemapChunk{{r.map[0], r.map[1]}, spans[k].first, spans[k].count};
         }
     }
     for (int k = 0; k < R; k++) {
-        c->remap_img.h[k] = s.remap[order[k]].left;
-        c->remap_img.h[R + k] = s.remap[order[k]].right;
-    }
-}
-
-int pack_pyramids(svo_group* c, Step& s) {
+        pb.remap_img.h[k] = s.remap[order[k]].left;
+        pb.remap_img.h[R + k] = s.remap[order[k]].right;
+    }
+}
+
+int pack_pyramids(svo_group* c, Step& s, PyrBlocks& pb, bool ahead) {
     bool any_rect = false;
     for (int seq : s.act) {
         const uint8_t* maps[2];
@@ -136,12 +141,14 @@
     for (int j = 0; j < (int)s.act.size(); j++) {
         const int seq = s.act[j];
         Seq& q = c->seqs[seq];
-        release_set(q, q.prev_set);
-        q.prev_set = q.cur_set;
-        const int rc = acquire_set(c, q, &q.cur_set);
+        if (!ahead) {
+            release_set(q, q.prev_set);
+            q.prev_set = q.cur_set;
+        }
+        const int rc = acquire_set(c, q, ahead ? &q.next_set : &q.cur_set);
         if (rc) return rc;
-        ImageSet* is = q.cur_set;
-        PyrArgs& hs = clear(c->args.pyr.h[j]);
+        ImageSet* is = ahead ? q.next_set : q.cur_set;
+        PyrArgs& hs = clear(pb.pyr.h[j]);
         hs.n_levels = c->cam.max_pyramid_levels;
         const bool host = s.mem == SVO_MEM_HOST;
         const uint8_t* buf[2];
@@ -163,8 +170,8 @@
                 gray_r = ImgView{c->d_raw_gray + (size_t)(c->B + seq) * c->raw_plane_bytes, c->width, c->height, pitch};
                 s.remap.push_back({{maps[0], maps[1]}, RemapImg{gray_l, is->own_left0}, RemapImg{gray_r, is->own_right}});
             }
-            c->ingest_img.h[j] = ingest_image(*c->fmt, 0, buf[c->fmt->left.buffer], s.stride, gray_l);
-            c->ingest_img.h[M + j] = ingest_image(*c->fmt, 1, buf[c->fmt->right.buffer], s.stride, gray_r);
+            pb.ingest_img.h[j] = ingest_image(*c->fmt, 0, buf[c->fmt->left.buffer], s.stride, gray_l);
+            pb.ingest_img.h[M + j] = ingest_image(*c->fmt, 1, buf[c->fmt->right.buffer], s.stride, gray_r);
             hs.src_left = is->left[0];
         } else if (rect) {
             is->left[0] = is->own_left0;
@@ -191,19 +198,52 @@
         const int rows = pyr_stream_rows(hs);
         s.pyr_stream = (s.pyr_stream == 0 || rows == 0) ? 0 : std::max(s.pyr_stream, rows);
     }
-    if (!s.remap.empty()) pack_remap(c, s);
-    return SVO_OK;
-}
-
-CompactArgs& pack_compact(svo_group* c, Seq& q, int slot, int mode) {
-    CompactArgs& ca = clear(c->args.compact.h[slot]);
+    if (!s.remap.empty()) pack_remap(pb, s);
+    return SVO_OK;
+}
+
+int launch_pyramids(svo_group* c, const Step& s, const PyrBlocks& pb) {
+    hipStream_t st = c->stream.get();
+    const int M = (int)s.act.size();
+    HIP_TRY(hipMemcpyAsync(pb.pyr.d, pb.pyr.h, s.remap_chunks ? pb.chunk_bytes : sizeof(PyrArgs) * M, hipMemcpyHostToDevice, st));
+    if (converts(c->input_format)) {
+        HIP_TRY(hipMemcpyAsync(pb.ingest_img.d, pb.ingest_img.h, sizeof(IngestImg) * 2 * M, hipMemcpyHostToDevice, st));
+        for (int i0 = 0; i0 < 2 * M; i0 += 32768) {
+            launch_ingest(pb.ingest_img.d + i0, std::min(32768, 2 * M - i0), c->width, c->height, st);
+            HIP_TRY(hipGetLastError());
+        }
+    }
+    if (const int R = (int)s.remap.size()) {
+        HIP_TRY(hipMemcpyAsync(pb.remap_img.d, pb.remap_img.h, sizeof(RemapImg) * 2 * R, hipMemcpyHostToDevice, st));
+        if (s.remap_shared) {
+            RemapLaunch ra;
+            for (int side = 0; side < 2; side++)
+                ra.map[side] = remap_map_view(const_cast<uint8_t*>(s.remap[0].map[side]), c->width, c->height);
+            ra.img = pb.remap_img.d; ra.n = R;
+            launch_remap(ra, 2, st);
+        } else {
+            RemapMultiLaunch ra;
+            clear(ra);
+            ra.chunks = pb.remap_chunk.d; ra.img = pb.remap_img.d; ra.n = R;
+            launch_remap_multi(ra, c->width, c->height, s.remap_chunks, s.remap_single, 2, st);
+        }
+        HIP_TRY(hipGetLastError());
+    }
+    launch_pyr_fused(pb.pyr.d, M, c->width, c->height, s.copy_right, std::max(s.pyr_stream, 0), st);
+    HIP_TRY(hipGetLastError());
+    if (c->timing) HIP_TRY(hipEventRecord(pb.ev[1].get(), st));
+    return SVO_OK;
+}
+
+CompactArgs& pack_compact(Seq& q, CompactArgs& args, int mode) {
+    CompactArgs& ca = clear(args);
     ca.src = q.kps[q.cur]; ca.dst = q.kps[q.cur ^ 1]; ca.mode = mode;
     q.cur ^= 1;
     return ca;
 }
 
-void pack_ssd(svo_group* c, const Seq& q, int slot, int clamp_half, const int* first_ptr) {
-    SsdArgs& sa = clear(c->args.ssd.h[slot]);
+void pack_ssd(svo_group* c, const Seq& q, SsdArgs& args, int clamp_half, const int* first_ptr) {
+    SsdArgs& sa = clear(args);
     const KpsDev& k = q.kps[q.cur];
     sa.left = q.cur_set->left[0]; sa.right = q.cur_set->right;
     sa.n_ptr = k.n; sa.kps2d = k.kps2d; sa.disparity = q.disparity;
@@ -219,7 +259,7 @@
         Seq& q = c->seqs[s];
         FrameResult* dr = c->d_res + s;
         for (int i = 0; i < 6; i++) a.guess.h[s][i] = q.pending ? q.kf.statePost[i] : q.kf.statePre[i];
-        pack_compact(c, q, slot, 0).min_kf = &dr->min_kf;
+        pack_compact(q, a.compact.h[slot], 0).min_kf = &dr->min_kf;
         const KpsDev& k = q.kps[q.cur];
         SiaArgs& sa = clear(a.sia.h[slot]);
         for (int l = 0; l < c->cam.max_pyramid_levels; l++) {
@@ -245,7 +285,7 @@
         ra.pose_out = dr->pose_refined; ra.cost_out = &dr->reproj_cost; ra.trace = &dr->reproj_trace;
         ra.exact_pinv = c->exact_pinv;
         ra.zero_out = c->d_inside + s;
-        pack_ssd(c, q, slot, 1, nullptr);
+        pack_ssd(c, q, a.ssd.h[slot], 1, nullptr);
         FilterArgs& fa = clear(a.filter.h[slot]);
         fa.cam = q.cam; fa.n_ptr = k.n; fa.frame_pose = dr->pose_refined;
         fa.kps2d = k.kps2d; fa.kps3d = k.kps3d; fa.flags = k.flags;
@@ -269,39 +309,13 @@
 int launch_tracking(svo_group* c, const Step& s) {
     const ArgBlocks& a = c->args;
     hipStream_t st = c->stream.get();
-    const int M = (int)s.act.size(), T = (int)s.trk.size();
-    HIP_TRY(hipMemcpyAsync(a.dev, a.host.get(), s.remap_chunks ? a.frame_rig_bytes : a.frame_bytes, hipMemcpyHostToDevice, st));
-    const bool ingest = converts(c->input_format);
-    if (ingest) {
-        HIP_TRY(hipMemcpyAsync(c->ingest_img.d, c->ingest_img.h, sizeof(IngestImg) * 2 * M, hipMemcpyHostToDevice, st));
-        for (int i0 = 0; i0 < 2 * M; i0 += 32768) {
-            launch_ingest(c->ingest_img.d + i0, std::min(32768, 2 * M - i0), c->width, c->height, st);
-            HIP_TRY(hipGetLastError());
-        }
-    }
-    if (const int R = (int)s.remap.size()) {
-        HIP_TRY(hipMemcpyAsync(c->remap_img.d, c->remap_img.h, sizeof(RemapImg) * 2 * R, hipMemcpyHostToDevice, st));
-        if (s.remap_shared) {
-            RemapLaunch ra;
-            for (int side = 0; side < 2; side++)
-                ra.map[side] = remap_map_view(const_cast<uint8_t*>(s.remap[0].map[side]), c->width, c->height);
-            ra.img = c->remap_img.d; ra.n = R;
-            launch_remap(ra, 2, st);
-        } else {
-            RemapMultiLaunch ra;
-            clear(ra);
-            ra.chunks = a.remap_chunk.d; ra.img = c->remap_img.d; ra.n = R;
-            launch_remap_multi(ra, c->width, c->height, s.remap_chunks, s.remap_single, 2, st);
-        }
-        HIP_TRY(hipGetLastError());
-    }
-    launch_pyr_fused(a.pyr.d, M, c->width, c->height, s.copy_right, std::max(s.pyr_stream, 0), st);
-    HIP_TRY(hipGetLastError());
+    const int T = (int)s.trk.size();
     HIP_TRY(mark(c, 1));
     if (T == 0) {
         for (int i = 2; i <= 7; i++) HIP_TRY(mark(c, i));
         return SVO_OK;
     }
+    HIP_TRY(hipMemcpyAsync(a.dev, a.host.get(), a.frame_bytes, hipMemcpyHostToDevice, st));
     launch_compact(a.compact.d, T, c->cap, st);
     HIP_TRY(hipGetLastError());
     HIP_TRY(mark(c, 2));
@@ -333,6 +347,7 @@
     HIP_TRY(hipGetLastError());
     HIP_TRY(mark(c, 7));
     HIP_TRY(hipMemcpyAsync(c->h_inside, c->d_inside, sizeof(int) * c->B, hipMemcpyDeviceToHost, st));
+    HIP_TRY(hipEventRecord(c->ev_inside.get(), st));
     return SVO_OK;
 }
 
@@ -355,7 +370,7 @@
     const int id = (int)q.kfs.size();
     const int rc = new_keyframe_storage(c, q, s, id);
     if (rc) return rc;
-    CompactArgs& ca = pack_compact(c, q, slot, 1);
+    CompactArgs& ca = pack_compact(q, a.kf_compact.h[slot], 1);
     ca.width = c->width; ca.height = c->height;
     ca.zero = q.n_det; ca.zero_count = SVO_MAX_PYRAMID_LEVELS;
     if (first_frame) {
@@ -372,7 +387,7 @@
     ma.kps = q.kps[q.cur]; ma.cap = c->cap;
     ma.sel = q.sel; ma.sel_level = q.sel_level; ma.sel_cell = q.sel_cell; ma.occupied = q.occupied;
     ma.old_count = &dr->old_count; ma.overflow = &dr->overflow;
-    pack_ssd(c, q, slot, 0, &dr->old_count);
+    pack_ssd(c, q, a.kf_ssd.h[slot], 0, &dr->old_count);
     KfInitArgs& ia = clear(a.kf_init.h[slot]);
     ia.cam = q.cam; ia.kps = q.kps[q.cur]; ia.old_count = &dr->old_count;
     ia.disparity = q.disparity; ia.frame_pose = dr->pose_refined;
@@ -384,18 +399,40 @@
     return SVO_OK;
 }
 
+size_t carve_keyframe_arrays(ArgBlocks& a, size_t m) {
+    size_t off = a.kf_off;
+    a.keyframe_arrays([&](auto& arr) {
+        using T = typename std::decay_t<decltype(arr)>::type;
+        arr.h = reinterpret_cast<T*>(a.host.get() + off);
+        arr.d = reinterpret_cast<T*>(a.dev + off);
+        off += align_up(sizeof(T) * m, 256);
+    });
+    return off - a.kf_off;
+}
+
 int enqueue_keyframes(svo_group* c, const Step& s) {
-    const ArgBlocks& a = c->args;
+    ArgBlocks& a = c->args;
     hipStream_t st = c->stream.get();
     int m = 0;
+    for (int seq = 0; seq < c->B; seq++) m += s.need[seq] ? 1 : 0;
+    if (m == 0) return SVO_OK;
+#if SVO_KF_PACKED_UPLOAD
+    const size_t packed = carve_keyframe_arrays(a, (size_t)m);
+#else
+    (void)carve_keyframe_arrays(a, (size_t)c->B);
+#endif
+    m = 0;
     for (int seq = 0; seq < c->B; seq++) {
         if (!s.need[seq]) continue;
         const int rc = pack_keyframe_args(c, m++, seq, s.start[seq] != 0);
         if (rc) return rc;
     }
-    if (m == 0) return SVO_OK;
+#if SVO_KF_PACKED_UPLOAD
+    HIP_TRY(hipMemcpyAsync(a.dev + a.kf_off, a.host.get() + a.kf_off, packed, hipMemcpyHostToDevice, st));
+#else
     HIP_TRY(hipMemcpyAsync(a.dev, a.host.get(), a.bytes, hipMemcpyHostToDevice, st));
-    launch_compact(a.compact.d, m, c->cap, st);
+#endif
+    launch_compact(a.kf_compact.d, m, c->cap, st);
     HIP_TRY(hipGetLastError());
     if (c->det_levels > 0) {
         launch_detect(a.detect.d, m, c->max_cells, c->det_levels, c->cam.grid_width, c->cam.grid_height, st);
@@ -403,7 +440,7 @@
     }
     launch_select_merge(a.merge.d, m, c->max_cells, st);
     HIP_TRY(hipGetLastError());
-    launch_ssd(a.ssd.d, m, c->cap, c->cam.window_size_depth_calculator, c->cam.search_y, st);
+    launch_ssd(a.kf_ssd.d, m, c->cap, c->cam.window_size_depth_calculator, c->cam.search_y, st);
     HIP_TRY(hipGetLastError());
     launch_kf_init(a.kf_init.d, m, st);
     HIP_TRY(hipGetLastError());
@@ -424,7 +461,14 @@
     HIP_TRY(mark(c, 8));
     if (!c->timing) return SVO_OK;
     HIP_TRY(hipEventSynchronize(c->ev[8].get()));
-    for (int i = 0; i < 8; i++) (void)hipEventElapsedTime(&s.stage_ms[i], c->ev[i].get(), c->ev[i + 1].get());
+    (void)hipEventElapsedTime(&s.stage_ms[0], s.pyr->ev[0].get(), s.pyr->ev[1].get());
+    for (int i = 1; i < 8; i++) (void)hipEventElapsedTime(&s.stage_ms[i], c->ev[i].get(), c->ev[i + 1].get());
+    if (s.ahead) {
+        float before = 0, after = 0;
+        (void)hipEventElapsedTime(&before, c->ev[7].get(), s.ahead->ev[0].get());
+        (void)hipEventElapsedTime(&after, s.ahead->ev[1].get(), c->ev[8].get());
+        s.stage_ms[7] = before + after;
+    }
     return SVO_OK;
 }
 
@@ -439,6 +483,36 @@
             if (old.set && !((r.live_kf[i >> 5] >> (i & 31)) & 1u)) release_set(q, old.set);
         }
     }
+}
+
+void book_stats(svo_group* c, const std::vector<int>& act, const std::vector<int>& start, const std::vector<int>& need,
+                const int* inside, const float stage_ms[8], double wall_ms) {
+    for (int seq : act) {
+        Seq& q = c->seqs[seq];
+        const FrameResult& r = c->h_res[seq];
+        const bool first = start[seq] != 0;
+        svo_frame_stats& st = clear(q.stats);
+        st.frame_id = q.frame_id; st.is_keyframe = need[seq]; st.n_keypoints = q.n_host;
+        st.n_keyframes = (int)q.kfs.size(); st.inside_count = first ? 0 : inside[seq]; st.overflow = r.overflow;
+        std::memcpy(st.pose_sia, r.pose_sia, sizeof(st.pose_sia));
+        std::memcpy(st.pose_refined, r.pose_refined, sizeof(st.pose_refined));
+        st.sia_cost = r.sia_cost; st.reproj_cost = r.reproj_cost; st.sia_ms = stage_ms[2];
+        std::memcpy(st.stage_ms, stage_ms, sizeof(st.stage_ms));
+        std::memcpy(st.sia_trace, r.sia_trace, sizeof(st.sia_trace));
+        st.reproj_trace = r.reproj_trace;
+        c->totals.frames++;
+        c->totals.keyframes += need[seq];
+        c->totals.keypoints += q.n_host;
+        if (!first)
+            for (int l = 0; l < SVO_MAX_PYRAMID_LEVELS; l++) {
+                c->totals.gn_gradient_calls += r.sia_trace[l].n_gradient;
+                c->totals.gn_cost_calls += r.sia_trace[l].n_cost;
+            }
+    }
+    c->host_steps++;
+    c->totals.launches++;
+    for (int i = 0; i < 8; i++) c->totals.stage_ms[i] += stage_ms[i];
+    c->totals.wall_ms += wall_ms;
 }
 
 int book_frame(svo_group* c, Step& s) {
@@ -465,32 +539,73 @@
             else std::memcpy(k.pose, r.pose_refined, sizeof(k.pose));
         }
         q.n_host = c->h_n[2 * seq + q.cur];
-        svo_frame_stats& st = clear(q.stats);
-        st.frame_id = q.frame_id; st.is_keyframe = s.need[seq]; st.n_keypoints = q.n_host;
-        st.n_keyframes = (int)q.kfs.size(); st.inside_count = first ? 0 : c->h_inside[seq]; st.overflow = r.overflow;
-        std::memcpy(st.pose_sia, r.pose_sia, sizeof(st.pose_sia));
-        std::memcpy(st.pose_refined, r.pose_refined, sizeof(st.pose_refined));
-        st.sia_cost = r.sia_cost; st.reproj_cost = r.reproj_cost; st.sia_ms = s.stage_ms[2];
-        std::memcpy(st.stage_ms, s.stage_ms, sizeof(s.stage_ms));
-        std::memcpy(st.sia_trace, r.sia_trace, sizeof(st.sia_trace));
-        st.reproj_trace = r.reproj_trace;
-        c->totals.frames++;
-        c->totals.keyframes += s.need[seq];
-        c->totals.keypoints += q.n_host;
-        if (!first)
-            for (int l = 0; l < SVO_MAX_PYRAMID_LEVELS; l++) {
-                c->totals.gn_gradient_calls += r.sia_trace[l].n_gradient;
-                c->totals.gn_cost_calls += r.sia_trace[l].n_cost;
-            }
         if (r.overflow && overflow_seq < 0) overflow_seq = seq;
     }
+    const double wall_ms = std::chrono::duration<double, std::milli>(std::chrono::steady_clock::now() - s.t0).count();
+    const bool later = c->late_booking && overflow_seq < 0 && s.peek && s.peek(s.queue).kind == GRP_NEXT_FRAMES;
+    if (later) {
+        LateBooking& b = c->late;
+        b.pending = true;
+        b.act = s.act; b.start = s.start; b.need = s.need;
+        b.inside.assign(c->h_inside, c->h_inside + c->B);
+        std::memcpy(b.stage_ms, s.stage_ms, sizeof(b.stage_ms));
+        b.wall_ms = wall_ms;
+    } else {
+        book_stats(c, s.act, s.start, s.need, c->h_inside, s.stage_ms, wall_ms);
+    }
     lap(c, s, 6);
-    c->host_steps++;
-    c->totals.launches++;
-    for (int i = 0; i < 8; i++) c->totals.stage_ms[i] += s.stage_ms[i];
-    c->totals.wall_ms += std::chrono::duration<double, std::milli>(std::chrono::steady_clock::now() - s.t0).count();
     if (overflow_seq >= 0)
         return svo_set_error(SVO_ERR_CAPACITY, "sequence %d: more than %d keypoints", overflow_seq, c->cap);
+    return SVO_OK;
+}
+
+bool adopt_ahead(svo_group* c, Step& s) {
+    PyrAhead& a = c->ahead;
+    if (!a.valid || a.left != s.left || a.right != s.right || a.stride != s.stride || a.mem != s.mem || a.act != s.act) return false;
+    for (int seq : s.act) {
+        Seq& q = c->seqs[seq];
+        release_set(q, q.prev_set);
+        q.prev_set = q.cur_set;
+        q.cur_set = q.next_set;
+        q.next_set = nullptr;
+    }
+    s.pyr = &c->pyr_args[a.turn];
+    a.valid = false;
+    c->ahead_steps++;
+    return true;
+}
+
+int take_pyr_block(svo_group* c, PyrBlocks** pb, int* turn) {
+    *turn = c->pyr_turn;
+    *pb = &c->pyr_args[c->pyr_turn];
+    c->pyr_turn ^= 1;
+    if (c->timing) HIP_TRY(hipEventRecord((*pb)->ev[0].get(), c->stream.get()));
+    return SVO_OK;
+}
+
+int launch_ahead(svo_group* c, Step& s) {
+    if (!c->prefetch || !s.peek) return SVO_OK;
+    const GroupNext n = s.peek(s.queue);
+    if (n.kind != GRP_NEXT_FRAMES || !n.left || (!n.right && c->fmt->buffers == 2) ||
+        (long long)n.stride < (long long)ingest_row_pixels(*c->fmt, c->width) * c->fmt->channels)
+        return SVO_OK;
+    Step a;
+    a.left = n.left; a.right = n.right; a.stride = n.stride; a.mem = n.mem;
+    const bool one_buffer = c->fmt->buffers == 1;
+    for (int q = 0; q < c->B; q++) {
+        const bool l = n.left[q] != nullptr, r = !one_buffer && n.right[q] != nullptr;
+        if (grp_prefetch_allowed(n.kind, c->failed, l, r, one_buffer)) a.act.push_back(q);
+        else if (!one_buffer && l != r) return SVO_OK;
+    }
+    if (a.act.empty()) return SVO_OK;
+    int rc, turn;
+    if ((rc = take_pyr_block(c, &s.ahead, &turn))) return rc;
+    if (a.mem == SVO_MEM_HOST && (rc = stage_host_frames(c, a))) return rc;
+    if ((rc = pack_pyramids(c, a, *s.ahead, true))) return rc;
+    if ((rc = launch_pyramids(c, a, *s.ahead))) return rc;
+    PyrAhead& h = c->ahead;
+    h.valid = true; h.left = n.left; h.right = n.right; h.stride = n.stride; h.mem = n.mem; h.turn = turn;
+    h.act = std::move(a.act);
     return SVO_OK;
 }
 
@@ -498,22 +613,35 @@
     HIP_TRY(hipSetDevice(c->device));
     s.t0 = s.lap_start = std::chrono::steady_clock::now();
     int rc = select_sequences(c, s);
-    if (rc || s.act.empty()) return rc;
-    HIP_TRY(mark(c, 0));
-    if (s.mem == SVO_MEM_HOST && (rc = stage_host_frames(c, s))) return rc;
-    if ((rc = pack_pyramids(c, s))) return rc;
+    if (rc || s.act.empty()) {
+        grp_settle(c);
+        return rc;
+    }
+    const bool adopted = adopt_ahead(c, s);
+    if (!adopted) {
+        drop_ahead(c);
+        int turn;
+        if ((rc = take_pyr_block(c, &s.pyr, &turn))) return rc;
+        if (s.mem == SVO_MEM_HOST && (rc = stage_host_frames(c, s))) return rc;
+        if ((rc = pack_pyramids(c, s, *s.pyr, false))) return rc;
+    }
     pack_tracking_args(c, s);
     lap(c, s, 0);
+    if (!adopted && (rc = launch_pyramids(c, s, *s.pyr))) return rc;
     if ((rc = launch_tracking(c, s))) return rc;
     lap(c, s, 1);
+    book_late(c);
     flush_pending(c);
     lap(c, s, 2);
-    if (!s.trk.empty()) HIP_TRY(hipStreamSynchronize(c->stream.get()));
+    if ((rc = launch_ahead(c, s))) return rc;
+    lap(c, s, 1);
+    if (!s.trk.empty()) HIP_TRY(hipEventSynchronize(c->ev_inside.get()));
     lap(c, s, 3);
     if ((rc = decide_keyframes(c, s))) return rc;
     lap(c, s, 4);
     HIP_TRY(hipMemcpyAsync(c->h_res, c->d_res, c->readback_bytes, hipMemcpyDeviceToHost, c->stream.get()));
-    HIP_TRY(hipStreamSynchronize(c->stream.get()));
+    HIP_TRY(hipEventRecord(c->ev_res.get(), c->stream.get()));
+    HIP_TRY(hipEventSynchronize(c->ev_res.get()));
     lap(c, s, 5);
     if ((rc = read_stage_times(c, s))) return rc;
     if (c->retire_kf_images) retire_keyframe_images(c, s);
@@ -527,8 +655,34 @@
 
 }
 
+namespace svo {
+
+void book_late(svo_group* c) {
+    LateBooking& b = c->late;
+    if (!b.pending) return;
+    b.pending = false;
+    book_stats(c, b.act, b.start, b.need, b.inside.data(), b.stage_ms, b.wall_ms);
+}
+
+void drop_ahead(svo_group* c) {
+    if (!c->ahead.valid) return;
+    c->ahead.valid = false;
+    for (int seq : c->ahead.act) release_set(c->seqs[seq], c->seqs[seq].next_set);
+}
+
+}
+
+bool grp_prefetch_allowed(int next_kind, bool failed, bool has_left, bool has_right, bool one_buffer) {
+    return next_kind == GRP_NEXT_FRAMES && !failed && has_left && (one_buffer || has_right);
+}
+
+void grp_settle(svo_group* c) {
+    book_late(c);
+    drop_ahead(c);
+}
+
 int grp_new_images(svo_group* c, const uint8_t* const* left, const uint8_t* const* right, int stride,
-                   const float* time_stamps, int mem) {
+                   const float* time_stamps, int mem, GroupPeek peek, void* queue) {
     if (!c || !left || (!right && c->fmt->buffers == 2) || !time_stamps ||
         (long long)stride < (long long)ingest_row_pixels(*c->fmt, c->width) * c->fmt->channels)
         return svo_set_error(SVO_ERR_INVALID, "svo_new_images: bad arguments");
@@ -536,7 +690,11 @@
         return svo_set_error(SVO_ERR_INVALID, "svo_new_images: an earlier frame of this ctx failed; create a new ctx");
     Step s;
     s.left = left; s.right = right; s.stride = stride; s.mem = mem; s.time_stamps = time_stamps;
+    s.peek = peek; s.queue = queue;
     const int rc = step(c, s);
-    if (rc != SVO_OK) c->failed = true;
+    if (rc != SVO_OK) {
+        c->failed = true;
+        grp_settle(c);
+    }
     return rc;
 }
diff --git a/stereo-svo-slam_amd/stereo_svo_slam_amd/hip_lib.py b/stereo-svo-slam_amd/stereo_svo_slam_amd/hip_lib.py
--- a/stereo-svo-slam_amd/stereo_svo_slam_amd/hip_lib.py
+++ b/stereo-svo-slam_amd/stereo_svo_slam_amd/hip_lib.py
@@ -14,7 +14,7 @@
     "svo_handle_set_stream", "svo_handle_synchronize", "svo_build_pyramid",
     "svo_build_lk_pyramid", "svo_sparse_align", "svo_klt_track", "svo_reproj_gn",
     "svo_ssd_disparity", "svo_depth_filter_update",
-    "svo_ctx_create", "svo_ctx_destroy", "svo_new_images", "svo_submit_images", "svo_wait",
+    "svo_ctx_create", "svo_ctx_destroy", "svo_new_images", "svo_submit_images", "svo_wait", "svo_step_prefetch_allowed",
     "svo_ctx_get_groups", "svo_new_image", "svo_get_pose",
     "svo_get_frame_keypoints", "svo_get_keyframe_count", "svo_get_keyframe",
     "svo_get_trajectory", "svo_update_pose", "svo_get_frame_stats", "svo_ctx_enable_timing",
```

Result: slower. 278,000 (-1.4%).
